# mpieva/mapping-iterative-assembler

Measured on AMD Instinct MI355X. Metric: reads aligned/sec per iteration (16.5kb mito ref, 100bp reads), higher is better.
Workload: dtype int32; 1 GPU; configs[1]: 1000000 synthetic 100 bp reads per GPU vs mt311 (16619 bp, circular), matrix flat; step = reiterate_assembly + pop_smp + cull + consensus; pass-1 coordinates = true positions; reads_per_gpu=1000000, total_reads=1000000, consensus_len=16619, bytes_per_read=182

## Files before the change

include/mia_hip.h:

```cpp
#ifndef MIA_HIP_H
#define MIA_HIP_H

#include <stddef.h>
#include <stdint.h>

#ifdef __cplusplus
extern "C" {
#endif

#define MIA_HIP_OK 0
#define MIA_HIP_ERR_DEVICE (-1)
#define MIA_HIP_ERR_ARG (-2)
#define MIA_HIP_ERR_RANGE (-3)
#define MIA_HIP_ERR_STATE (-4)
#define MIA_HIP_ERR_NOMEM (-5)

#define MIA_HIP_PSSM_WORDS (31 * 5 * 5)
#define MIA_HIP_MAX_READ 256
#define MIA_HIP_TALLY_WORDS 12

#define MIA_HIP_COL_INSERT (-1)
#define MIA_HIP_COL_CLIP (-2)

typedef struct mia_hip_ctx mia_hip_ctx;

int mia_hip_create(mia_hip_ctx **ctx, int device_index);
void mia_hip_destroy(mia_hip_ctx *ctx);
const char *mia_hip_last_error(const mia_hip_ctx *ctx);
int mia_hip_sync(mia_hip_ctx *ctx);


int mia_hip_set_pssm(mia_hip_ctx *ctx, const int32_t *fwd, const int32_t *rc);

int mia_hip_upload_reads(mia_hip_ctx *ctx, int64_t n_reads, const char *bases, const int64_t *offsets,
                         const uint8_t *rc, const uint8_t *strand_known, const int32_t *as, const int32_t *ae);


#define MIA_HIP_P1_PASSED 1
#define MIA_HIP_P1_KEPT 2
#define MIA_HIP_P1_STRAND_KNOWN 4
#define MIA_HIP_P1_SPLIT 8

int mia_hip_pass1(mia_hip_ctx *ctx, const char *ref, int32_t ref_len, int circular, int kmer_len, int soft_mask,
                  int64_t n_reads, const char *bases, const int64_t *offsets, int32_t *score, uint8_t *rc, int32_t *as,
                  int32_t *ae, uint8_t *flags);


int mia_hip_realign(mia_hip_ctx *ctx, const char *new_ref, int32_t ref_len, int circular);

int mia_hip_get_alignments(mia_hip_ctx *ctx, int32_t *score, int32_t *as, int32_t *ae);

int mia_hip_align_windows(mia_hip_ctx *ctx, const char *ref, int64_t ref_len, const int64_t *win_start, const int32_t *win_len);

int mia_hip_get_scripts(mia_hip_ctx *ctx, int16_t *cols, int32_t stride, int32_t *ref_start);

int mia_hip_cull(mia_hip_ctx *ctx, int32_t hard_cut, double slope, double intercept, int64_t slot_base);
int mia_hip_get_dropped(mia_hip_ctx *ctx, uint8_t *front_dropped, uint8_t *back_dropped);
int mia_hip_set_slot_dropped(mia_hip_ctx *ctx, const uint8_t *flags, int64_t n_flags);

int mia_hip_set_back_slots(mia_hip_ctx *ctx, const int64_t *back_slot);
int mia_hip_set_pass1_state(mia_hip_ctx *ctx, const int64_t *front_slot, const int64_t *back_slot, const int32_t *score);
int mia_hip_get_record_params(mia_hip_ctx *ctx, int32_t *params, int64_t *back_slot);
int mia_hip_set_read_base(mia_hip_ctx *ctx, int64_t read_base);
int mia_hip_links(mia_hip_ctx *ctx, int64_t **d_links, int64_t *n_links);
int mia_hip_set_links(mia_hip_ctx *ctx, const int64_t *d_links_all, int64_t n_all);
int mia_hip_link_lengths(mia_hip_ctx *ctx, int32_t **d_len, int32_t **d_act, int64_t *n);
int mia_hip_finish_links(mia_hip_ctx *ctx);

void mia_hip_score_cut(const int32_t *score, const int32_t *seq_len, const uint8_t *unique_best, int64_t n,
                       double *slope, double *intercept);
int mia_hip_pre_cull_counts(mia_hip_ctx *ctx, int64_t *n_records, int64_t *n_links);

int mia_hip_score_sums(mia_hip_ctx *ctx, int64_t *sums5);
int mia_hip_score_cut_from_sums(const int64_t *sums5, double *slope, double *intercept);
int mia_hip_num_records(mia_hip_ctx *ctx, int64_t *n_records);

int mia_hip_tally(mia_hip_ctx *ctx);
int mia_hip_tally_buffers(mia_hip_ctx *ctx, int32_t **d_tally, int64_t *n_tally_words, int32_t **d_gaps,
                          int64_t *n_gaps_words);
int mia_hip_ins_events(mia_hip_ctx *ctx, uint64_t **d_events, int64_t *n_events);
int mia_hip_set_ins_events(mia_hip_ctx *ctx, const uint64_t *d_events, int64_t n_events);
int mia_hip_get_tally(mia_hip_ctx *ctx, int32_t *tally, int32_t *gaps);
int mia_hip_set_tally(mia_hip_ctx *ctx, int32_t ref_len, const int32_t *tally, const int32_t *gaps);

int mia_hip_consensus(mia_hip_ctx *ctx, int cons_code, char *out, int64_t out_cap, int64_t *out_len);

int mia_hip_iterate(mia_hip_ctx *ctx, const char *new_ref, int32_t ref_len, int circular, int32_t hard_cut,
                    const double *slope_intercept, int cons_code, char *out, int64_t out_cap, int64_t *out_len);

#define MIA_HIP_COMM_ID_BYTES 128
int mia_hip_comm_unique_id(void *id128);
int mia_hip_comm_init(mia_hip_ctx *ctx, const void *id128, int32_t n_ranks, int32_t rank);
int mia_hip_comm_destroy(mia_hip_ctx *ctx);

#define MIA_HIP_OP_SUM 0
#define MIA_HIP_OP_MAX 1
typedef struct mia_hip_collectives {
  void *user;
  int32_t n_ranks, rank;
  int (*all_gather)(void *user, const void *d_send, void *d_recv, size_t bytes, void *hip_stream);
  int (*all_reduce_i32)(void *user, void *d_buf, size_t count, int op, void *hip_stream);
  int (*query)(void *user, int32_t *n_ranks, int32_t *rank);
  void (*abort)(void *user);
  void (*destroy)(void *user);
  const char *(*error)(void *user);
  const char *name;
} mia_hip_collectives;
int mia_hip_comm_attach(mia_hip_ctx *ctx, const mia_hip_collectives *table);
int mia_hip_comm_info(mia_hip_ctx *ctx, int32_t *n_ranks, int32_t *rank, const char **transport);

int mia_hip_loopback_create(int32_t n_ranks, void **group);
int mia_hip_loopback_table(void *group, int32_t rank, mia_hip_collectives *table);
void mia_hip_loopback_destroy(void *group);


int mia_hip_trim(mia_hip_ctx *ctx, const char *adapter, int64_t n_reads, const char *bases, const int64_t *offsets,
                 uint8_t *trimmed, int32_t *trim_point);

int mia_hip_trim_stats(mia_hip_ctx *ctx, int64_t *exact_reruns);

int mia_hip_trim_rerun_stats(mia_hip_ctx *ctx, int64_t *launches, int64_t *scratch_bytes);


int mia_hip_ma_tally(mia_hip_ctx *ctx, int32_t ref_len, const int32_t *gaps, int64_t n_records, const int32_t *start,
                     const uint8_t *revcom, const int64_t *col_off, const char *seq, const char *smp, int64_t n_ins,
                     const int32_t *ins_record, const int32_t *ins_pos, const int64_t *ins_off, const char *ins_bases);

int mia_hip_get_ins_tally(mia_hip_ctx *ctx, int32_t *ins_off, int32_t *ins_tally, int64_t cap_slots, int64_t *n_slots);

int mia_hip_ma_region(mia_hip_ctx *ctx, int32_t first, int32_t last, int64_t *n_rows, int64_t *width);
int mia_hip_get_ma_region(mia_hip_ctx *ctx, int64_t *rows, char *text, int64_t cap_rows);

int mia_hip_ma_ace(mia_hip_ctx *ctx, int64_t *n_records, int64_t *body_bytes);
int mia_hip_get_ma_ace(mia_hip_ctx *ctx, int64_t *af_pos, int64_t *padded_len, int64_t *body_off, char *body, int64_t cap_bytes);

int mia_hip_ma_sam(mia_hip_ctx *ctx, const char *ref_seq, int64_t *n_records, int64_t *body_bytes);
int mia_hip_get_ma_sam(mia_hip_ctx *ctx, int32_t *nm, int64_t *body_off, char *body, int64_t cap_bytes);

int mia_hip_ma_profile(mia_hip_ctx *ctx, const char *ref_seq, const uint8_t *use, int64_t *n_used, int64_t *n_events);
int mia_hip_get_ma_profile(mia_hip_ctx *ctx, int64_t *count, int64_t *del, int64_t *bad_code, int64_t *beyond);

int mia_hip_ma_ends(mia_hip_ctx *ctx, const char *ref_seq, const uint8_t *segment, const uint8_t *use, int64_t *n_used, int64_t *n_ends5,
                    int64_t *n_ends3);
int mia_hip_get_ma_ends(mia_hip_ctx *ctx, int64_t *ctx_count, int64_t *len_count, int64_t *halves);

int mia_hip_ma_cols(mia_hip_ctx *ctx, const uint8_t *segment, const uint8_t *use, int64_t *n_used, int64_t *n_events, int64_t *beyond,
                    int64_t *ends_outside);
int mia_hip_get_ma_cols(mia_hip_ctx *ctx, int32_t *cols);

int mia_hip_ma_dedup(mia_hip_ctx *ctx, int32_t ref_len, int64_t n_records, const int32_t *start, const int32_t *end, const uint8_t *revcom,
                     const int32_t *score, const int64_t *mate, int32_t tolerance, int64_t *n_molecules, int64_t *n_clusters);
int mia_hip_get_ma_dedup(mia_hip_ctx *ctx, uint8_t *keep, int64_t *rep, int64_t *size_hist, int64_t *orphans);

int mia_hip_ma_damage(mia_hip_ctx *ctx, const char *ref_seq, const uint8_t *use, const int64_t *mate, int32_t n_pos, int32_t single_stranded,
                      int32_t ends_mode, int64_t *n_molecules, int64_t *n_kept);
int mia_hip_get_ma_damage(mia_hip_ctx *ctx, uint8_t *pos5, uint8_t *pos3, uint8_t *keep, int64_t *hist, int64_t *orphans);

int mia_hip_ma_mask(mia_hip_ctx *ctx, int32_t n5, int32_t n3, int32_t mode, int32_t single_stranded, int64_t *n_kept, int64_t *cols_kept);
int mia_hip_get_ma_mask(mia_hip_ctx *ctx, int32_t *first, int32_t *count, int32_t *start, int64_t *col_off, char *seq, char *smp, int64_t cap_bytes,
                        uint8_t *pair_keep, int32_t *ins_pos, int64_t *hist, int64_t *scalars);


int mia_hip_myers(mia_hip_ctx *ctx, int64_t n_pairs, const char *const *seq_a, const char *const *seq_b, const int32_t *mode,
                  const int32_t *maxd, uint32_t *dist);

int mia_hip_myers_packed(mia_hip_ctx *ctx, int64_t n_pairs, const uint32_t *codes, int64_t n_words, const uint32_t *a_off, const uint32_t *b_off,
                         const int32_t *la, const int32_t *lb, const int32_t *mode, const int32_t *maxd, uint32_t *dist);

int mia_hip_myers_time(mia_hip_ctx *ctx, double *kernel_ms);

int mia_hip_myers_align(mia_hip_ctx *ctx, const char *seq_a, int32_t mode, const char *seq_b, int32_t maxd, uint32_t *dist,
                        char *bt_a, char *bt_b);

int mia_hip_kernel_time(mia_hip_ctx *ctx, int reset, double *align_ms, int64_t *align_launches);
int mia_hip_plain_stats(mia_hip_ctx *ctx, int reset, double *plain_ms, int64_t *plain_launches, int64_t *reads_in,
                        int64_t *reads_retried);

int mia_hip_filter_stats(mia_hip_ctx *ctx, int reset, int64_t *reads_seen, int64_t *reads_finished, double *kernel_ms, int64_t *launches);
int mia_hip_band_stats(mia_hip_ctx *ctx, int reset, int64_t *reads_finished, double *kernel_ms, int64_t *launches);
int mia_hip_bx_stats(mia_hip_ctx *ctx, int reset, int64_t *reads4, double *kernel_ms3, int64_t *launches);
int mia_hip_bx_counters(mia_hip_ctx *ctx, uint32_t *out32);
int mia_hip_stage_stats(mia_hip_ctx *ctx, int reset, int32_t cap, const char **names, double *ms, int64_t *launches, int32_t *n_stages);
int mia_hip_set_stage_mask(mia_hip_ctx *ctx, uint32_t mask);
int mia_hip_measure_peaks(mia_hip_ctx *ctx, int64_t copy_bytes, double *hbm_copy_gbs, double *valu_ginst_s);
int mia_hip_measure_issue(mia_hip_ctx *ctx, double *add_ginst_s, double *shader_clock_mhz);
int mia_hip_pass1_time(mia_hip_ctx *ctx, double *kernel_ms);
int mia_hip_pass1_filtered(mia_hip_ctx *ctx, int64_t *reads);
int mia_hip_pass1_anchored(mia_hip_ctx *ctx, int64_t *reads);

#ifdef __cplusplus
}
#endif
#endif
```

mapping-iterative-assembler_amd/__init__.py:

```python
import ctypes as C
import os

import numpy as np

_HERE = os.path.dirname(os.path.abspath(__file__))
LIB_PATH = os.environ.get("MIA_HIP_LIB") or os.path.join(_HERE, "libmia_hip.so")
ALT_LIB_PATH = os.path.join(_HERE, "libmia_hip_alt.so")
RELEASE_ENV = {"MIA_HIP_THREADS", "MIA_HIP_TIMING", "MIA_HIP_LOOPBACK_TIMEOUT", "MIA_HIP_SPIN_WAIT", "MIA_HIP_LIB"}


def alt_switches_set():
    return sorted(k for k in os.environ if k.startswith("MIA_HIP_") and k not in RELEASE_ENV)

PSSM_WORDS = 31 * 5 * 5
TALLY_WORDS = 12
COL_INSERT, COL_CLIP = -1, -2
P1_PASSED, P1_KEPT, P1_STRAND_KNOWN, P1_SPLIT = 1, 2, 4, 8


class MiaHipError(RuntimeError):
    pass


def _load(path=None):
    path = path or LIB_PATH
    if not os.path.exists(path):
        raise MiaHipError(f"{path} is missing: run __graft_entry__.build() (hipcc --offload-arch=gfx950)")
    lib = C.CDLL(path)
    P, vp = C.POINTER, C.c_void_p
    lib.mia_hip_create.argtypes = [P(vp), C.c_int]
    lib.mia_hip_destroy.argtypes = [vp]
    lib.mia_hip_destroy.restype = None
    lib.mia_hip_last_error.argtypes = [vp]
    lib.mia_hip_last_error.restype = C.c_char_p
    lib.mia_hip_sync.argtypes = [vp]
    lib.mia_hip_set_pssm.argtypes = [vp, vp, vp]
    lib.mia_hip_upload_reads.argtypes = [vp, C.c_int64, vp, vp, vp, vp, vp, vp]
    lib.mia_hip_pass1.argtypes = [vp, C.c_char_p, C.c_int32, C.c_int, C.c_int, C.c_int, C.c_int64, vp, vp, vp, vp, vp, vp, vp]
    lib.mia_hip_realign.argtypes = [vp, C.c_char_p, C.c_int32, C.c_int]
    lib.mia_hip_align_windows.argtypes = [vp, vp, C.c_int64, vp, vp]
    lib.mia_hip_get_alignments.argtypes = [vp, vp, vp, vp]
    lib.mia_hip_get_scripts.argtypes = [vp, vp, C.c_int32, vp]
    lib.mia_hip_cull.argtypes = [vp, C.c_int32, C.c_double, C.c_double, C.c_int64]
    lib.mia_hip_get_dropped.argtypes = [vp, vp, vp]
    lib.mia_hip_set_slot_dropped.argtypes = [vp, vp, C.c_int64]
    lib.mia_hip_score_cut.argtypes = [vp, vp, vp, C.c_int64, P(C.c_double), P(C.c_double)]
    lib.mia_hip_score_cut.restype = None
    lib.mia_hip_num_records.argtypes = [vp, P(C.c_int64)]
    lib.mia_hip_tally.argtypes = [vp]
    lib.mia_hip_tally_buffers.argtypes = [vp, P(vp), P(C.c_int64), P(vp), P(C.c_int64)]
    lib.mia_hip_ins_events.argtypes = [vp, P(vp), P(C.c_int64)]
    lib.mia_hip_set_ins_events.argtypes = [vp, vp, C.c_int64]
    lib.mia_hip_get_tally.argtypes = [vp, vp, vp]
    lib.mia_hip_set_tally.argtypes = [vp, C.c_int32, vp, vp]
    lib.mia_hip_iterate.argtypes = [vp, C.c_char_p, C.c_int32, C.c_int, C.c_int32, vp, C.c_int, vp, C.c_int64, P(C.c_int64)]
    lib.mia_hip_consensus.argtypes = [vp, C.c_int, vp, C.c_int64, P(C.c_int64)]
    lib.mia_hip_myers.argtypes = [vp, C.c_int64, vp, vp, vp, vp, vp]
    if hasattr(lib, "mia_hip_myers_packed"):
        lib.mia_hip_myers_packed.argtypes = [vp, C.c_int64, vp, C.c_int64, vp, vp, vp, vp, vp, vp, vp]
    lib.mia_hip_pre_cull_counts.argtypes = [vp, vp, vp]
    lib.mia_hip_filter_stats.argtypes = [vp, C.c_int, vp, vp, vp, vp]
    lib.mia_hip_band_stats.argtypes = [vp, C.c_int, vp, vp, vp]
    lib.mia_hip_bx_stats.argtypes = [vp, C.c_int, vp, vp, vp]
    lib.mia_hip_bx_counters.argtypes = [vp, vp]
    lib.mia_hip_myers_align.argtypes = [vp, C.c_char_p, C.c_int32, C.c_char_p, C.c_int32, vp, vp, vp]
    lib.mia_hip_pass1_time.argtypes = [vp, P(C.c_double)]
    lib.mia_hip_myers_time.argtypes = [vp, P(C.c_double)]
    lib.mia_hip_ma_tally.argtypes = [vp, C.c_int32, vp, C.c_int64, vp, vp, vp, vp, vp, C.c_int64, vp, vp, vp, vp]
    lib.mia_hip_trim.argtypes = [vp, C.c_char_p, C.c_int64, vp, vp, vp, vp]
    lib.mia_hip_set_back_slots.argtypes = [vp, vp]
    lib.mia_hip_set_pass1_state.argtypes = [vp, vp, vp, vp]
    lib.mia_hip_get_record_params.argtypes = [vp, vp, vp]
    lib.mia_hip_set_read_base.argtypes = [vp, C.c_int64]
    lib.mia_hip_links.argtypes = [vp, P(vp), P(C.c_int64)]
    lib.mia_hip_set_links.argtypes = [vp, vp, C.c_int64]
    lib.mia_hip_link_lengths.argtypes = [vp, P(vp), P(vp), P(C.c_int64)]
    lib.mia_hip_finish_links.argtypes = [vp]
    lib.mia_hip_plain_stats.argtypes = [vp, C.c_int, P(C.c_double), P(C.c_int64), P(C.c_int64), P(C.c_int64)]
    lib.mia_hip_score_sums.argtypes = [vp, vp]
    lib.mia_hip_score_cut_from_sums.argtypes = [vp, P(C.c_double), P(C.c_double)]
    lib.mia_hip_score_cut_from_sums.restype = C.c_int
    lib.mia_hip_trim_stats.argtypes = [vp, P(C.c_int64)]
    if hasattr(lib, "mia_hip_trim_rerun_stats"):
        lib.mia_hip_trim_rerun_stats.argtypes = [vp, P(C.c_int64), P(C.c_int64)]
    lib.mia_hip_get_ins_tally.argtypes = [vp, vp, vp, C.c_int64, P(C.c_int64)]
    if hasattr(lib, "mia_hip_ma_region"):
        lib.mia_hip_ma_region.argtypes = [vp, C.c_int32, C.c_int32, P(C.c_int64), P(C.c_int64)]
        lib.mia_hip_get_ma_region.argtypes = [vp, vp, vp, C.c_int64]
    if hasattr(lib, "mia_hip_ma_ace"):
        lib.mia_hip_ma_ace.argtypes = [vp, P(C.c_int64), P(C.c_int64)]
        lib.mia_hip_get_ma_ace.argtypes = [vp, vp, vp, vp, vp, C.c_int64]
    if hasattr(lib, "mia_hip_ma_sam"):
        lib.mia_hip_ma_sam.argtypes = [vp, vp, P(C.c_int64), P(C.c_int64)]
        lib.mia_hip_get_ma_sam.argtypes = [vp, vp, vp, vp, C.c_int64]
    if hasattr(lib, "mia_hip_ma_profile"):
        lib.mia_hip_ma_profile.argtypes = [vp, vp, vp, P(C.c_int64), P(C.c_int64)]
        lib.mia_hip_get_ma_profile.argtypes = [vp, vp, vp, P(C.c_int64), P(C.c_int64)]
    if hasattr(lib, "mia_hip_ma_ends"):
        lib.mia_hip_ma_ends.argtypes = [vp, vp, vp, vp, P(C.c_int64), P(C.c_int64), P(C.c_int64)]
        lib.mia_hip_get_ma_ends.argtypes = [vp, vp, vp, P(C.c_int64)]
    if hasattr(lib, "mia_hip_ma_cols"):
        lib.mia_hip_ma_cols.argtypes = [vp, vp, vp, P(C.c_int64), P(C.c_int64), P(C.c_int64), P(C.c_int64)]
        lib.mia_hip_get_ma_cols.argtypes = [vp, vp]
    if hasattr(lib, "mia_hip_ma_dedup"):
        lib.mia_hip_ma_dedup.argtypes = [vp, C.c_int32, C.c_int64, vp, vp, vp, vp, vp, C.c_int32, P(C.c_int64), P(C.c_int64)]
        lib.mia_hip_get_ma_dedup.argtypes = [vp, vp, vp, vp, P(C.c_int64)]
    if hasattr(lib, "mia_hip_ma_damage"):
        lib.mia_hip_ma_damage.argtypes = [vp, vp, vp, vp, C.c_int32, C.c_int32, C.c_int32, P(C.c_int64), P(C.c_int64)]
        lib.mia_hip_get_ma_damage.argtypes = [vp, vp, vp, vp, vp, P(C.c_int64)]
    if hasattr(lib, "mia_hip_ma_mask"):
        lib.mia_hip_ma_mask.argtypes = [vp, C.c_int32, C.c_int32, C.c_int32, C.c_int32, P(C.c_int64), P(C.c_int64)]
        lib.mia_hip_get_ma_mask.argtypes = [vp, vp, vp, vp, vp, vp, vp, C.c_int64, vp, vp, vp, vp]
    lib.mia_hip_kernel_time.argtypes = [vp, C.c_int, P(C.c_double), P(C.c_int64)]
    lib.mia_hip_stage_stats.argtypes = [vp, C.c_int, C.c_int32, vp, vp, vp, P(C.c_int32)]
    lib.mia_hip_set_stage_mask.argtypes = [vp, C.c_uint32]
    lib.mia_hip_comm_unique_id.argtypes = [vp]
    lib.mia_hip_comm_init.argtypes = [vp, vp, C.c_int32, C.c_int32]
    lib.mia_hip_comm_destroy.argtypes = [vp]
    lib.mia_hip_comm_attach.argtypes = [vp, vp]
    lib.mia_hip_comm_info.argtypes = [vp, P(C.c_int32), P(C.c_int32), P(C.c_char_p)]
    lib.mia_hip_loopback_create.argtypes = [C.c_int32, P(vp)]
    lib.mia_hip_loopback_table.argtypes = [vp, C.c_int32, vp]
    lib.mia_hip_loopback_destroy.argtypes = [vp]
    lib.mia_hip_loopback_destroy.restype = None
    lib.mia_hip_measure_peaks.argtypes = [vp, C.c_int64, P(C.c_double), P(C.c_double)]
    lib.mia_hip_measure_issue.argtypes = [vp, P(C.c_double), P(C.c_double)]
    return lib


_lib = None


def lib():
    global _lib
    if _lib is None:
        _lib = _load()
    return _lib


_alt_lib = None


def alt_lib():
    global _alt_lib
    if _alt_lib is None:
        _alt_lib = _load(ALT_LIB_PATH)
    return _alt_lib


def exported_symbols():
    return ["mia_hip_create", "mia_hip_destroy", "mia_hip_last_error", "mia_hip_sync", "mia_hip_set_pssm",
            "mia_hip_upload_reads", "mia_hip_pass1", "mia_hip_realign", "mia_hip_align_windows", "mia_hip_get_alignments", "mia_hip_get_scripts", "mia_hip_cull",
            "mia_hip_get_dropped", "mia_hip_set_slot_dropped", "mia_hip_score_cut", "mia_hip_num_records",
            "mia_hip_tally", "mia_hip_tally_buffers", "mia_hip_ins_events", "mia_hip_set_ins_events",
            "mia_hip_get_tally", "mia_hip_consensus", "mia_hip_myers", "mia_hip_myers_packed", "mia_hip_myers_align", "mia_hip_filter_stats", "mia_hip_band_stats", "mia_hip_bx_stats", "mia_hip_bx_counters", "mia_hip_kernel_time", "mia_hip_pass1_time", "mia_hip_myers_time", "mia_hip_pass1_filtered", "mia_hip_pass1_anchored", "mia_hip_pre_cull_counts", "mia_hip_ma_tally", "mia_hip_get_ins_tally", "mia_hip_ma_region", "mia_hip_get_ma_region", "mia_hip_ma_ace", "mia_hip_get_ma_ace", "mia_hip_ma_sam", "mia_hip_get_ma_sam", "mia_hip_ma_profile", "mia_hip_get_ma_profile", "mia_hip_ma_ends", "mia_hip_get_ma_ends", "mia_hip_ma_cols", "mia_hip_get_ma_cols", "mia_hip_ma_dedup", "mia_hip_get_ma_dedup", "mia_hip_ma_damage", "mia_hip_get_ma_damage", "mia_hip_ma_mask", "mia_hip_get_ma_mask", "mia_hip_trim", "mia_hip_trim_stats", "mia_hip_trim_rerun_stats", "mia_hip_set_back_slots", "mia_hip_set_pass1_state",
            "mia_hip_get_record_params", "mia_hip_set_read_base", "mia_hip_links", "mia_hip_set_links", "mia_hip_link_lengths",
            "mia_hip_finish_links", "mia_hip_plain_stats", "mia_hip_score_sums",
            "mia_hip_score_cut_from_sums", "mia_hip_stage_stats", "mia_hip_measure_peaks", "mia_hip_measure_issue", "mia_hip_set_tally", "mia_hip_iterate", "mia_hip_set_stage_mask", "mia_hip_comm_unique_id", "mia_hip_comm_init", "mia_hip_comm_destroy",
            "mia_hip_comm_attach", "mia_hip_comm_info", "mia_hip_loopback_create", "mia_hip_loopback_table", "mia_hip_loopback_destroy"]


def _ptr(a):
    return a.ctypes.data_as(C.c_void_p) if a is not None else None


def flat_pssm():
    p = np.zeros((31, 5, 5), dtype=np.int32)
    for i in range(5):
        for j in range(4):
            p[:, i, j] = 200 if i == j else -600
        p[:, i, 4] = -100
    p[:, 4, :] = -10
    return p


def revcom_pssm(p):
    idx = np.array([3, 2, 1, 0, 4])
    return np.ascontiguousarray(p[::-1][:, idx][:, :, idx]).astype(np.int32)


def read_pssm(path):
    p = np.zeros((31, 5, 5), dtype=np.int32)
    with open(path) as f:
        lines = f.read().split("\n")
    k = 0
    for d in range(31):
        if "# Matrix for position" not in lines[k]:
            raise ValueError(f"Problem parsing matrix file: {path}")
        for i in range(4):
            p[d, i, :4] = [int(x) for x in lines[k + 1 + i].split("\t")[:4]]
            p[d, i, 4] = -100
        p[d, 4, :] = -10
        k += 6
    return p


class Collectives(C.Structure):
    _fields_ = [("user", C.c_void_p), ("n_ranks", C.c_int32), ("rank", C.c_int32),
                ("all_gather", C.c_void_p), ("all_reduce_i32", C.c_void_p), ("query", C.c_void_p), ("abort", C.c_void_p),
                ("destroy", C.c_void_p), ("error", C.c_void_p), ("name", C.c_char_p)]


class LoopbackGroup:

    def __init__(self, n_ranks, like=None):
        self._l = like._l if like is not None else lib()
        self._g = C.c_void_p()
        if self._l.mia_hip_loopback_create(n_ranks, C.byref(self._g)) != 0:
            raise MiaHipError("mia_hip_loopback_create failed")
        self.n_ranks = n_ranks

    def attach(self, hip, rank):
        if hip._l is not self._l:
            raise MiaHipError("LoopbackGroup: this context comes from another build of the library than the group (pass like=<a context> when the group is made)")
        t = Collectives()
        if self._l.mia_hip_loopback_table(self._g, rank, C.byref(t)) != 0:
            raise MiaHipError("mia_hip_loopback_table failed")
        hip.comm_attach(t)

    def close(self):
        if self._g:
            self._l.mia_hip_loopback_destroy(self._g)
            self._g = C.c_void_p()


def comm_unique_id():
    buf = C.create_string_buffer(128)
    if lib().mia_hip_comm_unique_id(buf) != 0:
        raise MiaHipError("mia_hip_comm_unique_id failed: librccl could not be opened")
    return buf.raw


_IUPAC_BITS = np.zeros(256, np.uint8)
for _c, _v in zip("ACGTUSWRYKMBDHVN", (1, 2, 4, 8, 8, 6, 9, 5, 10, 12, 3, 14, 13, 11, 7, 15)):
    _IUPAC_BITS[ord(_c)] = _v
    _IUPAC_BITS[ord(_c.lower())] = _v


def pack_myers_pairs(seq_a, seq_b):
    n = len(seq_a)
    la = np.array([len(s) for s in seq_a], np.int32)
    lb = np.array([len(s) for s in seq_b], np.int32)
    wa, wb = (la + 7) // 8 + 1, (lb + 7) // 8 + 1
    tot = np.cumsum(np.stack([wa, wb], 1).reshape(-1).astype(np.int64))
    a_off = np.concatenate([[0], tot[1:-1:2]]).astype(np.uint32) if n else np.zeros(0, np.uint32)
    b_off = tot[0::2].astype(np.uint32)
    nib = np.zeros(int(tot[-1]) * 8 if n else 0, np.uint8)
    for i in range(n):
        a = np.frombuffer(seq_a[i] if isinstance(seq_a[i], bytes) else seq_a[i].encode(), np.uint8)
        b = np.frombuffer(seq_b[i] if isinstance(seq_b[i], bytes) else seq_b[i].encode(), np.uint8)
        nib[int(a_off[i]) * 8: int(a_off[i]) * 8 + len(a)] = _IUPAC_BITS[a]
        nib[int(b_off[i]) * 8: int(b_off[i]) * 8 + len(b)] = _IUPAC_BITS[b]
    codes = (nib.reshape(-1, 8).astype(np.uint32) << (4 * np.arange(8, dtype=np.uint32))).sum(axis=1).astype(np.uint32)
    return codes, a_off, b_off, la, lb


class MiaHip:

    def __init__(self, device=0):
        self.is_alt_build = bool(alt_switches_set() and not os.environ.get("MIA_HIP_LIB"))
        self._l = alt_lib() if self.is_alt_build else lib()
        self.lib_path = ALT_LIB_PATH if self.is_alt_build else LIB_PATH
        self._h = C.c_void_p()
        rc = self._l.mia_hip_create(C.byref(self._h), device)
        if rc != 0:
            raise MiaHipError(f"mia_hip_create failed ({rc}): no usable gfx950 device -- there is no CPU fallback")
        self.n = 0
        self.max_len = 0
        self.L = 0

    def close(self):
        if self._h:
            self._l.mia_hip_destroy(self._h)
            self._h = C.c_void_p()

    def __del__(self):
        try:
            self.close()
        except Exception:
            pass

    def _chk(self, rc):
        if rc != 0:
            raise MiaHipError(f"libmia_hip error {rc}: {self._l.mia_hip_last_error(self._h).decode()}")

    def set_pssm(self, fwd, rc=None):
        fwd = np.ascontiguousarray(fwd, dtype=np.int32)
        rc = np.ascontiguousarray(revcom_pssm(fwd) if rc is None else rc, dtype=np.int32)
        self._chk(self._l.mia_hip_set_pssm(self._h, _ptr(fwd), _ptr(rc)))

    def upload_reads(self, bases, offsets, rc, strand_known, as_, ae):
        bases = np.ascontiguousarray(bases, dtype=np.uint8)
        offsets = np.ascontiguousarray(offsets, dtype=np.int64)
        rc = np.ascontiguousarray(rc, dtype=np.uint8)
        sk = np.ascontiguousarray(strand_known, dtype=np.uint8)
        as_ = np.ascontiguousarray(as_, dtype=np.int32)
        ae = np.ascontiguousarray(ae, dtype=np.int32)
        self.n = len(offsets) - 1
        self.lens = (offsets[1:] - offsets[:-1]).astype(np.int32)
        self.max_len = int(self.lens.max()) if self.n else 0
        self._chk(self._l.mia_hip_upload_reads(self._h, self.n, _ptr(bases), _ptr(offsets), _ptr(rc), _ptr(sk), _ptr(as_), _ptr(ae)))

    def pass1(self, ref, circular, bases, offsets, kmer_len=-1, soft_mask=False):
        if isinstance(ref, str):
            ref = ref.encode()
        bases = np.ascontiguousarray(bases, dtype=np.uint8)
        offsets = np.ascontiguousarray(offsets, dtype=np.int64)
        n = len(offsets) - 1
        score = np.zeros(n, np.int32); as_ = np.zeros(n, np.int32); ae = np.zeros(n, np.int32)
        rc = np.zeros(n, np.uint8); flags = np.zeros(n, np.uint8)
# ... 307 lines not shown
            raise ValueError("ma_ends: the reference has %d characters, the tallied job %d columns" % (len(ref), self.L))
        if segment is not None:
            if isinstance(segment, str):
                segment = segment.encode("latin1")
            segment = np.frombuffer(segment, np.uint8) if isinstance(segment, (bytes, bytearray)) else np.ascontiguousarray(segment, dtype=np.uint8)
        if use is not None:
            use = np.ascontiguousarray(use, dtype=np.uint8)
        ctx, lens = np.zeros((2, 20, 6), dtype=np.int64), np.zeros((2, 513), dtype=np.int64)
        halves = C.c_int64()
        self._chk(self._l.mia_hip_ma_ends(self._h, C.c_char_p(ref), _ptr(segment) if segment is not None and segment.size else None,
                                          _ptr(use) if use is not None and use.size else None, None, None, None))
        self._chk(self._l.mia_hip_get_ma_ends(self._h, _ptr(ctx), _ptr(lens), C.byref(halves)))
        return ctx, lens, halves.value

    def ma_cols(self, segment=None, use=None):
        if segment is not None:
            if isinstance(segment, str):
                segment = segment.encode("latin1")
            segment = np.frombuffer(segment, np.uint8) if isinstance(segment, (bytes, bytearray)) else np.ascontiguousarray(segment, dtype=np.uint8)
        if use is not None:
            use = np.ascontiguousarray(use, dtype=np.uint8)
        cols = np.zeros((16, self.L), dtype=np.int32)
        n_used, n_events, beyond, outside = C.c_int64(), C.c_int64(), C.c_int64(), C.c_int64()
        self._chk(self._l.mia_hip_ma_cols(self._h, _ptr(segment) if segment is not None and segment.size else None,
                                          _ptr(use) if use is not None and use.size else None, C.byref(n_used), C.byref(n_events),
                                          C.byref(beyond), C.byref(outside)))
        self._chk(self._l.mia_hip_get_ma_cols(self._h, _ptr(cols)))
        return cols, n_used.value, n_events.value, beyond.value, outside.value

    def ma_dedup(self, ref_len, start, end, revcom, score, mate=None, tolerance=0):
        if not hasattr(self._l, "mia_hip_ma_dedup"):
            raise RuntimeError("this libmia_hip has no mia_hip_ma_dedup")
        start = np.ascontiguousarray(start, dtype=np.int32)
        end = np.ascontiguousarray(end, dtype=np.int32)
        revcom = np.ascontiguousarray(revcom, dtype=np.uint8)
        score = np.ascontiguousarray(score, dtype=np.int32)
        n = len(start)
        if not (len(end) == len(revcom) == len(score) == n):
            raise ValueError("ma_dedup: the arrays differ in length")
        if mate is not None:
            mate = np.ascontiguousarray(mate, dtype=np.int64)
            if len(mate) != n:
                raise ValueError("ma_dedup: the arrays differ in length")
        keep, rep, hist = np.zeros(n, dtype=np.uint8), np.zeros(n, dtype=np.int64), np.zeros((2, 1025), dtype=np.int64)
        n_mol, n_clu, orphans = C.c_int64(), C.c_int64(), C.c_int64()
        opt = lambda a: _ptr(a) if n else None
        self._chk(self._l.mia_hip_ma_dedup(self._h, int(ref_len), n, opt(start), opt(end), opt(revcom), opt(score),
                                           _ptr(mate) if mate is not None and n else None, int(tolerance), C.byref(n_mol), C.byref(n_clu)))
        self._chk(self._l.mia_hip_get_ma_dedup(self._h, opt(keep), opt(rep), _ptr(hist), C.byref(orphans)))
        return keep, rep, hist, n_mol.value, n_clu.value, orphans.value

    DAMAGE_MODES = {"any": 0, "5": 1, "3": 2, "both": 3}

    def ma_damage(self, ref_seq, n_pos, use=None, mate=None, single_stranded=False, mode="any"):
        if not hasattr(self._l, "mia_hip_ma_damage"):
            raise RuntimeError("this libmia_hip has no mia_hip_ma_damage")
        ref = ref_seq.encode("latin1") if isinstance(ref_seq, str) else bytes(ref_seq)
        if len(ref) != self.L:
            raise ValueError("ma_damage: the reference has %d characters, the tallied job %d columns" % (len(ref), self.L))
        if mode not in self.DAMAGE_MODES:
            raise ValueError("ma_damage: mode must be one of any, 5, 3, both")
        if use is not None:
            use = np.ascontiguousarray(use, dtype=np.uint8)
        if mate is not None:
            mate = np.ascontiguousarray(mate, dtype=np.int64)
        n = getattr(self, "_ma_n", 0)
        if (use is not None and len(use) != n) or (mate is not None and len(mate) != n):
            raise ValueError("ma_damage: use and mate hold one entry per tallied record (%d)" % n)
        n_mol, n_kept, orphans = C.c_int64(), C.c_int64(), C.c_int64()
        self._chk(self._l.mia_hip_ma_damage(self._h, C.c_char_p(ref), _ptr(use) if use is not None and use.size else None,
                                            _ptr(mate) if mate is not None and mate.size else None, int(n_pos), 1 if single_stranded else 0,
                                            self.DAMAGE_MODES[mode], C.byref(n_mol), C.byref(n_kept)))
        pos5, pos3, keep = np.zeros(n, dtype=np.uint8), np.zeros(n, dtype=np.uint8), np.zeros(n, dtype=np.uint8)
        hist = np.zeros((2, 16, 16), dtype=np.int64)
        opt = lambda a: _ptr(a) if n else None
        self._chk(self._l.mia_hip_get_ma_damage(self._h, opt(pos5), opt(pos3), opt(keep), _ptr(hist), C.byref(orphans)))
        return pos5, pos3, keep, hist, n_mol.value, n_kept.value, orphans.value

    def ma_mask(self, n5, n3, substitute=False, single_stranded=False):
        if not hasattr(self._l, "mia_hip_ma_mask"):
            raise RuntimeError("this libmia_hip has no mia_hip_ma_mask")
        n_kept, cols_kept = C.c_int64(), C.c_int64()
        self._chk(self._l.mia_hip_ma_mask(self._h, int(n5), int(n3), 1 if substitute else 0, 1 if single_stranded else 0, C.byref(n_kept), C.byref(cols_kept)))
        n = getattr(self, "_ma_n", 0)
        n_ins = getattr(self, "_ma_n_ins", 0)
        first, count, start = np.zeros(n, dtype=np.int32), np.zeros(n, dtype=np.int32), np.zeros(n, dtype=np.int32)
        col_off = np.zeros(n + 1, dtype=np.int64)
        seq, smp = np.zeros(cols_kept.value, dtype=np.uint8), np.zeros(cols_kept.value, dtype=np.uint8)
        pair_keep, ins_pos = np.zeros(n_ins, dtype=np.uint8), np.zeros(n_ins, dtype=np.int32)
        hist, scalars = np.zeros((2, 2, 16), dtype=np.int64), np.zeros(6, dtype=np.int64)
        opt = lambda a: _ptr(a) if a.size else None
        self._chk(self._l.mia_hip_get_ma_mask(self._h, opt(first), opt(count), opt(start), _ptr(col_off), opt(seq), opt(smp), cols_kept.value, opt(pair_keep),
                                              opt(ins_pos), _ptr(hist), _ptr(scalars)))
        return {"first": first, "count": count, "start": start, "col_off": col_off, "seq": seq, "smp": smp, "pair_keep": pair_keep, "ins_pos": ins_pos, "hist": hist,
                "emptied": [int(scalars[0]), int(scalars[1])], "stripped": int(scalars[2]), "pairs_dropped": int(scalars[3]), "n_kept": int(scalars[4]),
                "cols_kept": int(scalars[5])}

    def ins_tally(self):
        n = C.c_int64()
        off = np.empty(self.L + 1, dtype=np.int32)
        self._chk(self._l.mia_hip_get_ins_tally(self._h, _ptr(off), None, 0, C.byref(n)))
        t = np.zeros((max(n.value, 1), 9), dtype=np.int32)
        if n.value:
            self._chk(self._l.mia_hip_get_ins_tally(self._h, None, _ptr(t), n.value, None))
        return off, t[: n.value]

    def trim(self, adapter, bases, offsets):
        if isinstance(adapter, str):
            adapter = adapter.encode()
        bases = np.ascontiguousarray(bases, dtype=np.uint8)
        offsets = np.ascontiguousarray(offsets, dtype=np.int64)
        n = len(offsets) - 1
        trimmed = np.zeros(n, np.uint8)
        point = np.zeros(n, np.int32)
        self._chk(self._l.mia_hip_trim(self._h, adapter, n, _ptr(bases), _ptr(offsets), _ptr(trimmed), _ptr(point)))
        return trimmed, point

    def set_back_slots(self, back_slot):
        b = np.ascontiguousarray(back_slot, dtype=np.int64)
        assert len(b) == self.n
        self._chk(self._l.mia_hip_set_back_slots(self._h, _ptr(b)))

    def set_pass1_state(self, front_slot=None, back_slot=None, score=None):
        f = None if front_slot is None else np.ascontiguousarray(front_slot, dtype=np.int64)
        b = None if back_slot is None else np.ascontiguousarray(back_slot, dtype=np.int64)
        sc = None if score is None else np.ascontiguousarray(score, dtype=np.int32)
        self._chk(self._l.mia_hip_set_pass1_state(self._h, _ptr(f), _ptr(b), _ptr(sc)))

    def record_params(self):
        p = np.empty((self.n, 8), dtype=np.int32)
        b = np.empty(self.n, dtype=np.int64)
        self._chk(self._l.mia_hip_get_record_params(self._h, _ptr(p), _ptr(b)))
        return p, b

    def set_read_base(self, base):
        self._chk(self._l.mia_hip_set_read_base(self._h, int(base)))

    def links(self):
        p, n = C.c_void_p(), C.c_int64()
        self._chk(self._l.mia_hip_links(self._h, C.byref(p), C.byref(n)))
        return p.value, n.value

    def set_links(self, dptr, n):
        self._chk(self._l.mia_hip_set_links(self._h, C.c_void_p(dptr), int(n)))

    def link_lengths(self):
        p, q, n = C.c_void_p(), C.c_void_p(), C.c_int64()
        self._chk(self._l.mia_hip_link_lengths(self._h, C.byref(p), C.byref(q), C.byref(n)))
        return p.value, q.value, n.value

    def finish_links(self):
        self._chk(self._l.mia_hip_finish_links(self._h))

    def plain_stats(self, reset=False):
        ms, a, b, c = C.c_double(), C.c_int64(), C.c_int64(), C.c_int64()
        self._chk(self._l.mia_hip_plain_stats(self._h, 1 if reset else 0, C.byref(ms), C.byref(a), C.byref(b), C.byref(c)))
        return ms.value, a.value, b.value, c.value

    def trim_exact_reruns(self):
        n = C.c_int64()
        self._chk(self._l.mia_hip_trim_stats(self._h, C.byref(n)))
        return n.value

    def trim_rerun_stats(self):
        a, b = C.c_int64(), C.c_int64()
        self._chk(self._l.mia_hip_trim_rerun_stats(self._h, C.byref(a), C.byref(b)))
        return a.value, b.value

    def pass1_time(self):
        ms = C.c_double()
        self._chk(self._l.mia_hip_pass1_time(self._h, C.byref(ms)))
        return ms.value

    def sync(self):
        self._chk(self._l.mia_hip_sync(self._h))
```

mapping-iterative-assembler_amd/csrc/mia_consensus_kernels.h:

```cpp
#pragma once
#include <hip/hip_runtime.h>
#include <stdint.h>

#include "ma_records.h"
#include "mia_kernels.h"
#include "mia_layout.h"

namespace mia {

struct TallyBuf {
  int32_t* tally;
  int32_t Lp;
  int32_t* gaps;
  uint64_t* events;
  int32_t* n_events;
  int32_t cap_events;
  uint32_t* flags;
};

struct RecGeom {
  int start_w, end, split, ncols_f, ncols_b;
};
MIA_HD inline RecGeom rec_geom(int as, int ae, int L) {
  RecGeom g;
  g.start_w = as;
  g.end = ae > L ? ae - L : ae;
  g.split = as > g.end;
  g.ncols_f = g.split ? (L - as) : (g.end - as + 1);
  g.ncols_b = g.split ? g.end + 1 : 0;
  return g;
}

__global__ void k_scan_blocks(ReadSet rs, int32_t L, int64_t* partial) {
  __shared__ int32_t sh[256];
  const int64_t base = ((int64_t)blockIdx.x * 256 + threadIdx.x) * 16;
  int32_t s = 0;
  for (int k = 0; k < 16; k++) {
    int64_t i = base + k;
    if (i < rs.n && rs.sk[i]) s += rec_geom(rs.as[i], rs.ae[i], L).split ? 2 : 1;
  }
  sh[threadIdx.x] = s;
  __syncthreads();
  for (int o = 128; o > 0; o >>= 1) {
    if ((int)threadIdx.x < o) sh[threadIdx.x] += sh[threadIdx.x + o];
    __syncthreads();
  }
  if (threadIdx.x == 0) partial[blockIdx.x] = sh[0];
}
__global__ __launch_bounds__(256) void k_scan_partials(int64_t* partial, int nb, int64_t base, int64_t* total, const int32_t* abort_if = nullptr) {
  if (abort_if && *abort_if != 0) return;
  __shared__ int64_t s_run[256];
  const int t = threadIdx.x, per = (nb + 255) / 256, b0 = t * per, b1 = b0 + per < nb ? b0 + per : nb;
  int64_t mine = 0;
  for (int b = b0; b < b1; b++) mine += partial[b];
  const int lane = t & 63, w = t >> 6;
  int64_t inc = mine;
#pragma unroll
  for (int o = 1; o < 64; o <<= 1) { const int64_t u = (int64_t)__shfl_up((long long)inc, o); if (lane >= o) inc += u; }
  if (lane == 63) s_run[w] = inc;
  __syncthreads();
  int64_t off = 0;
  for (int k = 0; k < w; k++) off += s_run[k];
  const int64_t all = s_run[0] + s_run[1] + s_run[2] + s_run[3];
  int64_t run = base + off + inc - mine;
  for (int b = b0; b < b1; b++) { const int64_t v = partial[b]; partial[b] = run; run += v; }
  if (t == 255) *total = all;
}
__global__ void k_scan_apply(ReadSet rs, int32_t L, const int64_t* partial, int64_t* slot) {
  __shared__ int32_t sh[256];
  const int64_t base = ((int64_t)blockIdx.x * 256 + threadIdx.x) * 16;
  int32_t cnt[16], s = 0;
  for (int k = 0; k < 16; k++) {
    int64_t i = base + k;
    cnt[k] = (i < rs.n && rs.sk[i]) ? (rec_geom(rs.as[i], rs.ae[i], L).split ? 2 : 1) : 0;
    s += cnt[k];
  }
  sh[threadIdx.x] = s;
  __syncthreads();
  for (int o = 1; o < 256; o <<= 1) {
    int32_t v = ((int)threadIdx.x >= o) ? sh[threadIdx.x - o] : 0;
    __syncthreads();
    sh[threadIdx.x] += v;
    __syncthreads();
  }
  int64_t run = partial[blockIdx.x] + sh[threadIdx.x] - s;
  for (int k = 0; k < 16; k++) {
    int64_t i = base + k;
    if (i < rs.n) slot[i] = run;
    run += cnt[k];
  }
}

__global__ void k_score_sums_init(unsigned long long* sums, const int32_t* wide_count) {
  if (threadIdx.x == 0) {
    sums[0] = 0; sums[1] = 0; sums[2] = 0; sums[3] = (unsigned long long)(long long)INT32_MAX; sums[4] = (unsigned long long)(long long)INT32_MIN; sums[5] = 0; sums[6] = 0;
    sums[7] = wide_count ? (unsigned long long)*wide_count : 0;
  }
}

__global__ __launch_bounds__(256) void k_score_sums(ReadSet rs, unsigned long long* out, int32_t L, const int64_t* back_slot,
                                                     const int64_t* front_slot0) {
  __shared__ unsigned long long sh[5][256];
  __shared__ int shl[2][256];
  unsigned long long sx = 0, sy = 0, j = 0, nrec = 0, nlink = 0;
  int lmin = INT32_MAX, lmax = INT32_MIN;
  for (int64_t i = (int64_t)blockIdx.x * blockDim.x + threadIdx.x; i < rs.n; i += (int64_t)gridDim.x * blockDim.x) {
    const int sc = rs.score[i], ln = rs.len[i];
    if (sc >= 2000) { sx += (unsigned long long)ln; sy += (unsigned long long)sc; j++; lmin = ln < lmin ? ln : lmin; lmax = ln > lmax ? ln : lmax; }
    if (rs.sk[i]) {
      const bool split = rec_geom(rs.as[i], rs.ae[i], L).split;
      nrec += split ? 2 : 1;
      if (!split && back_slot[i] >= 0) nlink++;
    } else {
      nlink += (front_slot0[i] >= 0) + (back_slot[i] >= 0);
    }
  }
  sh[0][threadIdx.x] = sx; sh[1][threadIdx.x] = sy; sh[2][threadIdx.x] = j; sh[3][threadIdx.x] = nrec; sh[4][threadIdx.x] = nlink;
  shl[0][threadIdx.x] = lmin; shl[1][threadIdx.x] = lmax;
  __syncthreads();
  for (int o = 128; o > 0; o >>= 1) {
    if ((int)threadIdx.x < o) {
      for (int k = 0; k < 5; k++) sh[k][threadIdx.x] += sh[k][threadIdx.x + o];
      shl[0][threadIdx.x] = min(shl[0][threadIdx.x], shl[0][threadIdx.x + o]);
      shl[1][threadIdx.x] = max(shl[1][threadIdx.x], shl[1][threadIdx.x + o]);
    }
    __syncthreads();
  }
  if (threadIdx.x == 0) {
    atomicAdd(&out[0], sh[0][0]); atomicAdd(&out[1], sh[1][0]); atomicAdd(&out[2], sh[2][0]);
    atomicAdd(&out[5], sh[3][0]); atomicAdd(&out[6], sh[4][0]);
    atomicMin(reinterpret_cast<long long*>(&out[3]), (long long)shl[0][0]);
    atomicMax(reinterpret_cast<long long*>(&out[4]), (long long)shl[1][0]);
  }
}

struct RecInfo {
  int32_t* flen;
  int32_t* blen;
  int32_t* actf;
  int32_t* trec;
};
enum { TREC_AS = 0, TREC_AE, TREC_LEN_ABR, TREC_FLAGS, TREC_REFSTART, TREC_ROFF, TREC_ACTF, TREC_SPARE, TREC_PARAMS = 8 };
constexpr int TRF_RC = 1, TRF_DF = 2, TRF_DB = 4, TRF_DIAG = 8, TRF_TOO_LONG = 16, TRF_SK = 32, TRF_ONEGAP = 64;
constexpr int TRF_NO_N = 128;
__device__ __forceinline__ void rec_write(const ReadSet& rs, int64_t i, int32_t* trec, uint8_t* drop_front, uint8_t* drop_back, uint8_t df, uint8_t db, const int32_t* p,
                                          uint32_t st, int32_t actf, const int32_t* umax) {
  drop_front[i] = df;
  drop_back[i] = db;
  int4* t4 = reinterpret_cast<int4*>(trec + i * 16);
  const int fl = (rs.rc[i] ? TRF_RC : 0) | (df ? TRF_DF : 0) | (db ? TRF_DB : 0) | ((st & ST_DIAG) ? TRF_DIAG : 0) |
                 ((st & ST_TOO_LONG) ? TRF_TOO_LONG : 0) | (rs.sk[i] ? TRF_SK : 0) | ((st & ST_ONEGAP) ? TRF_ONEGAP : 0) |
                 ((umax && umax[i] >= 0) ? TRF_NO_N : 0);
  t4[0] = make_int4(rs.as[i], rs.ae[i], (int32_t)((uint32_t)rs.len[i] | ((uint32_t)(uint16_t)rs.abr[i] << 16)), fl);
  t4[1] = make_int4(rs.refstart[i], (int32_t)rs.roff[i], actf, (int32_t)(st >> 8));
  t4[2] = make_int4(p[0], p[1], p[2], p[3]);
  t4[3] = make_int4(p[4], p[5], p[6], p[7]);
}

__device__ __forceinline__ void rec_make(const ReadSet& rs, int64_t i, uint8_t* drop_front, uint8_t* drop_back, uint8_t df, uint8_t db, const int32_t* p,
                                         uint32_t st, int32_t actf, const int32_t* umax, int4* r4) {
  drop_front[i] = df;
  drop_back[i] = db;
  const int fl = (rs.rc[i] ? TRF_RC : 0) | (df ? TRF_DF : 0) | (db ? TRF_DB : 0) | ((st & ST_DIAG) ? TRF_DIAG : 0) |
                 ((st & ST_TOO_LONG) ? TRF_TOO_LONG : 0) | (rs.sk[i] ? TRF_SK : 0) | ((st & ST_ONEGAP) ? TRF_ONEGAP : 0) |
                 ((umax && umax[i] >= 0) ? TRF_NO_N : 0);
  r4[0] = make_int4(rs.as[i], rs.ae[i], (int32_t)((uint32_t)rs.len[i] | ((uint32_t)(uint16_t)rs.abr[i] << 16)), fl);
  r4[1] = make_int4(rs.refstart[i], (int32_t)rs.roff[i], actf, (int32_t)(st >> 8));
  r4[2] = make_int4(p[0], p[1], p[2], p[3]);
  r4[3] = make_int4(p[4], p[5], p[6], p[7]);
}
__device__ __forceinline__ void rec_store_wave(int32_t* trec, int64_t i0, int64_t n, const int4* r4, int lane, int4* buf) {
#pragma unroll
  for (int q = 0; q < 4; q++) buf[lane * 4 + q] = r4[q];
  __builtin_amdgcn_fence(__ATOMIC_RELEASE, "wavefront");
  __builtin_amdgcn_wave_barrier();
  __builtin_amdgcn_fence(__ATOMIC_ACQUIRE, "wavefront");
  int4* out = reinterpret_cast<int4*>(trec) + i0 * 4;
#pragma unroll
  for (int k = 0; k < 4; k++) {
    const int w = k * 64 + lane;
    if (i0 + (w >> 2) < n) out[w] = buf[w];
  }
}

struct SlotInfo {
  int64_t base;
  const int64_t* n_local_p;
  int32_t* reclen;
  int32_t* recact;
  unsigned long long* writer;
  int32_t* mult;
};
constexpr unsigned long long LINK_NONE = 0xFFFFFull;
struct Links {
  int64_t* rec;
  int32_t* n;
  int32_t cap;
};

__device__ __forceinline__ void rec_store_at(int64_t i, const RecGeom& g, int nf, int nb, int af, int bases, int64_t slot_i, RecInfo& ri,
                                             SlotInfo& si, int64_t read_base, uint32_t* flags) {
  const int flen = g.ncols_f + nf, blen = g.split ? g.ncols_b + nb : 0;
  ri.flen[i] = flen; ri.blen[i] = blen; ri.actf[i] = af + nf;
  const int64_t ls = slot_i - si.base;
  if (ls >= 0 && ls + (g.split ? 1 : 0) < (*si.n_local_p)) {
    const unsigned long long me = ((unsigned long long)(read_base + i) << 20) | LINK_NONE;
    si.reclen[ls] = flen; si.recact[ls] = af + nf; si.mult[ls] = 1; si.writer[ls] = me;
    if (g.split) { si.reclen[ls + 1] = blen; si.recact[ls + 1] = bases - (af + nf); si.mult[ls + 1] = 1; si.writer[ls + 1] = me; }
  } else atomicOr(flags, 4u);
}
__device__ __forceinline__ void rec_store(int64_t i, const RecGeom& g, int nf, int nb, int af, int bases, const int64_t* slot, RecInfo& ri,
                                          SlotInfo& si, int64_t read_base, uint32_t* flags) {
  rec_store_at(i, g, nf, nb, af, bases, slot[i], ri, si, read_base, flags);
}

__global__ __launch_bounds__(256) void k_rec_geom(ReadSet rs, int32_t L, const int64_t* slot, RecInfo ri, SlotInfo si, int64_t read_base,
                                                    uint32_t* flags) {
  const int lane = threadIdx.x & 63;
  const int64_t i0 = (int64_t)blockIdx.x * 256 + (threadIdx.x & ~63);
  const int64_t me = i0 + lane;
  bool walk = false;
  if (me < rs.n) {
    if (!rs.sk[me]) { ri.flen[me] = 0; ri.blen[me] = 0; ri.actf[me] = 0; }
    else if (rs.status[me] & ST_DIAG) {
      const int len2 = rs.len[me], abr = rs.abr[me];
      const RecGeom g = rec_geom(rs.as[me], rs.ae[me], L);
      const int af = (len2 - abr) < g.ncols_f ? (len2 - abr) : g.ncols_f;
      rec_store(me, g, 0, 0, af, len2 - abr, slot, ri, si, read_base, flags);
    } else if ((rs.status[me] & ST_ONEGAP) && !rec_geom(rs.as[me], rs.ae[me], L).split) {
      const uint32_t desc = rs.status[me] >> 8;
      const int len2 = rs.len[me], abr = rs.abr[me], gn = (int)((desc >> 10) & 63u), ins = (int)(desc & 1u);
      const RecGeom g = rec_geom(rs.as[me], rs.ae[me], L);
      rec_store(me, g, ins ? gn : 0, 0, len2 - abr - (ins ? gn : 0), len2 - abr, slot, ri, si, read_base, flags);
    } else walk = true;
  }
  unsigned long long todo = __ballot(walk);
  while (todo) {
    const int64_t i = i0 + __builtin_ctzll(todo);
    todo &= todo - 1;
    const int len2 = rs.len[i], abr = rs.abr[i];
    const RecGeom g = rec_geom(rs.as[i], rs.ae[i], L);
    const int16_t* cols = rs.cols + (int64_t)i * rs.stride;
    const int cbase = rs.refstart[i] - g.start_w;
    int nf = 0, nb = 0, af = 0;
    int n_ev = 0, ins_rows = 0, ev_row = 0, ev_len = 0, ev_kind = 0;
    for (int r0 = abr; r0 < len2; r0 += 64) {
      const int r = r0 + lane;
      bool isF = false, isB = false, alF = false, ins_row = false, ins_start = false, jump = false;
      int jump_len = 0;
      if (r < len2) {
        const int cp = r > abr ? (int)cols[r - 1] : -3;
        if (cols[r] == COL_INSERT) {
          int rn = r + 1;
          while (rn < len2 && cols[rn] < 0) rn++;
          const int o = cbase + cols[rn];
          if (o < g.ncols_f) isF = true; else if (g.split && o - g.ncols_f < g.ncols_b) isB = true;
          ins_row = true;
          ins_start = cp != COL_INSERT;
        } else if (cols[r] >= 0) {
          alF = (cbase + cols[r]) < g.ncols_f;
          if (cp >= 0 && cols[r] - cp > 1) { jump = true; jump_len = cols[r] - cp - 1; }
        }
      }
      nf += __popcll(__ballot(isF));
      nb += __popcll(__ballot(isB));
      af += __popcll(__ballot(alF));
      const unsigned long long m_ins = __ballot(ins_start), m_del = __ballot(jump);
      ins_rows += __popcll(__ballot(ins_row));
      if (n_ev == 0 && (m_ins | m_del)) {
        const int l = __builtin_ctzll(m_ins | m_del);
        ev_row = r0 + l;
        ev_kind = (int)((m_ins >> l) & 1ull);
        ev_len = __shfl(jump_len, l);
      }
      n_ev += __popcll(m_ins) + __popcll(m_del);
    }
    if (lane == 0) {
      const uint32_t st = rs.status[i];
      if (!(st & (ST_ESCAPE | ST_TOO_LONG | ST_SKIPPED | ST_BAND | ST_DIAG))) {
        const int gn = ev_kind ? ins_rows : ev_len, n_al = len2 - abr;
        const bool one = n_ev == 1 && !g.split && gn > 0 && gn < 64 && ev_row < 512 && g.ncols_f == (ev_kind ? n_al - gn : n_al + gn);
        const uint32_t want = one ? (ST_ONEGAP | (((uint32_t)ev_kind | ((uint32_t)ev_row << 1) | ((uint32_t)gn << 10)) << 8)) : ST_OK;
        if (st != want) rs.status[i] = want;
      }
    }
    if (lane == 0) rec_store(i, g, nf, nb, af, len2 - abr, slot, ri, si, read_base, flags);
  }
}

__global__ __launch_bounds__(256) void k_slot_count(ReadSet rs, int32_t L, int64_t* partial, int nb, int64_t base, int64_t* total, uint32_t* blocks_done, const int32_t* abort_if = nullptr) {
  if (abort_if && *abort_if != 0) return;
  __shared__ bool last;
  __shared__ int64_t s_run[256];
  __shared__ int32_t wsum[16][4];
  const int64_t base_read = (int64_t)blockIdx.x * 4096;
  uint8_t sk16[16];
  int32_t as16[16], ae16[16];
#pragma unroll
  for (int k = 0; k < 16; k++) {
    const int64_t i = base_read + k * 256 + threadIdx.x;
    const bool in = i < rs.n;
    sk16[k] = in ? rs.sk[i] : (uint8_t)0;
    as16[k] = in ? rs.as[i] : 0;
    ae16[k] = in ? rs.ae[i] : 0;
  }
#pragma unroll
  for (int k = 0; k < 16; k++) {
    const int cnt = sk16[k] ? (rec_geom(as16[k], ae16[k], L).split ? 2 : 1) : 0;
    const int w = __popcll(__ballot(cnt >= 1)) + __popcll(__ballot(cnt == 2));
    if ((threadIdx.x & 63) == 0) wsum[k][threadIdx.x >> 6] = w;
  }
  __syncthreads();
  if (threadIdx.x < 16 && blockIdx.x * 16 + (int)threadIdx.x < nb)
    partial[blockIdx.x * 16 + threadIdx.x] = (int64_t)wsum[threadIdx.x][0] + wsum[threadIdx.x][1] + wsum[threadIdx.x][2] + wsum[threadIdx.x][3];
  if (!blocks_done) {
    if (threadIdx.x == 0) {
      int64_t g = 0;
      for (int k = 0; k < 16; k++) g += (int64_t)wsum[k][0] + wsum[k][1] + wsum[k][2] + wsum[k][3];
      partial[nb + blockIdx.x] = g;
    }
    return;
  }
  __threadfence();
  __syncthreads();
  if (threadIdx.x == 0) last = atomicAdd(blocks_done, 1u) == (uint32_t)gridDim.x - 1u;
  __syncthreads();
  if (!last) return;
  __threadfence();
  const int t = threadIdx.x, per = (nb + 255) / 256, b0 = t * per, b1 = b0 + per < nb ? b0 + per : nb;
  int64_t mine = 0;
  for (int b2 = b0; b2 < b1; b2++) mine += __builtin_nontemporal_load(partial + b2);
  s_run[t] = mine;
  __syncthreads();
  for (int o = 1; o < 256; o <<= 1) {
    const int64_t a2 = t >= o ? s_run[t - o] : 0;
    __syncthreads();
    s_run[t] += a2;
    __syncthreads();
  }
  int64_t run = base + s_run[t] - mine;
  for (int b2 = b0; b2 < b1; b2++) { const int64_t v = __builtin_nontemporal_load(partial + b2); partial[b2] = run; run += v; }
  if (t == 255) *total = s_run[255];
  if (t == 0) *blocks_done = 0;
}

__global__ __launch_bounds__(256) void k_cull_records(ReadSet rs, int32_t L, const int64_t* partial, int64_t* slot, RecInfo ri, SlotInfo si, int64_t read_base,
                                                        uint32_t* flags, uint8_t* slot_dropped, int64_t n_slots, int32_t hard_cut, double slope, double intercept,
                                                        int64_t* back_slot, const int64_t* front_slot0, Links lk, const double* dev_cut, const int32_t* abort_if = nullptr,
                                                        int32_t raw_nb = 0, int64_t slot_base = 0, int64_t* total_out = nullptr,
                                                        int32_t with_records = 0, uint8_t* drop_front = nullptr, uint8_t* drop_back = nullptr, const int32_t* umax = nullptr) {
  if (abort_if && *abort_if != 0) return;
  __shared__ int32_t wsum[4];
  __shared__ int64_t s_red[2][4], s_first, s_total;
  const int lane = threadIdx.x & 63, wv = threadIdx.x >> 6;
  if (raw_nb) {
    const int ng = (raw_nb + 15) >> 4, myg = (int)(blockIdx.x >> 4);
    int64_t pre = 0, tot = 0;
    for (int g = threadIdx.x; g < ng; g += 256) { const int64_t v = partial[raw_nb + g]; tot += v; if (g < myg) pre += v; }
    if (threadIdx.x < 16) { const int b = myg * 16 + (int)threadIdx.x; if (b < (int)blockIdx.x) pre += partial[b]; }
#pragma unroll
    for (int o = 32; o; o >>= 1) { pre += __shfl_xor(pre, o); tot += __shfl_xor(tot, o); }
    if (lane == 0) { s_red[0][wv] = pre; s_red[1][wv] = tot; }
    __syncthreads();
    if (threadIdx.x == 0) {
      s_first = slot_base + s_red[0][0] + s_red[0][1] + s_red[0][2] + s_red[0][3];
      s_total = s_red[1][0] + s_red[1][1] + s_red[1][2] + s_red[1][3];
      if (blockIdx.x == 0 && total_out) *total_out = s_total;
    }
    si.n_local_p = &s_total;
  }
  const int64_t i0 = (int64_t)blockIdx.x * 256 + (threadIdx.x & ~63);
  const int64_t me = i0 + lane;
  const bool in = me < rs.n;
  const bool sk = in && rs.sk[me];
  int as_me = 0, ae_me = 0;
  if (sk) { as_me = rs.as[me]; ae_me = rs.ae[me]; }
  const RecGeom g_me = rec_geom(as_me, ae_me, L);
  const int cnt = sk ? (g_me.split ? 2 : 1) : 0;
  const unsigned long long m1 = __ballot(cnt >= 1), m2 = __ballot(cnt == 2), below = (1ull << lane) - 1ull;
  if (lane == 0) wsum[wv] = __popcll(m1) + __popcll(m2);
  __syncthreads();
  int64_t my_slot = (raw_nb ? s_first : partial[blockIdx.x]) + __popcll(m1 & below) + __popcll(m2 & below);
  for (int k = 0; k < wv; k++) my_slot += wsum[k];
  if (in) slot[me] = my_slot;
  int my_flen = 0, my_actf = 0, my_blen = 0;
  uint32_t my_st = in ? rs.status[me] : 0u;
  bool walk = false;
  if (in) {
    if (!sk) { ri.flen[me] = 0; ri.blen[me] = 0; ri.actf[me] = 0; }
    else if (rs.status[me] & ST_DIAG) {
      const int len2 = rs.len[me], abr = rs.abr[me];
      const int af = (len2 - abr) < g_me.ncols_f ? (len2 - abr) : g_me.ncols_f;
      rec_store_at(me, g_me, 0, 0, af, len2 - abr, my_slot, ri, si, read_base, flags);
      my_flen = g_me.ncols_f; my_actf = af; my_blen = g_me.split ? g_me.ncols_b : 0;
    } else if ((rs.status[me] & ST_ONEGAP) && !g_me.split) {
      const uint32_t desc = rs.status[me] >> 8;
      const int len2 = rs.len[me], abr = rs.abr[me], gn = (int)((desc >> 10) & 63u), ins = (int)(desc & 1u);
      rec_store_at(me, g_me, ins ? gn : 0, 0, len2 - abr - (ins ? gn : 0), len2 - abr, my_slot, ri, si, read_base, flags);
      my_flen = g_me.ncols_f + (ins ? gn : 0); my_actf = len2 - abr;
    } else walk = true;
  }
  unsigned long long todo = __ballot(walk);
  while (todo) {
    const int li = __builtin_ctzll(todo);
    const int64_t i = i0 + li;
    todo &= todo - 1;
    const int len2 = rs.len[i], abr = rs.abr[i];
    const RecGeom g = rec_geom(rs.as[i], rs.ae[i], L);
    const int16_t* cols = rs.cols + (int64_t)i * rs.stride;
    const int cbase = rs.refstart[i] - g.start_w;
    int nf = 0, nb = 0, af = 0;
    int n_ev = 0, ins_rows = 0, ev_row = 0, ev_len = 0, ev_kind = 0;
    for (int r0 = abr; r0 < len2; r0 += 64) {
      const int r = r0 + lane;
      bool isF = false, isB = false, alF = false, ins_row = false, ins_start = false, jump = false;
      int jump_len = 0;
      if (r < len2) {
        const int cp = r > abr ? (int)cols[r - 1] : -3;
        if (cols[r] == COL_INSERT) {
          int rn = r + 1;
          while (rn < len2 && cols[rn] < 0) rn++;
          const int o = cbase + cols[rn];
          if (o < g.ncols_f) isF = true; else if (g.split && o - g.ncols_f < g.ncols_b) isB = true;
          ins_row = true;
          ins_start = cp != COL_INSERT;
        } else if (cols[r] >= 0) {
          alF = (cbase + cols[r]) < g.ncols_f;
          if (cp >= 0 && cols[r] - cp > 1) { jump = true; jump_len = cols[r] - cp - 1; }
        }
      }
      nf += __popcll(__ballot(isF));
      nb += __popcll(__ballot(isB));
      af += __popcll(__ballot(alF));
      const unsigned long long m_ins = __ballot(ins_start), m_del = __ballot(jump);
      ins_rows += __popcll(__ballot(ins_row));
      if (n_ev == 0 && (m_ins | m_del)) {
        const int l = __builtin_ctzll(m_ins | m_del);
        ev_row = r0 + l;
        ev_kind = (int)((m_ins >> l) & 1ull);
        ev_len = __shfl(jump_len, l);
      }
      n_ev += __popcll(m_ins) + __popcll(m_del);
    }
    const int64_t slot_i = __shfl(my_slot, li);
    uint32_t st_new = rs.status[i];
    if (!(st_new & (ST_ESCAPE | ST_TOO_LONG | ST_SKIPPED | ST_BAND | ST_DIAG))) {
      const int gn = ev_kind ? ins_rows : ev_len, n_al = len2 - abr;
      const bool one = n_ev == 1 && !g.split && gn > 0 && gn < 64 && ev_row < 512 && g.ncols_f == (ev_kind ? n_al - gn : n_al + gn);
      const uint32_t want = one ? (ST_ONEGAP | (((uint32_t)ev_kind | ((uint32_t)ev_row << 1) | ((uint32_t)gn << 10)) << 8)) : ST_OK;
      if (st_new != want) { if (lane == 0) rs.status[i] = want; st_new = want; }
    }
    if (lane == 0) rec_store_at(i, g, nf, nb, af, len2 - abr, slot_i, ri, si, read_base, flags);
    if (lane == li) { my_flen = g.ncols_f + nf; my_actf = af + nf; my_blen = g.split ? g.ncols_b + nb : 0; my_st = st_new; }
  }
  __shared__ int4 s_rec[4][256];
  int4 r4[4] = {make_int4(0, 0, 0, 0), make_int4(0, 0, 0, 0), make_int4(0, 0, 0, 0), make_int4(0, 0, 0, 0)};
  if (in) {
  if (dev_cut) { slope = dev_cut[0]; intercept = dev_cut[1]; }
  const double min_score = hard_cut > 0 ? (double)hard_cut : (double)(intercept + (slope * (double)rs.len[me]));
  const bool low = (double)rs.score[me] < min_score;
  auto add_link = [&](int64_t target, int kind, int fl, int ac) {
    const int e = atomicAdd(lk.n, 1);
    if (e < lk.cap) {
      int64_t* r = lk.rec + (int64_t)e * 4;
      r[0] = read_base + me; r[1] = target;
      r[2] = ((int64_t)fl << 32) | (uint32_t)ac;
      r[3] = (low ? 1 : 0) | (kind << 8);
    } else atomicOr(flags, 8u);
  };
  int32_t p[8] = {0, 0, 0, 0, 0, 0, 0, 0};
  if (!sk) {
    if (front_slot0[me] >= 0) add_link(front_slot0[me], 1, 0, 0);
    if (back_slot[me] >= 0) add_link(back_slot[me], 2, 0, 0);
    if (with_records) rec_make(rs, me, drop_front, drop_back, 0, 0, p, my_st, 0, umax, r4);
  } else {
  uint8_t df = 0, db = 0;
  if (with_records && my_slot < n_slots) df = low ? (uint8_t)1 : slot_dropped[my_slot];
  if (with_records && g_me.split && my_slot + 1 < n_slots) db = low ? (uint8_t)1 : slot_dropped[my_slot + 1];
  if (low && my_slot < n_slots) slot_dropped[my_slot] = 1;
  if (g_me.split) {
    if (low && my_slot + 1 < n_slots) slot_dropped[my_slot + 1] = 1;
    back_slot[me] = my_slot + 1;
  } else if (back_slot[me] >= 0) add_link(back_slot[me], 0, my_flen, my_actf);
  if (with_records) {
    const int64_t ls = my_slot - si.base, n_local = *si.n_local_p;
    if (ls >= 0 && ls < n_local) { p[2] = my_flen + my_blen; p[3] = 1; }
    if (g_me.split && ls + 1 < n_local) { p[4] = my_flen; p[5] = my_actf; p[6] = my_flen + my_blen; p[7] = 1; }
    rec_make(rs, me, drop_front, drop_back, df, db, p, my_st, my_actf, umax, r4);
  }
  }
  }
  if (with_records) rec_store_wave(ri.trec, i0, rs.n, r4, lane, s_rec[wv]);
}

__global__ void k_cull_mark(ReadSet rs, int32_t L, const int64_t* slot, uint8_t* slot_dropped, int64_t n_slots, int32_t hard_cut, double slope,
                            double intercept, int64_t* back_slot, const int64_t* front_slot0, RecInfo ri, Links lk, int64_t read_base,
                            uint32_t* flags, const double* dev_cut) {
  int64_t i = (int64_t)blockIdx.x * blockDim.x + threadIdx.x;
  if (i >= rs.n) return;
  if (dev_cut) { slope = dev_cut[0]; intercept = dev_cut[1]; }
  const double min_score = hard_cut > 0 ? (double)hard_cut : (double)(intercept + (slope * (double)rs.len[i]));
  const bool low = (double)rs.score[i] < min_score;
  auto add_link = [&](int64_t target, int kind, int fl, int ac) {
    const int e = atomicAdd(lk.n, 1);
    if (e < lk.cap) {
      int64_t* r = lk.rec + (int64_t)e * 4;
      r[0] = read_base + i; r[1] = target;
      r[2] = ((int64_t)fl << 32) | (uint32_t)ac;
      r[3] = (low ? 1 : 0) | (kind << 8);
    } else atomicOr(flags, 8u);
  };
  if (!rs.sk[i]) {
    if (front_slot0[i] >= 0) add_link(front_slot0[i], 1, 0, 0);
    if (back_slot[i] >= 0) add_link(back_slot[i], 2, 0, 0);
    return;
  }
  const bool split = rec_geom(rs.as[i], rs.ae[i], L).split;
  const int64_t s = slot[i];
  if (low && s < n_slots) slot_dropped[s] = 1;
  if (split) {
    if (low && s + 1 < n_slots) slot_dropped[s + 1] = 1;
    back_slot[i] = s + 1;
  } else if (back_slot[i] >= 0) add_link(back_slot[i], 0, ri.flen[i], ri.actf[i]);
}

__global__ void k_links_apply(const int64_t* links, const int32_t* n_links_p, int32_t cap, SlotInfo si, uint8_t* slot_dropped, int64_t n_slots,
                              int32_t* link_len, int32_t* link_act, uint32_t* flags, const int32_t* abort_if = nullptr) {
  if (abort_if && *abort_if != 0) return;
  const int n_links = min(*n_links_p, cap);
  for (int e = blockIdx.x * blockDim.x + threadIdx.x; e < n_links; e += gridDim.x * blockDim.x) {
    const int64_t* r = links + (int64_t)e * 4;
    const int64_t ls = r[1] - si.base;
    link_len[e] = -1;
    link_act[e] = -1;
    if (ls < 0 || ls >= (*si.n_local_p)) continue;
    atomicMax(&si.writer[ls], ((unsigned long long)r[0] << 20) | (unsigned long long)e);
    atomicAdd(&si.mult[ls], 1);
    if ((r[3] & 1) && r[1] < n_slots) slot_dropped[r[1]] = 1;
    link_len[e] = si.reclen[ls];
    link_act[e] = si.recact[ls];
  }
}

__global__ void k_rec_params(ReadSet rs, int32_t L, const int64_t* slot, const uint8_t* slot_dropped, int64_t n_slots, const int64_t* back_slot,
                             RecInfo ri, SlotInfo si, const int64_t* links, const int32_t* link_len, const int32_t* link_act, const int32_t* n_links_p,
                             int32_t cap, int64_t read_base,
                             uint8_t* drop_front, uint8_t* drop_back, uint32_t* flags, const int32_t* abort_if = nullptr,
                             const int32_t* umax = nullptr,
                             int32_t skip_if_no_links = 0) {
  if (abort_if && *abort_if != 0) return;
  if (skip_if_no_links && *n_links_p == 0) return;
  int64_t i = (int64_t)blockIdx.x * blockDim.x + threadIdx.x;
  if (i >= rs.n) return;
  const int n_links = min(*n_links_p, cap);
  uint8_t df = 0, db = 0;
  int32_t p[8] = {0, 0, 0, 0, 0, 0, 0, 0};
  if (rs.sk[i]) {
    const bool split = rec_geom(rs.as[i], rs.ae[i], L).split;
    const int64_t s = slot[i], ls = s - si.base;
    if (s < n_slots) df = slot_dropped[s];
    if (split && s + 1 < n_slots) db = slot_dropped[s + 1];
    const int flen = ri.flen[i], blen = ri.blen[i], actf = ri.actf[i];
    int back_len = blen;
    if (!split && back_slot[i] >= 0) {
      back_len = -1;
      for (int e = 0; e < n_links; e++)
        if (links[(int64_t)e * 4] == read_base + i && (links[(int64_t)e * 4 + 3] >> 8) == 0) { back_len = link_len[e]; break; }
      if (back_len < 0) { atomicOr(flags, 4u); back_len = 0; }
    }
    auto fill = [&](int32_t* q, int64_t lsl, int own_base, int own_off, int own_B, int own_len) {
      const unsigned long long w = si.writer[lsl];
      if ((w & LINK_NONE) == LINK_NONE) { q[0] = own_base; q[1] = own_off; q[2] = own_B; }
      else {
        const int we = (int)(w & LINK_NONE);
        const int64_t* r = links + (int64_t)we * 4;
        const int kind = (int)(r[3] >> 8);
        if (kind == 0) {
          const int rf = (int)(r[2] >> 32), ra = (int)(uint32_t)r[2];
          q[0] = rf; q[1] = ra; q[2] = rf + own_len;
        } else {
          int sib_len = 0, sib_act = 0;
          for (int e = 0; e < n_links; e++)
            if (links[(int64_t)e * 4] == r[0] && (links[(int64_t)e * 4 + 3] >> 8) == 3 - kind) {
              sib_len = link_len[e]; sib_act = link_act[e];
              if (sib_len < 0) { atomicOr(flags, 4u); sib_len = 0; sib_act = 0; }
              break;
            }
          if (kind == 1) { q[0] = 0; q[1] = 0; q[2] = own_len + sib_len; }
          else { q[0] = sib_len; q[1] = sib_act; q[2] = sib_len + own_len; }
        }
      }
      q[3] = si.mult[lsl];
    };
    if (ls >= 0 && ls < (*si.n_local_p)) fill(p, ls, 0, 0, flen + back_len, flen);
    if (split && ls + 1 < (*si.n_local_p)) fill(p + 4, ls + 1, flen, actf, flen + blen, blen);
  }
  const uint32_t st = rs.status[i];
  rec_write(rs, i, ri.trec, drop_front, drop_back, df, db, p, st, ri.actf[i], umax);
}

__device__ __forceinline__ int depth_code(int dff, int dfb) {
  return dff <= PSSM_DEPTH ? dff : (dfb < PSSM_DEPTH ? 2 * PSSM_DEPTH - dfb : PSSM_DEPTH);
}

constexpr int TALLY_EV_CAP = 256;
constexpr int TALLY_CHUNK_LINEAR = 256;
constexpr int TALLY_BUCKET = 128, TALLY_WIN = 384, TALLY_CHUNK = 512;

__device__ __forceinline__ int tally_slot(int gc, int win_base, int Lp) {
  const int wc = gc - win_base;
  return wc < 0 ? wc + Lp : wc;
}

template <bool BINNED>
__device__ __forceinline__ void tally_one_read(int64_t i, int lane, const ReadSet& rs, const RefInfo& ref, const int32_t* pssm2,
                                               const uint8_t* drop_front, const uint8_t* drop_back, const TallyBuf& tb,
                                               int32_t* lds, int win_base, const int32_t* rec_params, const int32_t* rec_actf,
                                               const int16_t* pssm_lds, unsigned long long* ev_buf, int* ev_cnt, int32_t* n_cnt = nullptr,
                                               const int32_t* rec_lds = nullptr) {
  const int32_t* tr = rec_lds ? rec_lds : rec_params + i * 16;
  const int flags = tr[TREC_FLAGS];
  if (!(flags & TRF_SK)) return;
  if (flags & TRF_TOO_LONG) { if (lane == 0) atomicOr(tb.flags, 2u); return; }
  const int L = ref.L, Lp = tb.Lp;
  const int len2 = tr[TREC_LEN_ABR] & 0xFFFF, abr = (int)(int16_t)((uint32_t)tr[TREC_LEN_ABR] >> 16);
  const RecGeom g = rec_geom(tr[TREC_AS], tr[TREC_AE], L);
  const int16_t* cols = rs.cols + (int64_t)i * rs.stride;
  const int cbase = tr[TREC_REFSTART] - g.start_w;
  const uint8_t* rp = rs.packed + (uint32_t)tr[TREC_ROFF];
  const bool is_rc = (flags & TRF_RC) != 0;
  const int pmo = is_rc ? PSSM_WORDS : 0;
  const int32_t* pm = pssm2 + pmo;
  const bool dF = (flags & TRF_DF) != 0, dB = (flags & TRF_DB) != 0;
  const bool diag = (flags & TRF_DIAG) != 0;
  if (g.split && g.start_w >= L) { if (lane == 0) atomicOr(tb.flags, 2u); return; }
  const int32_t* prm = tr + TREC_PARAMS;
  const int fBase = prm[0], fOff = prm[1], fB = prm[2], fMult = prm[3], bBase = prm[4], bOff = prm[5], bB = prm[6], bMult = prm[7];
  const int actF = tr[TREC_ACTF];
  auto dcode = [&](bool back, int act) {
    const int a = back ? bOff + (act - actF) : fOff + act;
    return depth_code((back ? bBase : fBase) + a, (back ? bB : fB) - a - 1);
  };
  auto emit = [&](int o, int act, int code ) {
    int p, gc, mult;
    bool dropped, back;
    if (o < g.ncols_f) { p = o; gc = g.start_w + o; back = false; dropped = dF; mult = fMult; }
    else if (g.split && o - g.ncols_f < g.ncols_b) { p = o - g.ncols_f; gc = p; back = true; dropped = dB; mult = bMult; }
    else return;
    if (gc < 0 || gc >= Lp) { atomicOr(tb.flags, 2u); return; }
    const int d = dcode(back, act);
    if (d < 0 || d > 2 * PSSM_DEPTH) { atomicOr(tb.flags, 2u); return; }
    const int wc = tally_slot(gc, win_base, Lp);
    const bool in_lds = BINNED && wc >= 0 && wc < TALLY_WIN;
    int s0 = 0, s1 = 0, s2 = 0, s3 = 0;
    if (!dropped && code != 5) {
      if (BINNED) { const int16_t* row = pssm_lds + pmo + d * 25 + code; s0 = row[0]; s1 = row[5]; s2 = row[10]; s3 = row[15]; }
      else { const int32_t* row = pm + d * 25 + code; s0 = row[0]; s1 = row[5]; s2 = row[10]; s3 = row[15]; }
    }
    auto aadd = [](auto* q, int v) { (void)__hip_atomic_fetch_add(q, v, __ATOMIC_RELAXED, __HIP_MEMORY_SCOPE_AGENT); };
    auto add_all = [&](auto* t, const int ws, auto* ncount) {
      if (!dropped) {
        aadd(&t[T_COV * ws], mult);
        if (code == 5) aadd(&t[T_GAP * ws], mult);
        else {
          if (code < 4) aadd(&t[(T_A + code) * ws], mult);
          else if (ncount) aadd(ncount, mult);
          if (!ncount) {
            aadd(&t[T_SA * ws], mult * s0);
            aadd(&t[T_SC * ws], mult * s1);
            aadd(&t[T_SG * ws], mult * s2);
            aadd(&t[T_ST * ws], mult * s3);
          }
        }
      }
      if (p > 0) aadd(&t[T_SPAN * ws], mult);
// ... 1137 lines not shown
```

mapping-iterative-assembler_amd/csrc/mia_hip.hip:

```cpp
#include <hip/hip_runtime.h>
#include <atomic>
#include <hip/hip_ext.h>
#include <stdio.h>
#include <stdlib.h>
#include <string.h>

#include <algorithm>
#include <cmath>
#include <chrono>
#include <optional>
#include <string>
#include <thread>
#include <tuple>
#include <utility>
#include <vector>

#include "../../include/mia_hip.h"
#include "dev_buf.h"
#include "ref_ahead.h"
#include "dev_pool.h"
#include "mia_comm.h"
#include "mia_consensus_kernels.h"
#include "mia_kernels.h"
#include "bandx_kernels.h"
#include "align_route.h"
#include "pass1_route.h"
#include "mia_pass1_kernels.h"
#include "mia_myers_kernels.h"
#include "mia_trim_kernels.h"
#include "mia_peak_kernels.h"
#include "mia_iter_kernels.h"
#include "mia_ma_region_kernels.h"
#include "mia_ma_ace_kernels.h"
#include "mia_ma_sam_kernels.h"
#include "mia_ma_profile_kernels.h"
#include "mia_ma_ends_kernels.h"
#include "mia_ma_cols_kernels.h"
#include "mia_ma_dedup_kernels.h"
#include "mia_ma_damage_kernels.h"
#include "mia_ma_mask_kernels.h"

using namespace mia;

enum Stage { STG_TRACE = 0, STG_PLAIN, STG_FILTER, STG_BAND, STG_BX_PLAN, STG_BX_VALUES, STG_BX_TRACE, STG_TALLY, STG_PASS1, STG_MA_SELECT, STG_MA_RENDER, STG_MA_ACE_LAYOUT, STG_MA_ACE_RENDER, STG_MA_MASK_BOUNDS, STG_MA_MASK_LAYOUT, STG_MA_MASK_APPLY, STG_MA_SAM_LAYOUT, STG_MA_SAM_RENDER, STG_MA_DAMAGE_HITS, STG_MA_DAMAGE_MOLECULES, STG_MA_PROFILE, STG_MA_DEDUP_KEYS, STG_MA_DEDUP_SORT, STG_MA_DEDUP_RUNS, STG_MA_DEDUP_NEXT, STG_MA_DEDUP_ANCHORS, STG_MA_DEDUP_CLUSTERS, STG_MA_TALLY, STG_MA_COLS, STG_MA_ENDS, STG_COUNT };
static const char* const STAGE_NAMES[STG_COUNT] = {"k_align_quad", "k_align_quad_plain", "k_diag_filter", "k_band_align", "k_bx_plan",
                                                   "k_bx_values", "k_bx_trace", "k_tally_binned", "k_pass1", "k_ma_region_select",
                                                   "k_ma_region_render", "k_ma_ace_layout", "k_ma_ace_render", "k_ma_mask_bounds", "k_ma_mask_layout", "k_ma_mask_apply", "k_ma_sam_layout",
                                                   "k_ma_sam_render", "k_ma_damage_hits", "k_ma_damage_molecules", "k_ma_profile", "k_ma_dedup_keys", "k_ma_dedup_sort", "k_ma_dedup_runs",
                                                   "k_ma_dedup_next", "k_ma_dedup_anchors", "k_ma_dedup_clusters", "k_ma_tally", "k_ma_cols", "k_ma_ends"};

constexpr int OPEN_WGS = 1024;
constexpr int64_t OPEN_SLAB_BYTES = (int64_t)MAX_READ * 64 * 12;
constexpr int CTRL_BINS = 0;
constexpr int CTRL_HDR = (3 * N_BINS + 2 + 1) & ~1;
constexpr int CTRL_FILTER = CTRL_HDR + PH_WORDS;
constexpr int CTRL_LKN = CTRL_FILTER + 4, CTRL_CULLF = CTRL_LKN + 1, CTRL_NEV = CTRL_CULLF + 1, CTRL_TFLAGS = CTRL_NEV + 1;
constexpr int CTRL_GENN = CTRL_TFLAGS + 2;
constexpr int CTRL_BXC = (CTRL_GENN + 1 + 63) & ~63;
constexpr int CTRL_WORDS = CTRL_BXC + BXC_WORDS;
constexpr int CTRL_C0 = CTRL_BINS + 3 * N_BINS, CTRL_CN = CTRL_WORDS - CTRL_C0;

#ifdef MIA_HIP_ALT_PATHS
static inline const char* alt_env(const char* name) { return getenv(name); }
#define ALT_KERNEL(k) ((const void*)(k))
#else
static inline const char* alt_env(const char*) { return nullptr; }
#define ALT_KERNEL(k) ((const void*)nullptr)
#endif
static inline std::optional<int> alt_int(const char* name) {
  const char* v = alt_env(name);
  return v ? std::optional<int>(atoi(v)) : std::nullopt;
}

struct mia_hip_ctx {
  int device = 0;
  int cus = 1;
  std::string err;
  DevPool pool;
  unsigned char* h_pin = nullptr; static constexpr size_t PIN_BYTES = 1 << 20, PIN_MISC = 64 << 10;
  DevBuf<int32_t> d_ctrl; int ctrl_half = 0;
  int32_t* ctrl = nullptr;
  int32_t* d_genn = nullptr;
  const int32_t* d_ctr0 = nullptr;
  uint32_t dbg = 0;

  hipStream_t stream = nullptr;
  hipStream_t stream2 = nullptr; hipEvent_t ev_fork = nullptr, ev_join = nullptr;
  hipEvent_t ev_cons = nullptr;
  hipStream_t stream3 = nullptr; hipEvent_t ev_join3 = nullptr;
  uint32_t ext_events = 31u; bool align_end_signalled = false;
  bool spin_wait = true;
  uint32_t stage_mask = ~0u;
  struct StageTimer { std::vector<std::pair<hipEvent_t, hipEvent_t>> pending; double ms = 0; int64_t launches = 0; };
  StageTimer stg[STG_COUNT];
  std::vector<std::pair<hipEvent_t, hipEvent_t>> ev_free;

  DevBuf<int32_t> d_pssm;
  int max_abs = 0;
  int max_pos = 0;
  bool have_pssm = false;
  bool flat = false;
  PackSet packs;
  ReadSet rs{};
  DevBuf<uint8_t> d_packed; DevBuf<uint32_t> d_roff; DevBuf<uint16_t> d_len;
  DevBuf<uint8_t> d_rc, d_sk;
  DevBuf<int32_t> d_as, d_ae, d_score, d_refstart;
  DevBuf<int16_t> d_abr; DevBuf<uint32_t> d_status; DevBuf<int16_t> d_cols;
  int max_len = 0;
  int min_len = 0;
  std::vector<int32_t> h_len;
  DevBuf<uint64_t> d_rplanes; int rplane_words = 0;
  DevBuf<int32_t> d_umax; bool umax_valid = false;
  DevBuf<uint8_t> d_ref; int L = 0, wrap = 0; int explicit_win = 0; bool have_ref = false; bool aligned = false;
  bool ref_mostly_bases = true;
  bool ref_few_n = true;
  int64_t kh_entries = 0;

  DevBuf<int32_t> d_bin_of, d_list, d_wide_list, d_retry_list;
  int32_t* d_bins = nullptr;
  int32_t* d_plan_hdr = nullptr;
  bool deferred = false;
  DevBuf<unsigned char> d_slabs[N_CPL];
  DevBuf<unsigned char> d_slabs_retry[3];
  DevBuf<unsigned char> d_quad_slabs;
  int quad_wgs = 0;
  int grid_wgs = 0;
  int window_wgs[N_CPL] = {0, 0, 0};
  int64_t plain_retried = 0, plain_total = 0;
  bool wide_to_caller = false;
  DevBuf<int32_t> d_scratch; DevBuf<int64_t> d_scratch_off;
  DevBuf<int32_t> d_open_list; DevBuf<unsigned char> d_slabs_open; bool use_direct_open = true; int64_t direct_open_steps = 0;

  int use_filter = 1;
  DevBuf<int32_t> d_kocc_cnt, d_kocc_pos;
  DevBuf<uint64_t> d_planes;
  uint32_t* d_filter_n = nullptr; int64_t filter_proven = 0, filter_seen = 0;
  int use_banddp = 1;
  DevBuf<int32_t> d_left_list;
  DevBuf<uint32_t> d_band_slabs;
  int64_t band_done = 0;

  bool bx_ok = false;
  int use_bx = 1, use_lanes = 1; bool bx_serial = false; uint32_t bx_dbg = 0;
  DevBuf<int32_t> d_bx_sub, d_bx_mrow; DevBuf<int16_t> d_bx_loss, d_bx_dl;
  int32_t bx_min_m = 0, bx_max_m = 0;
  DevBuf<uint32_t> d_refnib;
  DevBuf<uint32_t> d_khash; DevBuf<int32_t> d_khash_ovf;
  DevBuf<KbPair> d_kbits;
  int use_quick = 1; int64_t quick_steps = 0;
  DevBuf<uint32_t> d_prep_bar; uint32_t prep_bar_count = 0; bool no_prep_fuse = false;
  struct RefAhead {
    DevBuf<uint8_t> d_ref; DevBuf<uint64_t> d_planes; DevBuf<uint32_t> d_refnib, d_khash; DevBuf<int32_t> d_khash_ovf; DevBuf<KbPair> d_kbits;
    bool queued = false;
    bool valid = false;
    RefAheadKey key; std::string str;
  } ahead;
  bool no_ref_ahead = false;
  bool ref_ready = false;
  bool last_route_bx = false;
  DevBuf<uint32_t> d_bx_plan; DevBuf<int32_t> d_bx_expect, d_bx_lists;
  DevBuf<BxCandRec> d_bx_cand; bool plan_split = true;
  DevBuf<BxCandRec> d_bx_cand2; int use_fine = 1;
  uint32_t* d_bx_ctr = nullptr;
  DevBuf<uint32_t> d_bx_slabs;
  int bx_values_wgs = 0, bx_trace_wgs = 0;
  DevBuf<uint32_t> d_bx_slabs_late; int bx_late_wgs = 0;
  DevBuf<uint32_t> d_bx_slabs_late2;
  DevBuf<int32_t> d_retry2;
  bool diag_scripts_missing = false;
  int64_t bx_seen = 0, bx_done[3] = {0, 0, 0};
  int64_t bx_launches = 0;
  uint32_t bx_last[BXC_COUNTERS] = {0};

  DevBuf<int64_t> d_slot, d_partial, d_total;
  DevBuf<uint8_t> d_slot_dropped, d_drop_f, d_drop_b; int64_t n_slots = 0;
  DevBuf<int64_t> d_back_slot;
  DevBuf<int64_t> d_front_slot0;
  DevBuf<int32_t> d_link_act;
  RecInfo ri{};
  DevBuf<int32_t> d_ri_flen, d_ri_blen, d_ri_actf, d_ri_trec;
  SlotInfo si{};
  DevBuf<int32_t> d_si_reclen, d_si_recact, d_si_mult; DevBuf<unsigned long long> d_si_writer;
  Links lk{};
  DevBuf<int64_t> d_lk_rec;
  int64_t* d_links_all = nullptr; int32_t n_links_all = 0;
  int32_t* d_n_links_all = nullptr; int64_t links_cap_all = 0; DevBuf<int32_t> d_n_links_gathered;
  DevBuf<int32_t> d_link_len;
  uint32_t* d_cull_flags = nullptr;
  DevBuf<uint32_t> d_cull_sync;
  DevBuf<unsigned long long> d_sums;
  int64_t read_base = 0;
  int64_t slot_base = 0;
  bool culled = false, links_applied = false;
  std::vector<DevBuf<int64_t>> owned_links;
  bool cull_scan = false, tail_scans = false;
  bool cull_with_records = true;
  int64_t pre_cull_records = 0, pre_cull_links = 0; bool pre_cull_valid = false;

  TallyBuf tb{}; DevBuf<int32_t> d_tb_tally, d_ins_off, d_ins_total; DevBuf<uint64_t> d_tb_events;
  DevBuf<int32_t> d_ins_tally; DevBuf<char> d_calls, d_ins_calls;
  int64_t ins_tally_cap = 0;
  int32_t n_events_host = 0; bool tallied = false;
  int64_t ins_total_host = 0;
  bool consensus_done = false;
  bool fake_event_overflow = false;
  bool no_linear_tally = false, sort2_unpacked = false;
  bool tally_linear = false;
  int tally_pk_bias = -1;
  int use_binned_tally = 1;
  DevBuf<int32_t> d_bucket, d_order;
  int bucket_clean_nb = -1;
  int buckets_queued = 0;
  bool no_side_buckets = false;
  DevBuf<int32_t> d_tally_slabs;
  DevBuf<int32_t> d_gen_list;
  bool tally_defer = true;
  bool tally_strand_split = true;
  bool tally_rall = true;
  bool tally_runs = true;
  DevBuf<int32_t> d_order2; DevBuf<uint8_t> d_okey; DevBuf<int32_t> d_sort2;

  bool in_iterate = false;
  const int32_t* abort_if = nullptr;
  bool spec_ok = false, spec_pending = false, spec_filtered = false, spec_bx = false, spec_plain = false;
  int64_t spec_redone = 0;
  bool no_spec = false;
  bool spec_force = false; DevBuf<int32_t> d_one;
  bool pend_encode = false; int32_t pend_L = 0, pend_wl = 0, pend_total = 0;
  bool zero_copy = true;
  const double* dev_cut = nullptr; DevBuf<double> d_cut_buf;
  DevBuf<char> d_ascii; const char* ascii_src = nullptr;
  DevBuf<char> d_cons;
  DevBuf<int32_t> d_cons_pos;
  unsigned char* h_pin2 = nullptr; size_t pin2_bytes = 0;
  int64_t iter_fallbacks = 0;

  double pass1_ms = 0; int64_t pass1_filtered = 0, pass1_anchored = 0;
  double myers_kernel_ms = 0; bool myers_no_lanes = false, myers_no_ond = false;
  int64_t trim_escapes = 0;
  int64_t trim_launches = 0, trim_scratch_bytes = 0;
  bool trim_exact = false;
  bool ma_resident = false; int64_t ma_n = 0, ma_n_ins = 0; int32_t ma_L = 0;
  DevBuf<int32_t> d_ma_start, d_ma_gaps, d_ma_ipos, d_ma_rec_ins, d_ma_ins_list;
  DevBuf<int64_t> d_ma_coff, d_ma_ioff, d_ma_colmap, d_ma_rows;
  DevBuf<char> d_ma_seq, d_ma_ib, d_ma_text;
  DevBuf<unsigned long long> d_ma_ctl;
  struct MaOut {
    bool region_done = false, ace_done = false, sam_done = false, prof_done = false, ends_done = false, cols_done = false, damage_done = false, mask_done = false;
    int32_t first = 0, last = -1; int64_t rows = 0, width = 0, ace_bytes = 0, sam_bytes = 0;
  } ma_out;
  bool ma_ace_gaps_ok = false, ma_ace_cols_ok = false;
  DevBuf<int64_t> d_ace_g, d_ace_af, d_ace_len, d_ace_off; DevBuf<char> d_ace_body;
  bool ma_sam_gaps_ok = false;
  DevBuf<char> d_sam_ref, d_sam_body; DevBuf<int64_t> d_sam_cum, d_sam_cig, d_sam_off; DevBuf<int32_t> d_sam_nm;
  DevBuf<unsigned long long> d_sam_ctl;
  DevBuf<uint8_t> d_ma_rev, d_prof_use; DevBuf<char> d_ma_smp, d_prof_ref; DevBuf<unsigned long long> d_prof_bins;
  int64_t ma_cols = 0; int64_t ma_prof_bins[MA_PROF_BINS] = {0};
  DevBuf<uint8_t> d_ends_seg; DevBuf<unsigned long long> d_ends_bins;
  int64_t ma_ends_bins[MA_ENDS_BINS] = {0};
  DevBuf<uint32_t> d_cols_tab; DevBuf<unsigned long long> d_cols_out;
  std::vector<int32_t> ma_cols_tab;
  struct MaDedup {
    bool done = false; int64_t n = 0, molecules = 0, clusters = 0, orphans = 0;
    DevBuf<int32_t> d_start, d_end, d_score; DevBuf<uint8_t> d_rc, d_keep; DevBuf<int64_t> d_mate, d_rep;
    DevBuf<unsigned long long> d_key[2], d_runkey, d_best, d_ctl, d_hist;
    DevBuf<uint32_t> d_val[2], d_jump[2], d_counts, d_runid, d_first, d_mark, d_cluster, d_anchor;
    int64_t hist[MA_DEDUP_HIST] = {0};
  } dedup;

  struct MaDamage {
    DevBuf<int64_t> d_mate; DevBuf<uint32_t> d_hit; DevBuf<uint8_t> d_pos, d_keep; DevBuf<unsigned long long> d_bins;
    int64_t bins[MA_DMG_BINS] = {0};
  } damage;

  struct MaMask {
    DevBuf<uint32_t> d_lohi; DevBuf<int32_t> d_rec, d_ipos; DevBuf<int64_t> d_off; DevBuf<char> d_seq, d_smp; DevBuf<uint8_t> d_pair_keep;
    DevBuf<unsigned long long> d_ctl, d_bins;
    int64_t bins[MA_MASK_BINS] = {0}, cols_kept = 0; int32_t mode = 0;
  } mask;

  mia_hip_collectives coll{}; bool comm = false; int comm_ranks = 1, comm_rank = 0; std::string coll_name;
  DevBuf<unsigned long long> d_gather;
  std::vector<int64_t> h_gather;
  int64_t ev_pad = 0;
  DevBuf<int64_t> d_lstage, d_lmine, d_lall;
  DevBuf<int32_t> d_scores_all;
};

static void read_alt_switches(mia_hip_ctx* ctx) {
  auto on = [](const char* name) { const char* v = alt_env(name); return v && atoi(v) != 0; };
  if (on("MIA_HIP_NO_DIAG_FILTER")) { ctx->use_filter = 0; ctx->use_bx = 0; }
  if (on("MIA_HIP_NO_BAND_DP")) { ctx->use_banddp = 0; ctx->use_bx = 0; }
  if (on("MIA_HIP_NO_BANDX")) ctx->use_bx = 0;
  if (on("MIA_HIP_NO_LANES")) ctx->use_lanes = 0;
  if (on("MIA_HIP_BX_SERIAL")) ctx->bx_serial = true;
  if (on("MIA_HIP_NO_PLAN_SPLIT")) ctx->plan_split = false;
  if (on("MIA_HIP_NO_FINE")) ctx->use_fine = 0;
  if (const char* v = alt_env("MIA_HIP_FINE")) ctx->use_fine = atoi(v);
  if (on("MIA_HIP_NO_QUICK_PLAN")) ctx->use_quick = 0;
  if (const char* v = alt_env("MIA_HIP_QUICK_PLAN")) ctx->use_quick = atoi(v);
  if (on("MIA_HIP_NO_DIRECT_OPEN")) ctx->use_direct_open = false;
  if (on("MIA_HIP_NO_PREP_FUSE")) ctx->no_prep_fuse = true;
  if (on("MIA_HIP_NO_REF_AHEAD")) ctx->no_ref_ahead = true;
  if (on("MIA_HIP_NO_SPEC")) ctx->no_spec = true;
  if (on("MIA_HIP_SPEC_TEST")) ctx->spec_force = true;
  if (on("MIA_HIP_NO_SIDE_BUCKETS")) ctx->no_side_buckets = true;
  if (on("MIA_HIP_NO_ZERO_COPY")) ctx->zero_copy = false;
  if (on("MIA_HIP_NO_EXT_EVENTS")) ctx->ext_events = 0u;
  if (on("MIA_HIP_FAKE_EVENT_OVERFLOW")) ctx->fake_event_overflow = true;
  if (on("MIA_HIP_CULL_SCAN")) ctx->cull_scan = true;
  if (on("MIA_HIP_TAIL_SCANS")) ctx->tail_scans = true;
  if (on("MIA_HIP_NO_CULL_RECORDS")) ctx->cull_with_records = false;
  if (on("MIA_HIP_NO_BINNED_TALLY")) ctx->use_binned_tally = 0;
  if (on("MIA_HIP_NO_LINEAR_TALLY")) ctx->no_linear_tally = true;
  if (on("MIA_HIP_SORT2_UNPACKED")) ctx->sort2_unpacked = true;
  if (on("MIA_HIP_TALLY_INLINE")) ctx->tally_defer = false;
  if (const char* v = alt_env("MIA_HIP_STRAND_SPLIT")) ctx->tally_strand_split = atoi(v) != 0;
  if (on("MIA_HIP_NO_TALLY_RUNS")) ctx->tally_runs = false;
  if (on("MIA_HIP_NO_TALLY_RALL")) ctx->tally_rall = false;
  if (on("MIA_HIP_MYERS_NO_LANES")) ctx->myers_no_lanes = true;
  if (on("MIA_HIP_MYERS_NO_OND")) ctx->myers_no_ond = true;
  if (on("MIA_HIP_TRIM_EXACT")) ctx->trim_exact = true;
  if (const char* v = alt_env("MIA_HIP_DEBUG_SKIP")) ctx->dbg = (uint32_t)atoi(v);
  if (const char* v = alt_env("MIA_HIP_BX_DEBUG")) ctx->bx_dbg = (uint32_t)atoi(v);
}

#define HIPCHK(call)                                                                                   \
  do {                                                                                                 \
    hipError_t e_ = (call);                                                                            \
    if (e_ != hipSuccess) {                                                                            \
      ctx->err = std::string(#call) + ": " + hipGetErrorString(e_);                                    \
      return MIA_HIP_ERR_DEVICE;                                                                       \
    }                                                                                                  \
  } while (0)

static int dev_nomem(mia_hip_ctx* ctx, hipError_t e) {
  if (e == hipSuccess) return MIA_HIP_OK;
  ctx->err = std::string("hipMalloc: ") + hipGetErrorString(e);
  return MIA_HIP_ERR_NOMEM;
}
template <class T>
static int dev_alloc(mia_hip_ctx* ctx, DevBuf<T>& b, int64_t n) { return dev_nomem(ctx, b.alloc(n)); }
template <class T>
static int dev_ensure(mia_hip_ctx* ctx, DevBuf<T>& b, int64_t need, int64_t alloc_elems) { return dev_nomem(ctx, b.ensure(need, alloc_elems)); }
template <class T>
static int dev_ensure(mia_hip_ctx* ctx, DevBuf<T>& b, int64_t need) { return dev_nomem(ctx, b.ensure(need, need)); }

template <class T>
static int pool_take(mia_hip_ctx* ctx, PoolLease<T>& lease, size_t n) { return dev_nomem(ctx, lease.take(ctx->pool, n)); }

static_assert(CTRL_WORDS % 64 == 0, "the second half of the control block starts on a cache line, as the first does");
static void ctrl_bind(mia_hip_ctx* ctx, int half) {
  const bool own_links = ctx->d_n_links_all && ctx->d_n_links_all == ctx->lk.n;
  int32_t* b = ctx->d_ctrl + (size_t)half * CTRL_WORDS;
  ctx->ctrl_half = half;
  ctx->ctrl = b;
  ctx->d_bins = b + CTRL_BINS;
  ctx->d_plan_hdr = b + CTRL_HDR;
  ctx->d_filter_n = reinterpret_cast<uint32_t*>(b + CTRL_FILTER);
  ctx->lk.n = b + CTRL_LKN;
  ctx->d_cull_flags = reinterpret_cast<uint32_t*>(b + CTRL_CULLF);
  ctx->tb.n_events = b + CTRL_NEV;
  ctx->tb.flags = reinterpret_cast<uint32_t*>(b + CTRL_TFLAGS);
  ctx->d_genn = b + CTRL_GENN;
  ctx->d_bx_ctr = reinterpret_cast<uint32_t*>(b + CTRL_BXC);
  ctx->d_ctr0 = b + CTRL_C0;
  if (own_links) ctx->d_n_links_all = ctx->lk.n;
}

extern "C" const char* mia_hip_last_error(const mia_hip_ctx* ctx) { return ctx ? ctx->err.c_str() : "null context"; }

extern "C" int mia_hip_create(mia_hip_ctx** out, int device_index) {
  if (!out) return MIA_HIP_ERR_ARG;
  *out = nullptr;
  int ndev = 0;
  if (hipGetDeviceCount(&ndev) != hipSuccess || ndev <= 0) return MIA_HIP_ERR_DEVICE;
  if (device_index < 0 || device_index >= ndev) return MIA_HIP_ERR_ARG;
  mia_hip_ctx* ctx = new mia_hip_ctx();
  ctx->device = device_index;
  const unsigned evf = hipEventDisableTiming;
  if (hipSetDevice(device_index) != hipSuccess || hipStreamCreateWithFlags(&ctx->stream, hipStreamNonBlocking) != hipSuccess ||
      hipStreamCreateWithFlags(&ctx->stream2, hipStreamNonBlocking) != hipSuccess || hipStreamCreateWithFlags(&ctx->stream3, hipStreamNonBlocking) != hipSuccess ||
      hipEventCreateWithFlags(&ctx->ev_join3, evf) != hipSuccess || hipEventCreateWithFlags(&ctx->ev_cons, evf) != hipSuccess ||
      hipEventCreateWithFlags(&ctx->ev_fork, evf) != hipSuccess || hipEventCreateWithFlags(&ctx->ev_join, evf) != hipSuccess) {
    delete ctx;
    return MIA_HIP_ERR_DEVICE;
  }
  {
    hipDeviceProp_t prop;
    if (hipGetDeviceProperties(&prop, device_index) != hipSuccess) { delete ctx; return MIA_HIP_ERR_DEVICE; }
    ctx->cus = prop.multiProcessorCount > 0 ? prop.multiProcessorCount : 1;
    ctx->grid_wgs = prop.multiProcessorCount * 32;
    ctx->quad_wgs = prop.multiProcessorCount * 16;
    read_alt_switches(ctx);
    if (const char* sw = getenv("MIA_HIP_SPIN_WAIT")) ctx->spin_wait = atoi(sw) != 0;
  }
  if (dev_alloc(ctx, ctx->d_pssm, 2 * PSSM_WORDS) || dev_alloc(ctx, ctx->d_ctrl, 2 * CTRL_WORDS) ||
      dev_alloc(ctx, ctx->d_total, 1) || dev_alloc(ctx, ctx->d_ins_total, 1) ||
      dev_alloc(ctx, ctx->d_bx_sub, 2 * BX_SUB_WORDS) || dev_alloc(ctx, ctx->d_bx_mrow, 2 * 31 * 4) || dev_alloc(ctx, ctx->d_bx_loss, BX_LOSS_WORDS) ||
      dev_alloc(ctx, ctx->d_bx_dl, BX_DL_WORDS) ||
      dev_alloc(ctx, ctx->d_cut_buf, 2)) {
    delete ctx;
    return MIA_HIP_ERR_NOMEM;
  }
  ctrl_bind(ctx, 0);
  if (hipMemset(ctx->d_ctrl, 0, 2 * CTRL_WORDS * 4) != hipSuccess) { delete ctx; return MIA_HIP_ERR_DEVICE; }
  {
    const int32_t one = 1;
    if (dev_alloc(ctx, ctx->d_one, 1) || hipMemcpy(ctx->d_one, &one, 4, hipMemcpyHostToDevice) != hipSuccess) { delete ctx; return MIA_HIP_ERR_DEVICE; }
    if (dev_alloc(ctx, ctx->d_prep_bar, 1) || hipMemset(ctx->d_prep_bar, 0, 4) != hipSuccess) { delete ctx; return MIA_HIP_ERR_DEVICE; }
  }
  if (hipHostMalloc((void**)&ctx->h_pin, mia_hip_ctx::PIN_BYTES, hipHostMallocDefault) != hipSuccess) ctx->h_pin = nullptr;
  if (ctx->h_pin) memset(ctx->h_pin, 0, mia_hip_ctx::PIN_MISC);
  else ctx->no_prep_fuse = true;
  *out = ctx;
  return MIA_HIP_OK;
}

extern "C" int mia_hip_comm_destroy(mia_hip_ctx* ctx);
extern "C" void mia_hip_destroy(mia_hip_ctx* ctx) {
  if (!ctx) return;
  (void)hipSetDevice(ctx->device);
  (void)hipStreamSynchronize(ctx->stream);
  (void)mia_hip_comm_destroy(ctx);
  if (ctx->h_pin) (void)hipHostFree(ctx->h_pin);
  if (ctx->h_pin2) (void)hipHostFree(ctx->h_pin2);
  for (auto& e : ctx->ev_free) { (void)hipEventDestroy(e.first); (void)hipEventDestroy(e.second); }
  for (auto& t : ctx->stg) for (auto& e : t.pending) { (void)hipEventDestroy(e.first); (void)hipEventDestroy(e.second); }
  (void)hipStreamDestroy(ctx->stream);
  if (ctx->stream2) (void)hipStreamDestroy(ctx->stream2);
  if (ctx->stream3) (void)hipStreamDestroy(ctx->stream3);
  if (ctx->ev_join3) (void)hipEventDestroy(ctx->ev_join3);
  if (ctx->ev_cons) (void)hipEventDestroy(ctx->ev_cons);
  if (ctx->ev_fork) (void)hipEventDestroy(ctx->ev_fork);
  if (ctx->ev_join) (void)hipEventDestroy(ctx->ev_join);
  delete ctx;
}

extern "C" int mia_hip_sync(mia_hip_ctx* ctx) {
  if (!ctx) return MIA_HIP_ERR_ARG;
  HIPCHK(hipSetDevice(ctx->device));
  HIPCHK(hipStreamSynchronize(ctx->stream));
  return MIA_HIP_OK;
}

extern "C" int mia_hip_set_pssm(mia_hip_ctx* ctx, const int32_t* fwd, const int32_t* rc) {
  if (!ctx || !fwd || !rc) return MIA_HIP_ERR_ARG;
  HIPCHK(hipSetDevice(ctx->device));
  int m = 0;
  for (int i = 0; i < PSSM_WORDS; i++) {
    int a = fwd[i] < 0 ? -fwd[i] : fwd[i], b = rc[i] < 0 ? -rc[i] : rc[i];
    if (a > m) m = a;
    if (b > m) m = b;
  }
  if (m > 32000) { ctx->err = "PSSM entries beyond +-32000 do not fit the int16 substitution table"; return MIA_HIP_ERR_RANGE; }
  ctx->max_abs = m;
  {
    int lo = 0, hi = 0;
    for (int k = 0; k < PSSM_WORDS; k++) { lo = std::min(lo, std::min((int)fwd[k], (int)rc[k])); hi = std::max(hi, std::max((int)fwd[k], (int)rc[k])); }
    ctx->tally_pk_bias = -lo + hi <= 2047 ? -lo : -1;
  }
  ctx->max_pos = 0;
  for (int i = 0; i < PSSM_WORDS; i++) { if (fwd[i] > ctx->max_pos) ctx->max_pos = fwd[i]; if (rc[i] > ctx->max_pos) ctx->max_pos = rc[i]; }
  const int cpls[N_CPL] = {4, 8, 12};
  for (int c = 0; c < N_CPL; c++) ctx->packs.ok[c] = make_pack_params(64 * cpls[c], m, &ctx->packs.p[c]) ? 1 : 0;
  HIPCHK(hipMemcpyAsync(ctx->d_pssm, fwd, PSSM_WORDS * 4, hipMemcpyHostToDevice, ctx->stream));
  HIPCHK(hipMemcpyAsync(ctx->d_pssm + PSSM_WORDS, rc, PSSM_WORDS * 4, hipMemcpyHostToDevice, ctx->stream));
  HIPCHK(hipStreamSynchronize(ctx->stream));
  ctx->have_pssm = true;
  ctx->flat = pssm_is_flat(fwd, rc);
  ctx->tally_linear = true;
  for (int d = 0; d < 2 * PSSM_DEPTH + 1; d++)
    for (int x = 0; x < 4; x++)
      for (int b = 0; b < 5; b++)
        if (fwd[(d * 5 + x) * 5 + b] != fwd[x * 5 + b] || rc[(d * 5 + x) * 5 + b] != fwd[x * 5 + b]) ctx->tally_linear = false;
  if (ctx->no_linear_tally) ctx->tally_linear = false;
  {
    std::vector<int32_t> sub(2 * BX_SUB_WORDS, 0), mrow(2 * 31 * 4, 0);
    std::vector<int16_t> loss(BX_LOSS_WORDS, 0), dl(BX_DL_WORDS, 0);
    ctx->bx_ok = bx_make_tables(fwd, rc, sub.data(), mrow.data(), loss.data(), dl.data(), &ctx->bx_min_m, &ctx->bx_max_m);
    if (ctx->bx_ok) {
      for (int k = 0; k < BX_SUB_WORDS; k++) sub[(size_t)BX_SUB_WORDS + k] = sub[(size_t)k] * 256;
      HIPCHK(hipMemcpyAsync(ctx->d_bx_sub, sub.data(), sub.size() * 4, hipMemcpyHostToDevice, ctx->stream));
      HIPCHK(hipMemcpyAsync(ctx->d_bx_mrow, mrow.data(), mrow.size() * 4, hipMemcpyHostToDevice, ctx->stream));
      HIPCHK(hipMemcpyAsync(ctx->d_bx_loss, loss.data(), loss.size() * 2, hipMemcpyHostToDevice, ctx->stream));
      HIPCHK(hipMemcpyAsync(ctx->d_bx_dl, dl.data(), dl.size() * 2, hipMemcpyHostToDevice, ctx->stream));
      HIPCHK(hipStreamSynchronize(ctx->stream));
    }
    ctx->umax_valid = false;
    if (ctx->bx_ok && ctx->d_umax && ctx->rs.n > 0) {
      hipLaunchKernelGGL(k_bx_umax, dim3((unsigned)((ctx->rs.n + 255) / 256)), dim3(256), 0, ctx->stream, ctx->rs, ctx->d_bx_mrow, ctx->d_umax);
      HIPCHK(hipGetLastError());
      ctx->umax_valid = true;
    }
  }
  return MIA_HIP_OK;
}

static inline uint8_t base_code(char b) {
  switch (b) { case 'A': return 0; case 'C': return 1; case 'G': return 2; case 'T': return 3; default: return 4; }
}

static void pack_reads(int64_t n, const char* bases, const int64_t* offsets, const uint32_t* roff, const uint16_t* len, uint8_t* packed) {
  uint8_t lut[256];
  for (int c = 0; c < 256; c++) lut[c] = base_code((char)c);
  auto range = [&](int64_t lo, int64_t hi) {
    for (int64_t i = lo; i < hi; i++) {
      const unsigned char* s = reinterpret_cast<const unsigned char*>(bases) + offsets[i];
      uint8_t* d = packed + roff[i];
      const int l = len[i];
      int k = 0;
      for (; k + 1 < l; k += 2) d[k >> 1] = (uint8_t)(lut[s[k]] | (lut[s[k + 1]] << 4));
      if (k < l) d[k >> 1] = lut[s[k]];
    }
  };
  int T = (int)std::thread::hardware_concurrency();
  if (const char* e = getenv("MIA_HIP_THREADS")) T = atoi(e);
  T = std::max(1, std::min(std::min(T, 32), (int)(n / 16384) + 1));
  if (T == 1) { range(0, n); return; }
  std::vector<std::thread> th;
  for (int t = 1; t < T; t++) th.emplace_back(range, n * t / T, n * (t + 1) / T);
  range(0, n / T);
  for (auto& x : th) x.join();
}

extern "C" int mia_hip_upload_reads(mia_hip_ctx* ctx, int64_t n, const char* bases, const int64_t* offsets, const uint8_t* rc,
                                    const uint8_t* strand_known, const int32_t* as, const int32_t* ae) {
  if (!ctx || n < 0 || (n > 0 && (!bases || !offsets || !rc || !strand_known || !as || !ae))) return MIA_HIP_ERR_ARG;
  if (n >= (int64_t)1 << 31) { ctx->err = "more than 2^31 reads per context"; return MIA_HIP_ERR_ARG; }
  HIPCHK(hipSetDevice(ctx->device));
  std::vector<uint32_t> roff((size_t)n);
  std::vector<uint16_t> len((size_t)n);
  uint64_t total = 0;
  int max_len = 1;
  for (int64_t i = 0; i < n; i++) {
    int64_t l = offsets[i + 1] - offsets[i];
    if (l < 1 || l > MIA_HIP_MAX_READ) { ctx->err = "read length outside 1..256 (INIT_ALN_SEQ_LEN)"; return MIA_HIP_ERR_ARG; }
    roff[i] = (uint32_t)total;
    len[i] = (uint16_t)l;
    if (l > max_len) max_len = (int)l;
    total += (uint64_t)(((l + 1) / 2 + 3) & ~3);
    if (total >= ((uint64_t)1 << 32)) { ctx->err = "packed read store exceeds 4 GiB per context"; return MIA_HIP_ERR_ARG; }
  }
  std::vector<uint8_t> packed((size_t)total + 8, 0);
  pack_reads(n, bases, offsets, roff.data(), len.data(), packed.data());
  ctx->max_len = max_len;
  ctx->min_len = max_len;
  ctx->h_len.assign(len.begin(), len.end());
  for (int64_t i = 0; i < n; i++) if ((int)len[(size_t)i] < ctx->min_len) ctx->min_len = len[(size_t)i];
  const int stride = (max_len + 3) & ~3;
  int nomem = 0;
  nomem |= dev_alloc(ctx, ctx->d_packed, packed.size());
  nomem |= dev_alloc(ctx, ctx->d_roff, n);
  nomem |= dev_alloc(ctx, ctx->d_len, n);
  nomem |= dev_alloc(ctx, ctx->d_rc, n);
  nomem |= dev_alloc(ctx, ctx->d_sk, n);
  nomem |= dev_alloc(ctx, ctx->d_as, n);
  nomem |= dev_alloc(ctx, ctx->d_ae, n);
  nomem |= dev_alloc(ctx, ctx->d_score, n);
  nomem |= dev_alloc(ctx, ctx->d_refstart, n);
  nomem |= dev_alloc(ctx, ctx->d_abr, n);
  nomem |= dev_alloc(ctx, ctx->d_status, n);
  nomem |= dev_alloc(ctx, ctx->d_cols, n * stride);
  nomem |= dev_alloc(ctx, ctx->d_bin_of, n);
  nomem |= dev_alloc(ctx, ctx->d_umax, n);
  ctx->rplane_words = (max_len + 63) >> 6;
  nomem |= dev_alloc(ctx, ctx->d_rplanes, n * 2 * ctx->rplane_words + 2);
  nomem |= dev_alloc(ctx, ctx->d_list, n + 4 * N_BINS);
  nomem |= dev_alloc(ctx, ctx->d_wide_list, n);
  nomem |= dev_alloc(ctx, ctx->d_retry_list, n);
  nomem |= dev_alloc(ctx, ctx->d_slot, n);
  nomem |= dev_alloc(ctx, ctx->d_partial, (size_t)(n / 256 + n / 4096 + 8));
  nomem |= dev_alloc(ctx, ctx->d_drop_f, n);
  nomem |= dev_alloc(ctx, ctx->d_drop_b, n);
  nomem |= dev_alloc(ctx, ctx->d_slot_dropped, 2 * n + 16);
  ctx->n_slots = ctx->d_slot_dropped.cap;
  nomem |= dev_alloc(ctx, ctx->d_back_slot, n) | dev_alloc(ctx, ctx->d_front_slot0, n);
  nomem |= dev_alloc(ctx, ctx->d_ri_flen, n) | dev_alloc(ctx, ctx->d_ri_blen, n) | dev_alloc(ctx, ctx->d_ri_actf, n) |
         dev_alloc(ctx, ctx->d_ri_trec, n * 16);
  const int64_t slot_cap = 2 * n + 16;
  nomem |= dev_alloc(ctx, ctx->d_si_reclen, slot_cap) | dev_alloc(ctx, ctx->d_si_recact, slot_cap) | dev_alloc(ctx, ctx->d_si_writer, slot_cap) |
         dev_alloc(ctx, ctx->d_si_mult, slot_cap);
  ctx->lk.cap = (int32_t)std::min<int64_t>(n + 16, (int64_t)1 << 20);
  if (ctx->lk.cap > (int32_t)LINK_NONE - 1) ctx->lk.cap = (int32_t)LINK_NONE - 1;
  nomem |= dev_alloc(ctx, ctx->d_lk_rec, (size_t)ctx->lk.cap * 4);
  ctx->ri.flen = ctx->d_ri_flen; ctx->ri.blen = ctx->d_ri_blen; ctx->ri.actf = ctx->d_ri_actf; ctx->ri.trec = ctx->d_ri_trec;
  ctx->si.reclen = ctx->d_si_reclen; ctx->si.recact = ctx->d_si_recact; ctx->si.writer = ctx->d_si_writer; ctx->si.mult = ctx->d_si_mult;
  ctx->lk.rec = ctx->d_lk_rec;
  if (nomem) return MIA_HIP_ERR_NOMEM;
  HIPCHK(hipMemcpyAsync(ctx->d_packed, packed.data(), packed.size(), hipMemcpyHostToDevice, ctx->stream));
  HIPCHK(hipMemcpyAsync(ctx->d_roff, roff.data(), (size_t)n * 4, hipMemcpyHostToDevice, ctx->stream));
  HIPCHK(hipMemcpyAsync(ctx->d_len, len.data(), (size_t)n * 2, hipMemcpyHostToDevice, ctx->stream));
  HIPCHK(hipMemcpyAsync(ctx->d_rc, rc, (size_t)n, hipMemcpyHostToDevice, ctx->stream));
  HIPCHK(hipMemcpyAsync(ctx->d_sk, strand_known, (size_t)n, hipMemcpyHostToDevice, ctx->stream));
  HIPCHK(hipMemcpyAsync(ctx->d_as, as, (size_t)n * 4, hipMemcpyHostToDevice, ctx->stream));
  HIPCHK(hipMemcpyAsync(ctx->d_ae, ae, (size_t)n * 4, hipMemcpyHostToDevice, ctx->stream));
  HIPCHK(hipMemsetAsync(ctx->d_score, 0, (size_t)n * 4, ctx->stream));
  HIPCHK(hipMemsetAsync(ctx->d_status, 0, (size_t)n * 4, ctx->stream));
  HIPCHK(hipMemsetAsync(ctx->d_abr, 0, (size_t)n * 2, ctx->stream));
  HIPCHK(hipMemsetAsync(ctx->d_slot_dropped, 0, (size_t)ctx->n_slots, ctx->stream));
  HIPCHK(hipMemsetAsync(ctx->d_back_slot, 0xFF, (size_t)n * 8, ctx->stream));
  HIPCHK(hipMemsetAsync(ctx->d_front_slot0, 0xFF, (size_t)n * 8, ctx->stream));
  HIPCHK(hipMemsetAsync(ctx->d_drop_f, 0, (size_t)n, ctx->stream));
  HIPCHK(hipMemsetAsync(ctx->d_drop_b, 0, (size_t)n, ctx->stream));
  HIPCHK(hipStreamSynchronize(ctx->stream));
  ReadSet& r = ctx->rs;
  r.n = n; r.packed = ctx->d_packed; r.roff = ctx->d_roff; r.len = ctx->d_len; r.rc = ctx->d_rc; r.sk = ctx->d_sk;
  r.as = ctx->d_as; r.ae = ctx->d_ae; r.score = ctx->d_score; r.refstart = ctx->d_refstart; r.abr = ctx->d_abr;
  r.status = ctx->d_status; r.cols = ctx->d_cols; r.stride = stride;
  ctx->d_order.release(); ctx->d_order2.release(); ctx->d_okey.release();
  ctx->umax_valid = false;
  if (n > 0) hipLaunchKernelGGL(k_read_planes, dim3((unsigned)((n + 255) / 256)), dim3(256), 0, ctx->stream, ctx->rs, ctx->rplane_words, ctx->d_rplanes);
  if (ctx->have_pssm && ctx->bx_ok && n > 0) {
    hipLaunchKernelGGL(k_bx_umax, dim3((unsigned)((n + 255) / 256)), dim3(256), 0, ctx->stream, ctx->rs, ctx->d_bx_mrow, ctx->d_umax);
    HIPCHK(hipGetLastError());
    ctx->umax_valid = true;
  }
  ctx->aligned = false;
  ctx->tallied = false;
  ctx->culled = false;
  return MIA_HIP_OK;
}

template <typename... KArgs, typename... Args>
static void launch_k(void (*kernel)(KArgs...), dim3 g, dim3 b, size_t shm, hipStream_t s, hipEvent_t stop, Args&&... args) {
  static_assert(sizeof...(KArgs) == sizeof...(Args), "every kernel argument, defaults included");
  if (stop) hipExtLaunchKernelGGL(kernel, g, b, (uint32_t)shm, s, nullptr, stop, 0, static_cast<KArgs>(args)...);
  else hipLaunchKernelGGL(kernel, g, b, shm, s, static_cast<KArgs>(args)...);
}

static int stage_begin(mia_hip_ctx* ctx, Stage st, hipStream_t on = nullptr) {
  if (!((ctx->stage_mask >> st) & 1u)) return 0;
  if (ctx->ev_free.empty()) {
    hipEvent_t x, y;
    if (hipEventCreate(&x) != hipSuccess || hipEventCreate(&y) != hipSuccess) return -1;
    ctx->ev_free.push_back({x, y});
  }
  auto p = ctx->ev_free.back();
  ctx->ev_free.pop_back();
  ctx->stg[st].pending.push_back(p);
  (void)hipEventRecord(p.first, on ? on : ctx->stream);
  return 0;
}
static void stage_end(mia_hip_ctx* ctx, Stage st, hipStream_t on = nullptr) {
  if (((ctx->stage_mask >> st) & 1u) && !ctx->stg[st].pending.empty()) (void)hipEventRecord(ctx->stg[st].pending.back().second, on ? on : ctx->stream);
}

template <typename... KArgs, typename... Args>
static int stage_launch(mia_hip_ctx* ctx, Stage st, void (*kernel)(KArgs...), dim3 g, dim3 b, size_t shm, hipStream_t s, Args&&... args) {
  static_assert(sizeof...(KArgs) == sizeof...(Args), "every kernel argument, defaults included");
  if (!((ctx->stage_mask >> st) & 1u)) {
    if (stage_begin(ctx, st, s)) return -1;
    hipLaunchKernelGGL(kernel, g, b, shm, s, static_cast<KArgs>(args)...);
    stage_end(ctx, st, s);
    return 0;
  }
  if (ctx->ev_free.empty()) {
    hipEvent_t x, y;
    if (hipEventCreate(&x) != hipSuccess || hipEventCreate(&y) != hipSuccess) return -1;
    ctx->ev_free.push_back({x, y});
  }
  auto p = ctx->ev_free.back();
  ctx->ev_free.pop_back();
  ctx->stg[st].pending.push_back(p);
  hipExtLaunchKernelGGL(kernel, g, b, (uint32_t)shm, s, p.first, p.second, 0, static_cast<KArgs>(args)...);
  return 0;
}

static void drain_events(mia_hip_ctx* ctx, int except = -1) {
  for (int k = 0; k < STG_COUNT; k++) {
    if (k == except) continue;
    auto& t = ctx->stg[k];
    for (auto& e : t.pending) {
      float ms = 0;
      if (hipEventSynchronize(e.second) == hipSuccess && hipEventElapsedTime(&ms, e.first, e.second) == hipSuccess) {
        t.ms += ms;
        t.launches++;
      }
      ctx->ev_free.push_back(e);
    }
    t.pending.clear();
  }
}

extern "C" int mia_hip_set_stage_mask(mia_hip_ctx* ctx, uint32_t mask) {
  if (!ctx) return MIA_HIP_ERR_ARG;
  HIPCHK(hipSetDevice(ctx->device));
  drain_events(ctx);
  ctx->stage_mask = mask;
  return MIA_HIP_OK;
}

extern "C" int mia_hip_stage_stats(mia_hip_ctx* ctx, int reset, int32_t cap, const char** names, double* ms, int64_t* launches, int32_t* n_stages) {
  if (!ctx) return MIA_HIP_ERR_ARG;
  HIPCHK(hipSetDevice(ctx->device));
  drain_events(ctx);
  if (n_stages) *n_stages = STG_COUNT;
  for (int k = 0; k < STG_COUNT && k < cap; k++) {
    if (names) names[k] = STAGE_NAMES[k];
    if (ms) ms[k] = ctx->stg[k].ms;
    if (launches) launches[k] = ctx->stg[k].launches;
  }
  if (reset) for (auto& t : ctx->stg) { t.ms = 0; t.launches = 0; }
  return MIA_HIP_OK;
}

extern "C" int mia_hip_kernel_time(mia_hip_ctx* ctx, int reset, double* align_ms, int64_t* launches) {
  if (!ctx) return MIA_HIP_ERR_ARG;
  HIPCHK(hipSetDevice(ctx->device));
  drain_events(ctx);
  if (align_ms) *align_ms = ctx->stg[STG_TRACE].ms;
  if (launches) *launches = ctx->stg[STG_TRACE].launches;
  if (reset) { ctx->stg[STG_TRACE].ms = 0; ctx->stg[STG_TRACE].launches = 0; }
  return MIA_HIP_OK;
}

extern "C" int mia_hip_filter_stats(mia_hip_ctx* ctx, int reset, int64_t* reads_seen, int64_t* reads_finished, double* kernel_ms, int64_t* launches) {
  if (!ctx) return MIA_HIP_ERR_ARG;
  HIPCHK(hipSetDevice(ctx->device));
  drain_events(ctx);
  if (reads_seen) *reads_seen = ctx->filter_seen;
  if (reads_finished) *reads_finished = ctx->filter_proven;
  if (kernel_ms) *kernel_ms = ctx->stg[STG_FILTER].ms;
  if (launches) *launches = ctx->stg[STG_FILTER].launches;
  if (reset) { ctx->filter_seen = 0; ctx->filter_proven = 0; ctx->stg[STG_FILTER].ms = 0; ctx->stg[STG_FILTER].launches = 0; }
  return MIA_HIP_OK;
}

extern "C" int mia_hip_band_stats(mia_hip_ctx* ctx, int reset, int64_t* reads_finished, double* kernel_ms, int64_t* launches) {
  if (!ctx) return MIA_HIP_ERR_ARG;
  HIPCHK(hipSetDevice(ctx->device));
  drain_events(ctx);
  if (reads_finished) *reads_finished = ctx->band_done;
  if (kernel_ms) *kernel_ms = ctx->stg[STG_BAND].ms;
  if (launches) *launches = ctx->stg[STG_BAND].launches;
  if (reset) { ctx->band_done = 0; ctx->stg[STG_BAND].ms = 0; ctx->stg[STG_BAND].launches = 0; }
  return MIA_HIP_OK;
}

extern "C" int mia_hip_bx_stats(mia_hip_ctx* ctx, int reset, int64_t* reads4, double* kernel_ms3, int64_t* launches) {
  if (!ctx) return MIA_HIP_ERR_ARG;
  HIPCHK(hipSetDevice(ctx->device));
  drain_events(ctx);
  if (reads4) { reads4[0] = ctx->bx_seen; reads4[1] = ctx->bx_done[0]; reads4[2] = ctx->bx_done[1]; reads4[3] = ctx->bx_done[2]; }
  if (kernel_ms3) for (int k = 0; k < 3; k++) kernel_ms3[k] = ctx->stg[STG_BX_PLAN + k].ms;
  if (launches) *launches = ctx->bx_launches;
  if (reset) { ctx->bx_seen = 0; for (int k = 0; k < 3; k++) { ctx->bx_done[k] = 0; ctx->stg[STG_BX_PLAN + k].ms = 0; ctx->stg[STG_BX_PLAN + k].launches = 0; } ctx->bx_launches = 0; }
  return MIA_HIP_OK;
}

#ifdef MIA_HIP_ALT_PATHS
extern "C" int mia_hip_debug_tally_kinds(mia_hip_ctx* ctx, uint64_t* out8) {
  if (!ctx || !out8) return MIA_HIP_ERR_ARG;
  HIPCHK(hipStreamSynchronize(ctx->stream));
  HIPCHK(hipMemcpyFromSymbol(out8, HIP_SYMBOL(g_tally_kinds), 8 * sizeof(uint64_t)));
// ... 656 lines not shown
  int run2 = 0;
  for (int b = 0; b < N_BINS; b++) { h.h_off2[b] = run2; run2 += b >= BIN_QUAD0 ? ((h.h_count2[b] + 3) & ~3) : 0; }
  ctx->plain_total += (int64_t)h.n_quads * 4;
  for (int b = BIN_QUAD0; b < N_BINS; b++) ctx->plain_retried += h.h_count2[b];
  h.n_quads = run2 / 4;
  h.quad_begin = 0;
  if (h.n_quads > 0) {
    HIPCHK(hipMemsetAsync(ctx->d_list, 0xFF, (size_t)run2 * 4, ctx->stream));
    HIPCHK(hipMemcpyAsync(c.d_off, h.h_off2, (size_t)N_BINS * 4, hipMemcpyHostToDevice, ctx->stream));
    hipLaunchKernelGGL(k_plan_fill, dim3(c.gb), dim3(256), 0, ctx->stream, n, ctx->d_bin_of, c.d_off, c.d_cursor, ctx->d_list);
  }
  return MIA_HIP_OK;
}

static int align_planner_host_trace(mia_hip_ctx* ctx, AlignCall& c, HostPlan& h) {
  const int64_t slab = (int64_t)Q_G * MAX_READ * Q_TRACE_STRIDE;
  const int grid = h.n_quads < ctx->quad_wgs ? h.n_quads : ctx->quad_wgs;
  if (!ctx->d_quad_slabs && dev_alloc(ctx, ctx->d_quad_slabs, slab * ctx->quad_wgs)) return MIA_HIP_ERR_NOMEM;
  const size_t quad_lds = (size_t)Q_G * q_sub_bytes(ctx->max_len) + 16;
  if (stage_begin(ctx, STG_TRACE)) return MIA_HIP_ERR_NOMEM;
  hipLaunchKernelGGL(k_align_quad, dim3(grid), dim3(64), quad_lds, ctx->stream, ctx->rs, c.ref, ctx->d_pssm, ctx->packs.p[0], ctx->d_list + h.quad_begin,
                     h.n_quads, ctx->d_quad_slabs, slab, ctx->d_wide_list, c.d_wide_count, ctx->d_retry_list, c.d_wide_count + 1, 1,
                     ctx->dbg, (const int32_t*)nullptr);
  stage_end(ctx, STG_TRACE);
  HIPCHK(hipGetLastError());
  HIPCHK(hipMemcpyAsync(&h.h_misc[2], c.d_wide_count, 8, hipMemcpyDeviceToHost, ctx->stream));
  HIPCHK(hipStreamSynchronize(ctx->stream));
  const int32_t n_retry = h.h_misc[3];
  if (n_retry > 0) {
    hipError_t e = launch_window_class(ctx, 0, ctx->d_retry_list, n_retry);
    if (e != hipSuccess) { ctx->err = std::string("k_align_window retry launch: ") + hipGetErrorString(e); return MIA_HIP_ERR_DEVICE; }
  } else {
    h.wide_known = true;
  }
  return MIA_HIP_OK;
}

static int align_planner_host(mia_hip_ctx* ctx, AlignCall& c) {
  const AlignRoute& r = c.r;
  HostPlan h;
  if (int rc = align_planner_host_fill(ctx, c, h)) return rc;
  if ((h.n_quads > 0 || r.filtered) && r.use_plain) { if (int rc = align_planner_host_plain(ctx, c, h)) return rc; }
  if (h.n_quads > 0) { if (int rc = align_planner_host_trace(ctx, c, h)) return rc; }
  if (c.pending_join) { if (int rcj = bx_join_and_retry(ctx, c)) return rcj; h.wide_known = false; }
  if (!h.wide_known) {
    HIPCHK(hipMemcpyAsync(&h.h_misc[2], c.d_wide_count, 4, hipMemcpyDeviceToHost, ctx->stream));
    if (h.bx_counters_later) HIPCHK(hipMemcpyAsync(h.h_bxc, ctx->d_bx_ctr, BXC_WORDS * 4, hipMemcpyDeviceToHost, ctx->stream));
    HIPCHK(hipStreamSynchronize(ctx->stream));
    if (h.bx_counters_later) host_take_bx_counters(ctx, h);
  }
  const int32_t n_wide = h.h_misc[2];
  if (n_wide > 0) { if (int rcw = run_wide(ctx, c.ref, n_wide)) return rcw; }
  return align_close(ctx);
}

static int align_all(mia_hip_ctx* ctx) {
  const int64_t n = ctx->rs.n;
  if (!ctx->spec_ok) { ctx->spec_pending = false; ctx->abort_if = nullptr; }
  ctx->align_end_signalled = false;
  ctx->buckets_queued = 0;
  if (n == 0) { ctx->aligned = true; return MIA_HIP_OK; }
  AlignCall c;
  c.r = align_route(align_route_in(ctx));
  const AlignRoute& r = c.r;
  ctx->last_route_bx = r.bx;
  c.ref = RefInfo{ctx->d_ref, ctx->L, ctx->wrap, ctx->explicit_win};
  c.d_count = ctx->d_bins; c.d_off = ctx->d_bins + N_BINS; c.d_cursor = ctx->d_bins + 2 * N_BINS; c.d_wide_count = ctx->d_bins + 3 * N_BINS;
  c.gb = (int)((n + (int64_t)256 * PLAN_PER - 1) / ((int64_t)256 * PLAN_PER));
  c.dbg_steps = ctx->deferred && alt_env("MIA_HIP_ITER_DEBUG") != nullptr;
  if (int rc = align_ensure_buffers(ctx, c)) return rc;
  if (int rc = align_ref_prep(ctx, c)) return rc;
  if (r.bx) {
    align_bx_dev(ctx, c);
    if (int rc = align_plan_launches(ctx, c)) return rc;
    if (r.three_streams) { if (int rc = align_band_dps(ctx, c)) return rc; }
    else if (r.two_streams) { if (int rc = align_band_dps_serial(ctx, c)) return rc; }
    ctx->bx_launches++;
  } else if (r.filtered) {
    if (int rc = align_round1(ctx, c)) return rc;
  }
  c.ps = r.planner_aside ? ctx->stream2 : ctx->stream;
  if (r.plan_count_late)
    hipLaunchKernelGGL(k_plan_count, dim3(c.gb), dim3(256), 0, c.ps, ctx->rs, c.ref, ctx->packs, 1, (int)r.filtered, (int)(r.filtered && r.use_plain), ctx->d_bin_of,
                       c.d_count, ctx->d_filter_n);
  if (!ctx->deferred) return align_planner_host(ctx, c);
  if (int rc = align_planner_deferred(ctx, c)) return rc;
  return align_finish_deferred(ctx, c);
}

extern "C" int mia_hip_align_windows(mia_hip_ctx* ctx, const char* ref, int64_t ref_len, const int64_t* win_start, const int32_t* win_len) {
  if (!ctx || !ref || !win_start || !win_len || ref_len <= 0) return MIA_HIP_ERR_ARG;
  if (!ctx->have_pssm || !ctx->d_packed) { ctx->err = "set_pssm and upload_reads must precede align_windows"; return MIA_HIP_ERR_STATE; }
  if (ref_len > INT32_MAX - 128) { ctx->err = "align_windows: the reference string must stay below 2^31 characters"; return MIA_HIP_ERR_ARG; }
  HIPCHK(hipSetDevice(ctx->device));
  const int64_t n = ctx->rs.n;
  std::vector<int32_t> as((size_t)n), ae((size_t)n);
  for (int64_t i = 0; i < n; i++) {
    if (win_len[i] <= 0 || win_start[i] < 0 || win_start[i] + win_len[i] > ref_len) {
      ctx->err = "align_windows: window " + std::to_string(i) + " is empty or leaves the reference string";
      return MIA_HIP_ERR_ARG;
    }
    as[(size_t)i] = (int32_t)win_start[i];
    ae[(size_t)i] = (int32_t)(win_start[i] + win_len[i] - 1);
  }
  std::vector<uint8_t> codes((size_t)ref_len + 64, 4);
  for (int64_t i = 0; i < ref_len; i++) codes[(size_t)i] = base_code(ref[i]);
  if (dev_ensure(ctx, ctx->d_ref, (int64_t)codes.size())) return MIA_HIP_ERR_NOMEM;
  HIPCHK(hipMemcpyAsync(ctx->d_ref, codes.data(), codes.size(), hipMemcpyHostToDevice, ctx->stream));
  if (n) {
    HIPCHK(hipMemcpyAsync(ctx->d_as, as.data(), (size_t)n * 4, hipMemcpyHostToDevice, ctx->stream));
    HIPCHK(hipMemcpyAsync(ctx->d_ae, ae.data(), (size_t)n * 4, hipMemcpyHostToDevice, ctx->stream));
  }
  ctx->L = (int)ref_len; ctx->wrap = (int)ref_len; ctx->have_ref = false; ctx->explicit_win = 1; ctx->ref_mostly_bases = true; ctx->kh_entries = 0;
  const int rcode = align_all(ctx);
  HIPCHK(hipStreamSynchronize(ctx->stream));
  return rcode;
}

extern "C" int mia_hip_get_alignments(mia_hip_ctx* ctx, int32_t* score, int32_t* as, int32_t* ae) {
  if (!ctx) return MIA_HIP_ERR_ARG;
  if (!ctx->aligned) { ctx->err = "realign first"; return MIA_HIP_ERR_STATE; }
  HIPCHK(hipSetDevice(ctx->device));
  const size_t n = (size_t)ctx->rs.n;
  if (score) HIPCHK(hipMemcpyAsync(score, ctx->d_score, n * 4, hipMemcpyDeviceToHost, ctx->stream));
  if (as) HIPCHK(hipMemcpyAsync(as, ctx->d_as, n * 4, hipMemcpyDeviceToHost, ctx->stream));
  if (ae) HIPCHK(hipMemcpyAsync(ae, ctx->d_ae, n * 4, hipMemcpyDeviceToHost, ctx->stream));
  HIPCHK(hipStreamSynchronize(ctx->stream));
  return MIA_HIP_OK;
}

extern "C" int mia_hip_get_scripts(mia_hip_ctx* ctx, int16_t* cols, int32_t stride, int32_t* ref_start) {
  if (!ctx || (cols && stride < ctx->max_len)) return MIA_HIP_ERR_ARG;
  if (!ctx->aligned) { ctx->err = "realign first"; return MIA_HIP_ERR_STATE; }
  HIPCHK(hipSetDevice(ctx->device));
  const size_t n = (size_t)ctx->rs.n;
  if (cols) {
    if (ctx->diag_scripts_missing && n > 0) {
      hipLaunchKernelGGL(k_diag_scripts, dim3((unsigned)((n + 255) / 256)), dim3(256), 0, ctx->stream, ctx->rs);
      HIPCHK(hipGetLastError());
      ctx->diag_scripts_missing = false;
    }
    HIPCHK(hipMemcpy2DAsync(cols, (size_t)stride * 2, ctx->d_cols, (size_t)ctx->rs.stride * 2, (size_t)ctx->max_len * 2, n,
                            hipMemcpyDeviceToHost, ctx->stream));
  }
  if (ref_start) HIPCHK(hipMemcpyAsync(ref_start, ctx->d_refstart, n * 4, hipMemcpyDeviceToHost, ctx->stream));
  HIPCHK(hipStreamSynchronize(ctx->stream));
  return MIA_HIP_OK;
}

static int finish_params(mia_hip_ctx* ctx);
static int finish_cull(mia_hip_ctx* ctx) {
  const int64_t nl = ctx->links_cap_all;
  if (dev_ensure(ctx, ctx->d_link_len, nl, nl + 64) || dev_ensure(ctx, ctx->d_link_act, nl, nl + 64)) return MIA_HIP_ERR_NOMEM;
  hipLaunchKernelGGL(k_links_apply, dim3(32), dim3(256), 0, ctx->stream, ctx->d_links_all, ctx->d_n_links_all, (int32_t)ctx->links_cap_all, ctx->si,
                     ctx->d_slot_dropped, ctx->n_slots, ctx->d_link_len, ctx->d_link_act, ctx->d_cull_flags, ctx->abort_if);
  ctx->links_applied = true;
  return finish_params(ctx);
}

static int finish_params(mia_hip_ctx* ctx) {
  const int64_t n = ctx->rs.n;
  hipLaunchKernelGGL(k_rec_params, dim3((int)((n + 255) / 256)), dim3(256), 0, ctx->stream, ctx->rs, ctx->L, ctx->d_slot, ctx->d_slot_dropped,
                     ctx->n_slots, ctx->d_back_slot, ctx->ri, ctx->si, ctx->d_links_all, ctx->d_link_len, ctx->d_link_act, ctx->d_n_links_all,
                     (int32_t)ctx->links_cap_all, ctx->read_base, ctx->d_drop_f, ctx->d_drop_b, ctx->d_cull_flags, ctx->abort_if,
                     (ctx->umax_valid && ctx->rs.roff == ctx->d_roff && ctx->d_rplanes && ctx->d_umax) ? ctx->d_umax : (const int32_t*)nullptr,
                     (ctx->cull_with_records && ctx->d_n_links_all == ctx->lk.n) ? 1 : 0);
  HIPCHK(hipGetLastError());
  return MIA_HIP_OK;
}

static int check_cull_flags(mia_hip_ctx* ctx, uint32_t fl) {
  if (fl & 8u) { ctx->err = "more formerly split reads than the link list holds"; return MIA_HIP_ERR_RANGE; }
  if (fl & 4u) {
    ctx->err = "a formerly split read points at an AlnSeq slot that holds no record of this iteration (the reference would show "
               "the slot's content from an earlier iteration); not reproduced";
    return MIA_HIP_ERR_RANGE;
  }
  return MIA_HIP_OK;
}

extern "C" int mia_hip_cull(mia_hip_ctx* ctx, int32_t hard_cut, double slope, double intercept, int64_t slot_base) {
  if (!ctx) return MIA_HIP_ERR_ARG;
  if (!ctx->aligned) { ctx->err = "realign first"; return MIA_HIP_ERR_STATE; }
  if (ctx->explicit_win) { ctx->err = "the last alignment ran on caller-supplied windows (align_windows): realign first"; return MIA_HIP_ERR_STATE; }
  HIPCHK(hipSetDevice(ctx->device));
  const int64_t n = ctx->rs.n;
  if (n == 0) return MIA_HIP_OK;
  const int nb = (int)((n + 255) / 256);
  if (!ctx->d_cull_sync) {
    if (dev_alloc(ctx, ctx->d_cull_sync, 4)) return MIA_HIP_ERR_NOMEM;
    HIPCHK(hipMemsetAsync(ctx->d_cull_sync, 0, 16, ctx->stream));
  }
  hipLaunchKernelGGL(k_slot_count, dim3((unsigned)((n + 4095) / 4096)), dim3(256), 0, ctx->stream, ctx->rs, ctx->L, ctx->d_partial, nb, slot_base, ctx->d_total, (uint32_t*)nullptr, ctx->abort_if);
  if (ctx->cull_scan) hipLaunchKernelGGL(k_scan_partials, dim3(1), dim3(256), 0, ctx->stream, ctx->d_partial, nb, slot_base, ctx->d_total, ctx->abort_if);
  if (slot_base + 2 * n + 16 > ctx->n_slots) {
    DevBuf<uint8_t> nd;
    const int64_t ns = slot_base + 2 * n + 16;
    if (dev_alloc(ctx, nd, ns)) return MIA_HIP_ERR_NOMEM;
    HIPCHK(hipMemsetAsync(nd, 0, (size_t)ns, ctx->stream));
    HIPCHK(hipMemcpyAsync(nd, ctx->d_slot_dropped, (size_t)ctx->n_slots, hipMemcpyDeviceToDevice, ctx->stream));
    HIPCHK(hipStreamSynchronize(ctx->stream));
    ctx->d_slot_dropped = std::move(nd);
    ctx->n_slots = ns;
  }
  ctx->slot_base = slot_base;
  ctx->si.base = slot_base;
  ctx->si.n_local_p = ctx->d_total;
  if (!ctx->in_iterate) HIPCHK(hipMemsetAsync(ctx->lk.n, 0, 8, ctx->stream));
  hipLaunchKernelGGL(k_cull_records, dim3((unsigned)nb), dim3(256), 0, ctx->stream, ctx->rs, ctx->L, (const int64_t*)ctx->d_partial, ctx->d_slot, ctx->ri, ctx->si,
                     ctx->read_base, ctx->d_cull_flags, ctx->d_slot_dropped, ctx->n_slots, hard_cut, slope, intercept, ctx->d_back_slot,
                     (const int64_t*)ctx->d_front_slot0, ctx->lk, ctx->dev_cut, ctx->abort_if, ctx->cull_scan ? 0 : nb, slot_base, ctx->d_total,
                     ctx->cull_with_records ? 1 : 0, ctx->d_drop_f, ctx->d_drop_b,
                     (ctx->umax_valid && ctx->rs.roff == ctx->d_roff && ctx->d_rplanes && ctx->d_umax) ? ctx->d_umax : (const int32_t*)nullptr);
  HIPCHK(hipGetLastError());
  ctx->d_links_all = ctx->lk.rec;
  ctx->d_n_links_all = ctx->lk.n;
  ctx->links_cap_all = ctx->lk.cap;
  ctx->culled = true;
  ctx->links_applied = false;
  return finish_cull(ctx);
}

extern "C" int mia_hip_set_back_slots(mia_hip_ctx* ctx, const int64_t* back_slot) {
  if (ctx) ctx->pre_cull_valid = false;
  if (!ctx || !back_slot) return MIA_HIP_ERR_ARG;
  if (!ctx->d_back_slot) { ctx->err = "upload_reads first"; return MIA_HIP_ERR_STATE; }
  HIPCHK(hipSetDevice(ctx->device));
  HIPCHK(hipMemcpyAsync(ctx->d_back_slot, back_slot, (size_t)ctx->rs.n * 8, hipMemcpyHostToDevice, ctx->stream));
  HIPCHK(hipStreamSynchronize(ctx->stream));
  return MIA_HIP_OK;
}

extern "C" int mia_hip_set_pass1_state(mia_hip_ctx* ctx, const int64_t* front_slot, const int64_t* back_slot, const int32_t* score) {
  if (ctx) ctx->pre_cull_valid = false;
  if (!ctx) return MIA_HIP_ERR_ARG;
  if (!ctx->d_back_slot) { ctx->err = "upload_reads first"; return MIA_HIP_ERR_STATE; }
  HIPCHK(hipSetDevice(ctx->device));
  const size_t n = (size_t)ctx->rs.n;
  if (front_slot) HIPCHK(hipMemcpyAsync(ctx->d_front_slot0, front_slot, n * 8, hipMemcpyHostToDevice, ctx->stream));
  if (back_slot) HIPCHK(hipMemcpyAsync(ctx->d_back_slot, back_slot, n * 8, hipMemcpyHostToDevice, ctx->stream));
  if (score) HIPCHK(hipMemcpyAsync(ctx->d_score, score, n * 4, hipMemcpyHostToDevice, ctx->stream));
  HIPCHK(hipStreamSynchronize(ctx->stream));
  return MIA_HIP_OK;
}

extern "C" int mia_hip_set_read_base(mia_hip_ctx* ctx, int64_t read_base) {
  if (!ctx || read_base < 0) return MIA_HIP_ERR_ARG;
  ctx->read_base = read_base;
  return MIA_HIP_OK;
}

extern "C" int mia_hip_links(mia_hip_ctx* ctx, int64_t** d_links, int64_t* n_links) {
  if (!ctx || !ctx->culled) return MIA_HIP_ERR_STATE;
  int32_t nl = 0;
  HIPCHK(hipSetDevice(ctx->device));
  HIPCHK(hipMemcpyAsync(&nl, ctx->lk.n, 4, hipMemcpyDeviceToHost, ctx->stream));
  HIPCHK(hipStreamSynchronize(ctx->stream));
  if (d_links) *d_links = ctx->lk.rec;
  if (n_links) *n_links = nl;
  return MIA_HIP_OK;
}

extern "C" int mia_hip_set_links(mia_hip_ctx* ctx, const int64_t* d_links_all, int64_t n_all) {
  if (!ctx || n_all < 0 || (n_all > 0 && !d_links_all)) return MIA_HIP_ERR_ARG;
  if (!ctx->culled) { ctx->err = "cull first"; return MIA_HIP_ERR_STATE; }
  if (n_all >= (int64_t)LINK_NONE) { ctx->err = "too many links"; return MIA_HIP_ERR_RANGE; }
  HIPCHK(hipSetDevice(ctx->device));
  if (n_all * 4 > (ctx->owned_links.empty() ? 0 : ctx->owned_links.back().cap)) {
    DevBuf<int64_t> nb;
    if (dev_alloc(ctx, nb, (n_all + 64) * 4)) return MIA_HIP_ERR_NOMEM;
    ctx->owned_links.push_back(std::move(nb));
  }
  if (!ctx->owned_links.empty()) ctx->d_links_all = ctx->owned_links.back();
  if (n_all > 0) HIPCHK(hipMemcpyAsync(ctx->d_links_all, d_links_all, (size_t)n_all * 32, hipMemcpyDeviceToDevice, ctx->stream));
  ctx->n_links_all = (int32_t)n_all;
  if (!ctx->d_n_links_gathered && dev_alloc(ctx, ctx->d_n_links_gathered, 1)) return MIA_HIP_ERR_NOMEM;
  const int32_t n32 = (int32_t)n_all;
  HIPCHK(hipMemcpyAsync(ctx->d_n_links_gathered, &n32, 4, hipMemcpyHostToDevice, ctx->stream));
  ctx->d_n_links_all = ctx->d_n_links_gathered;
  ctx->links_cap_all = n_all;
  const int64_t n = ctx->rs.n;
  HIPCHK(hipMemsetAsync(ctx->d_cull_flags, 0, 4, ctx->stream));
  hipLaunchKernelGGL(k_rec_geom, dim3((unsigned)((n + 255) / 256)), dim3(256), 0, ctx->stream, ctx->rs, ctx->L, ctx->d_slot, ctx->ri, ctx->si,
                     ctx->read_base, ctx->d_cull_flags);
  HIPCHK(hipGetLastError());
  const int rc_fc = finish_cull(ctx);
  HIPCHK(hipStreamSynchronize(ctx->stream));
  return rc_fc;
}

extern "C" int mia_hip_link_lengths(mia_hip_ctx* ctx, int32_t** d_len, int32_t** d_act, int64_t* n) {
  if (!ctx || !ctx->links_applied) return MIA_HIP_ERR_STATE;
  HIPCHK(hipSetDevice(ctx->device));
  HIPCHK(hipStreamSynchronize(ctx->stream));
  if (d_len) *d_len = ctx->d_link_len;
  if (d_act) *d_act = ctx->d_link_act;
  if (n) *n = ctx->n_links_all;
  return MIA_HIP_OK;
}

extern "C" int mia_hip_finish_links(mia_hip_ctx* ctx) {
  if (!ctx || !ctx->links_applied) return MIA_HIP_ERR_STATE;
  HIPCHK(hipSetDevice(ctx->device));
  HIPCHK(hipMemsetAsync(ctx->d_cull_flags, 0, 4, ctx->stream));
  return finish_params(ctx);
}

extern "C" int mia_hip_get_record_params(mia_hip_ctx* ctx, int32_t* params, int64_t* back_slot) {
  if (!ctx) return MIA_HIP_ERR_ARG;
  if (!ctx->culled) { ctx->err = "cull first"; return MIA_HIP_ERR_STATE; }
  HIPCHK(hipSetDevice(ctx->device));
  const size_t n = (size_t)ctx->rs.n;
  if (params) HIPCHK(hipMemcpy2DAsync(params, 32, ctx->ri.trec + TREC_PARAMS, 64, 32, n, hipMemcpyDeviceToHost, ctx->stream));
  if (back_slot) HIPCHK(hipMemcpyAsync(back_slot, ctx->d_back_slot, n * 8, hipMemcpyDeviceToHost, ctx->stream));
  HIPCHK(hipStreamSynchronize(ctx->stream));
  return MIA_HIP_OK;
}

extern "C" int mia_hip_get_dropped(mia_hip_ctx* ctx, uint8_t* front, uint8_t* back) {
  if (!ctx) return MIA_HIP_ERR_ARG;
  HIPCHK(hipSetDevice(ctx->device));
  const size_t n = (size_t)ctx->rs.n;
  if (front) HIPCHK(hipMemcpyAsync(front, ctx->d_drop_f, n, hipMemcpyDeviceToHost, ctx->stream));
  if (back) HIPCHK(hipMemcpyAsync(back, ctx->d_drop_b, n, hipMemcpyDeviceToHost, ctx->stream));
  uint32_t cflags = 0;
  if (ctx->culled) HIPCHK(hipMemcpyAsync(&cflags, ctx->d_cull_flags, 4, hipMemcpyDeviceToHost, ctx->stream));
  HIPCHK(hipStreamSynchronize(ctx->stream));
  return check_cull_flags(ctx, cflags);
}

extern "C" int mia_hip_set_slot_dropped(mia_hip_ctx* ctx, const uint8_t* flags, int64_t n_flags) {
  if (!ctx || !flags || n_flags < 0) return MIA_HIP_ERR_ARG;
  if (!ctx->d_slot_dropped) { ctx->err = "upload_reads first"; return MIA_HIP_ERR_STATE; }
  HIPCHK(hipSetDevice(ctx->device));
  if (n_flags > ctx->n_slots) {
    const int rca = dev_alloc(ctx, ctx->d_slot_dropped, n_flags + 16);
    ctx->n_slots = ctx->d_slot_dropped.cap;
    if (rca) return rca;
  }
  HIPCHK(hipMemsetAsync(ctx->d_slot_dropped, 0, (size_t)ctx->n_slots, ctx->stream));
  HIPCHK(hipMemcpyAsync(ctx->d_slot_dropped, flags, (size_t)n_flags, hipMemcpyHostToDevice, ctx->stream));
  HIPCHK(hipStreamSynchronize(ctx->stream));
  return MIA_HIP_OK;
}

extern "C" void mia_hip_score_cut(const int32_t* score, const int32_t* seq_len, const uint8_t* unique_best, int64_t n,
                                  double* slope, double* intercept) {
  int64_t sx = 0, sy = 0, j = 0;
  int32_t lmin = INT32_MAX, lmax = INT32_MIN;
  for (int64_t i = 0; i < n; i++) {
    const bool u = (!unique_best || unique_best[i]) && score[i] >= 2000;
    sx += u ? seq_len[i] : 0;
    sy += u ? score[i] : 0;
    j += u;
    if (u) { lmin = seq_len[i] < lmin ? seq_len[i] : lmin; lmax = seq_len[i] > lmax ? seq_len[i] : lmax; }
  }
  double xbar = (double)sx, ybar = (double)sy;
  xbar /= (double)(size_t)j;
  ybar /= (double)(size_t)j;
  double slope_bf, intercept_bf, max_delta = 0;
  if (j > 0 && lmin == lmax) {
    const double zero = 0.0;
    slope_bf = zero / zero;
    intercept_bf = ybar - slope_bf * xbar;
  } else {
    double ssxy = 0, ssxx = 0;
    auto used = [&](int64_t i) { return (!unique_best || unique_best[i]) && score[i] >= 2000; };
    for (int64_t i = 0; i < n; i++) if (used(i)) {
      ssxy += (seq_len[i] - xbar) * (score[i] - ybar);
      ssxx += (seq_len[i] - xbar) * (seq_len[i] - xbar);
    }
    slope_bf = ssxy / ssxx;
    intercept_bf = ybar - slope_bf * xbar;
    double m4[4] = {0, 0, 0, 0};
    for (int64_t i = 0; i < n; i++) if (used(i)) {
      double d = (score[i] - ((slope_bf * seq_len[i]) + intercept_bf)) / seq_len[i];
      if (d > m4[i & 3]) m4[i & 3] = d;
    }
    for (int k = 0; k < 4; k++) if (m4[k] > max_delta) max_delta = m4[k];
  }
  *intercept = intercept_bf;
  if ((slope_bf - max_delta) > 0) *slope = slope_bf - (max_delta * 2.0);
  else *slope = (double)(slope_bf * (80 / 100.0));
}

extern "C" int mia_hip_score_sums(mia_hip_ctx* ctx, int64_t* sums5) {
  if (!ctx || !sums5) return MIA_HIP_ERR_ARG;
  if (!ctx->aligned) { ctx->err = "realign first"; return MIA_HIP_ERR_STATE; }
  HIPCHK(hipSetDevice(ctx->device));
  if (!ctx->d_sums && dev_alloc(ctx, ctx->d_sums, 8)) return MIA_HIP_ERR_NOMEM;
  ctx->pre_cull_valid = false;
  hipLaunchKernelGGL(k_score_sums_init, dim3(1), dim3(64), 0, ctx->stream, ctx->d_sums, (const int32_t*)nullptr);
  const int64_t n = ctx->rs.n;
  if (n > 0) {
    int grid = (int)std::min<int64_t>((n + 255) / 256, (int64_t)ctx->cus);
    hipLaunchKernelGGL(k_score_sums, dim3(grid), dim3(256), 0, ctx->stream, ctx->rs, ctx->d_sums, ctx->L, ctx->d_back_slot, ctx->d_front_slot0);
    HIPCHK(hipGetLastError());
  }
  int64_t local7[7];
  int64_t* stage = ctx->h_pin ? reinterpret_cast<int64_t*>(ctx->h_pin + (16 << 10)) : local7;
  HIPCHK(hipMemcpyAsync(stage, ctx->d_sums, 56, hipMemcpyDeviceToHost, ctx->stream));
  HIPCHK(hipStreamSynchronize(ctx->stream));
  memcpy(sums5, stage, 40);
  ctx->pre_cull_records = stage[5];
  ctx->pre_cull_links = stage[6];
  ctx->pre_cull_valid = true;
  return MIA_HIP_OK;
}

extern "C" int mia_hip_pre_cull_counts(mia_hip_ctx* ctx, int64_t* n_records, int64_t* n_links) {
  if (!ctx) return MIA_HIP_ERR_ARG;
  if (!ctx->pre_cull_valid) { ctx->err = "score_sums (after the last realign) first"; return MIA_HIP_ERR_STATE; }
  if (n_records) *n_records = ctx->pre_cull_records;
  if (n_links) *n_links = ctx->pre_cull_links;
  return MIA_HIP_OK;
}

extern "C" int mia_hip_score_cut_from_sums(const int64_t* sums5, double* slope, double* intercept) {
  const int64_t sx = sums5[0], sy = sums5[1], j = sums5[2];
  if (!(j > 0 && sums5[3] == sums5[4])) return 1;
  double xbar = (double)sx, ybar = (double)sy;
  xbar /= (double)(size_t)j;
  ybar /= (double)(size_t)j;
  const double zero = 0.0;
  const double slope_bf = zero / zero;
  const double intercept_bf = ybar - slope_bf * xbar;
  const double max_delta = 0;
  *intercept = intercept_bf;
  if ((slope_bf - max_delta) > 0) *slope = slope_bf - (max_delta * 2.0);
  else *slope = (double)(slope_bf * (80 / 100.0));
  return 0;
}

extern "C" int mia_hip_num_records(mia_hip_ctx* ctx, int64_t* n_records) {
  if (!ctx || !n_records) return MIA_HIP_ERR_ARG;
  if (!ctx->aligned) { ctx->err = "realign first"; return MIA_HIP_ERR_STATE; }
  HIPCHK(hipSetDevice(ctx->device));
  const int64_t n = ctx->rs.n;
  *n_records = 0;
  if (n == 0) return MIA_HIP_OK;
  const int nb = (int)((n + 4095) / 4096);
  hipLaunchKernelGGL(k_scan_blocks, dim3(nb), dim3(256), 0, ctx->stream, ctx->rs, ctx->L, ctx->d_partial);
  hipLaunchKernelGGL(k_scan_partials, dim3(1), dim3(256), 0, ctx->stream, ctx->d_partial, nb, (int64_t)0, ctx->d_total);
  HIPCHK(hipMemcpyAsync(n_records, ctx->d_total, 8, hipMemcpyDeviceToHost, ctx->stream));
  HIPCHK(hipStreamSynchronize(ctx->stream));
  return MIA_HIP_OK;
}

static int ensure_events(mia_hip_ctx* ctx, int64_t elems) {
  const int rc = dev_alloc(ctx, ctx->d_tb_events, elems);
  ctx->tb.events = ctx->d_tb_events;
  ctx->tb.cap_events = (int32_t)std::min<int64_t>(ctx->d_tb_events.cap, INT32_MAX);
  return rc;
}

// ... 283 lines not shown
```

Before: 1.493 billion reads/s.

## Fuse link application into cull kernel and add lean cull path inside iterate

New measurement: 1.525 billion reads/s, median of 6. +2.2%, better.

```diff
diff --git a/include/mia_hip.h b/include/mia_hip.h
--- a/include/mia_hip.h
+++ b/include/mia_hip.h
@@ -66,6 +66,7 @@
 int mia_hip_set_links(mia_hip_ctx *ctx, const int64_t *d_links_all, int64_t n_all);
 int mia_hip_link_lengths(mia_hip_ctx *ctx, int32_t **d_len, int32_t **d_act, int64_t *n);
 int mia_hip_finish_links(mia_hip_ctx *ctx);
+int mia_hip_cull_stats(mia_hip_ctx *ctx, int64_t *links_before, int32_t *lean);
 
 void mia_hip_score_cut(const int32_t *score, const int32_t *seq_len, const uint8_t *unique_best, int64_t n,
                        double *slope, double *intercept);
diff --git a/mapping-iterative-assembler_amd/__init__.py b/mapping-iterative-assembler_amd/__init__.py
--- a/mapping-iterative-assembler_amd/__init__.py
+++ b/mapping-iterative-assembler_amd/__init__.py
@@ -76,6 +76,8 @@
     lib.mia_hip_set_links.argtypes = [vp, vp, C.c_int64]
     lib.mia_hip_link_lengths.argtypes = [vp, P(vp), P(vp), P(C.c_int64)]
     lib.mia_hip_finish_links.argtypes = [vp]
+    if hasattr(lib, "mia_hip_cull_stats"):
+        lib.mia_hip_cull_stats.argtypes = [vp, P(C.c_int64), P(C.c_int32)]
     lib.mia_hip_plain_stats.argtypes = [vp, C.c_int, P(C.c_double), P(C.c_int64), P(C.c_int64), P(C.c_int64)]
     lib.mia_hip_score_sums.argtypes = [vp, vp]
     lib.mia_hip_score_cut_from_sums.argtypes = [vp, P(C.c_double), P(C.c_double)]
@@ -155,7 +157,7 @@
             "mia_hip_tally", "mia_hip_tally_buffers", "mia_hip_ins_events", "mia_hip_set_ins_events",
             "mia_hip_get_tally", "mia_hip_consensus", "mia_hip_myers", "mia_hip_myers_packed", "mia_hip_myers_align", "mia_hip_filter_stats", "mia_hip_band_stats", "mia_hip_bx_stats", "mia_hip_bx_counters", "mia_hip_kernel_time", "mia_hip_pass1_time", "mia_hip_myers_time", "mia_hip_pass1_filtered", "mia_hip_pass1_anchored", "mia_hip_pre_cull_counts", "mia_hip_ma_tally", "mia_hip_get_ins_tally", "mia_hip_ma_region", "mia_hip_get_ma_region", "mia_hip_ma_ace", "mia_hip_get_ma_ace", "mia_hip_ma_sam", "mia_hip_get_ma_sam", "mia_hip_ma_profile", "mia_hip_get_ma_profile", "mia_hip_ma_ends", "mia_hip_get_ma_ends", "mia_hip_ma_cols", "mia_hip_get_ma_cols", "mia_hip_ma_dedup", "mia_hip_get_ma_dedup", "mia_hip_ma_damage", "mia_hip_get_ma_damage", "mia_hip_ma_mask", "mia_hip_get_ma_mask", "mia_hip_trim", "mia_hip_trim_stats", "mia_hip_trim_rerun_stats", "mia_hip_set_back_slots", "mia_hip_set_pass1_state",
             "mia_hip_get_record_params", "mia_hip_set_read_base", "mia_hip_links", "mia_hip_set_links", "mia_hip_link_lengths",
-            "mia_hip_finish_links", "mia_hip_plain_stats", "mia_hip_score_sums",
+            "mia_hip_finish_links", "mia_hip_cull_stats", "mia_hip_plain_stats", "mia_hip_score_sums",
             "mia_hip_score_cut_from_sums", "mia_hip_stage_stats", "mia_hip_measure_peaks", "mia_hip_measure_issue", "mia_hip_set_tally", "mia_hip_iterate", "mia_hip_set_stage_mask", "mia_hip_comm_unique_id", "mia_hip_comm_init", "mia_hip_comm_destroy",
             "mia_hip_comm_attach", "mia_hip_comm_info", "mia_hip_loopback_create", "mia_hip_loopback_table", "mia_hip_loopback_destroy"]
 
@@ -769,6 +771,11 @@
     def finish_links(self):
         self._chk(self._l.mia_hip_finish_links(self._h))
 
+    def cull_stats(self):
+        n, lean = C.c_int64(), C.c_int32()
+        self._chk(self._l.mia_hip_cull_stats(self._h, C.byref(n), C.byref(lean)))
+        return n.value, bool(lean.value)
+
     def plain_stats(self, reset=False):
         ms, a, b, c = C.c_double(), C.c_int64(), C.c_int64(), C.c_int64()
         self._chk(self._l.mia_hip_plain_stats(self._h, 1 if reset else 0, C.byref(ms), C.byref(a), C.byref(b), C.byref(c)))
diff --git a/mapping-iterative-assembler_amd/csrc/cull_body.h b/mapping-iterative-assembler_amd/csrc/cull_body.h
--- /dev/null
+++ b/mapping-iterative-assembler_amd/csrc/cull_body.h
@@ -0,0 +1,60 @@
+#pragma once
+#include <stdint.h>
+
+#ifndef MIA_HD
+#if defined(__HIPCC__)
+#define MIA_HD __host__ __device__
+#else
+#define MIA_HD
+#endif
+#endif
+
+namespace mia {
+
+struct RecGeom {
+  int start_w, end, split, ncols_f, ncols_b;
+};
+MIA_HD inline RecGeom rec_geom(int as, int ae, int L) {
+  RecGeom g;
+  g.start_w = as;
+  g.end = ae > L ? ae - L : ae;
+  g.split = as > g.end;
+  g.ncols_f = g.split ? (L - as) : (g.end - as + 1);
+  g.ncols_b = g.split ? g.end + 1 : 0;
+  return g;
+}
+
+MIA_HD inline int cull_records(bool sk, int as, int ae, int L) { return sk ? (rec_geom(as, ae, L).split ? 2 : 1) : 0; }
+
+MIA_HD inline int cull_link_mark(int64_t back_slot, int64_t front_slot0) { return (back_slot >= 0 ? 1 : 0) | (front_slot0 >= 0 ? 2 : 0); }
+MIA_HD inline int cull_links_marked(bool sk, bool split, int mark) {
+  if (!sk) return (mark & 1) + ((mark >> 1) & 1);
+  return (!split && (mark & 1)) ? 1 : 0;
+}
+MIA_HD inline int cull_links(bool sk, bool split, int64_t back_slot, int64_t front_slot0) {
+  return cull_links_marked(sk, split, cull_link_mark(back_slot, front_slot0));
+}
+
+MIA_HD inline int cull_groups(int nb) { return (nb + 15) >> 4; }
+MIA_HD inline int64_t cull_partial_words(int64_t n) { const int64_t nb = (n + 255) / 256; return nb + 2 * ((nb + 15) / 16) + 8; }
+
+struct CullShare {
+  int64_t pre, tot, links;
+};
+MIA_HD inline CullShare cull_share(const int64_t* partial, int nb, int block, int t, int threads) {
+  const int ng = cull_groups(nb), myg = block >> 4;
+  CullShare s = {0, 0, 0};
+  if (t < 16) {
+    const int b = myg * 16 + t;
+    if (b < block) s.pre = partial[b];
+  }
+  for (int g = t; g < ng; g += threads) {
+    const int64_t v = partial[nb + g];
+    s.tot += v;
+    if (g < myg) s.pre += v;
+    s.links += partial[nb + ng + g];
+  }
+  return s;
+}
+
+}
diff --git a/mapping-iterative-assembler_amd/csrc/mia_consensus_kernels.h b/mapping-iterative-assembler_amd/csrc/mia_consensus_kernels.h
--- a/mapping-iterative-assembler_amd/csrc/mia_consensus_kernels.h
+++ b/mapping-iterative-assembler_amd/csrc/mia_consensus_kernels.h
@@ -2,6 +2,7 @@
 #include <hip/hip_runtime.h>
 #include <stdint.h>
 
+#include "cull_body.h"
 #include "ma_records.h"
 #include "mia_kernels.h"
 #include "mia_layout.h"
@@ -18,18 +19,6 @@
   uint32_t* flags;
 };
 
-struct RecGeom {
-  int start_w, end, split, ncols_f, ncols_b;
-};
-MIA_HD inline RecGeom rec_geom(int as, int ae, int L) {
-  RecGeom g;
-  g.start_w = as;
-  g.end = ae > L ? ae - L : ae;
-  g.split = as > g.end;
-  g.ncols_f = g.split ? (L - as) : (g.end - as + 1);
-  g.ncols_b = g.split ? g.end + 1 : 0;
-  return g;
-}
 
 __global__ void k_scan_blocks(ReadSet rs, int32_t L, int64_t* partial) {
   __shared__ int32_t sh[256];
@@ -157,15 +146,17 @@
   t4[3] = make_int4(p[4], p[5], p[6], p[7]);
 }
 
-__device__ __forceinline__ void rec_make(const ReadSet& rs, int64_t i, uint8_t* drop_front, uint8_t* drop_back, uint8_t df, uint8_t db, const int32_t* p,
-                                         uint32_t st, int32_t actf, const int32_t* umax, int4* r4) {
-  drop_front[i] = df;
-  drop_back[i] = db;
-  const int fl = (rs.rc[i] ? TRF_RC : 0) | (df ? TRF_DF : 0) | (db ? TRF_DB : 0) | ((st & ST_DIAG) ? TRF_DIAG : 0) |
-                 ((st & ST_TOO_LONG) ? TRF_TOO_LONG : 0) | (rs.sk[i] ? TRF_SK : 0) | ((st & ST_ONEGAP) ? TRF_ONEGAP : 0) |
-                 ((umax && umax[i] >= 0) ? TRF_NO_N : 0);
-  r4[0] = make_int4(rs.as[i], rs.ae[i], (int32_t)((uint32_t)rs.len[i] | ((uint32_t)(uint16_t)rs.abr[i] << 16)), fl);
-  r4[1] = make_int4(rs.refstart[i], (int32_t)rs.roff[i], actf, (int32_t)(st >> 8));
+struct RecVals {
+  int32_t as, ae, len, abr, refstart;
+  uint32_t roff;
+  bool rc, sk, no_n;
+};
+__device__ __forceinline__ void rec_make(const RecVals& v, uint8_t df, uint8_t db, const int32_t* p, uint32_t st, int32_t actf, int4* r4) {
+  const int fl = (v.rc ? TRF_RC : 0) | (df ? TRF_DF : 0) | (db ? TRF_DB : 0) | ((st & ST_DIAG) ? TRF_DIAG : 0) |
+                 ((st & ST_TOO_LONG) ? TRF_TOO_LONG : 0) | (v.sk ? TRF_SK : 0) | ((st & ST_ONEGAP) ? TRF_ONEGAP : 0) |
+                 (v.no_n ? TRF_NO_N : 0);
+  r4[0] = make_int4(v.as, v.ae, (int32_t)((uint32_t)v.len | ((uint32_t)(uint16_t)v.abr << 16)), fl);
+  r4[1] = make_int4(v.refstart, (int32_t)v.roff, actf, (int32_t)(st >> 8));
   r4[2] = make_int4(p[0], p[1], p[2], p[3]);
   r4[3] = make_int4(p[4], p[5], p[6], p[7]);
 }
@@ -198,16 +189,22 @@
   int32_t cap;
 };
 
+__device__ __forceinline__ void rec_store_val(int64_t i, const RecGeom& g, int nf, int nb, int af, int bases, int64_t slot_i, const RecInfo& ri,
+                                              const SlotInfo& si, int64_t read_base, uint32_t* flags, int64_t n_local, bool lean) {
+  const int flen = g.ncols_f + nf, blen = g.split ? g.ncols_b + nb : 0;
+  if (!lean) { ri.flen[i] = flen; ri.blen[i] = blen; ri.actf[i] = af + nf; }
+  const int64_t ls = slot_i - si.base;
+  if (ls >= 0 && ls + (g.split ? 1 : 0) < n_local) {
+    if (!lean) {
+      const unsigned long long me = ((unsigned long long)(read_base + i) << 20) | LINK_NONE;
+      si.reclen[ls] = flen; si.recact[ls] = af + nf; si.mult[ls] = 1; si.writer[ls] = me;
+      if (g.split) { si.reclen[ls + 1] = blen; si.recact[ls + 1] = bases - (af + nf); si.mult[ls + 1] = 1; si.writer[ls + 1] = me; }
+    }
+  } else atomicOr(flags, 4u);
+}
 __device__ __forceinline__ void rec_store_at(int64_t i, const RecGeom& g, int nf, int nb, int af, int bases, int64_t slot_i, RecInfo& ri,
                                              SlotInfo& si, int64_t read_base, uint32_t* flags) {
-  const int flen = g.ncols_f + nf, blen = g.split ? g.ncols_b + nb : 0;
-  ri.flen[i] = flen; ri.blen[i] = blen; ri.actf[i] = af + nf;
-  const int64_t ls = slot_i - si.base;
-  if (ls >= 0 && ls + (g.split ? 1 : 0) < (*si.n_local_p)) {
-    const unsigned long long me = ((unsigned long long)(read_base + i) << 20) | LINK_NONE;
-    si.reclen[ls] = flen; si.recact[ls] = af + nf; si.mult[ls] = 1; si.writer[ls] = me;
-    if (g.split) { si.reclen[ls + 1] = blen; si.recact[ls + 1] = bases - (af + nf); si.mult[ls + 1] = 1; si.writer[ls + 1] = me; }
-  } else atomicOr(flags, 4u);
+  rec_store_val(i, g, nf, nb, af, bases, slot_i, ri, si, read_base, flags, *si.n_local_p, false);
 }
 __device__ __forceinline__ void rec_store(int64_t i, const RecGeom& g, int nf, int nb, int af, int bases, const int64_t* slot, RecInfo& ri,
                                           SlotInfo& si, int64_t read_base, uint32_t* flags) {
@@ -288,28 +285,42 @@
   }
 }
 
-__global__ __launch_bounds__(256) void k_slot_count(ReadSet rs, int32_t L, int64_t* partial, int nb, int64_t base, int64_t* total, uint32_t* blocks_done, const int32_t* abort_if = nullptr) {
+__global__ void k_link_marks(int64_t n, const int64_t* back_slot, const int64_t* front_slot0, uint8_t* link_mark) {
+  const int64_t i = (int64_t)blockIdx.x * blockDim.x + threadIdx.x;
+  if (i < n) link_mark[i] = (uint8_t)cull_link_mark(back_slot[i], front_slot0[i]);
+}
+
+__global__ __launch_bounds__(256) void k_slot_count(ReadSet rs, int32_t L, int64_t* partial, int nb, int64_t base, int64_t* total, uint32_t* blocks_done, const int32_t* abort_if = nullptr,
+                                                      const uint8_t* __restrict__ link_mark = nullptr) {
   if (abort_if && *abort_if != 0) return;
   __shared__ bool last;
   __shared__ int64_t s_run[256];
-  __shared__ int32_t wsum[16][4];
+  __shared__ int32_t wsum[16][4], lsum[4];
   const int64_t base_read = (int64_t)blockIdx.x * 4096;
-  uint8_t sk16[16];
+  uint8_t sk16[16], mk16[16];
   int32_t as16[16], ae16[16];
 #pragma unroll
   for (int k = 0; k < 16; k++) {
     const int64_t i = base_read + k * 256 + threadIdx.x;
     const bool in = i < rs.n;
-    sk16[k] = in ? rs.sk[i] : (uint8_t)0;
+    sk16[k] = in ? rs.sk[i] : (uint8_t)1;
     as16[k] = in ? rs.as[i] : 0;
     ae16[k] = in ? rs.ae[i] : 0;
-  }
+    mk16[k] = (in && link_mark) ? link_mark[i] : (uint8_t)0;
+  }
+  int my_links = 0;
 #pragma unroll
   for (int k = 0; k < 16; k++) {
-    const int cnt = sk16[k] ? (rec_geom(as16[k], ae16[k], L).split ? 2 : 1) : 0;
+    const int64_t i = base_read + k * 256 + threadIdx.x;
+    const bool in = i < rs.n;
+    const int cnt = in ? cull_records(sk16[k] != 0, as16[k], ae16[k], L) : 0;
     const int w = __popcll(__ballot(cnt >= 1)) + __popcll(__ballot(cnt == 2));
     if ((threadIdx.x & 63) == 0) wsum[k][threadIdx.x >> 6] = w;
-  }
+    my_links += cull_links_marked(sk16[k] != 0, cnt == 2, mk16[k]);
+  }
+#pragma unroll
+  for (int o = 32; o; o >>= 1) my_links += __shfl_xor(my_links, o);
+  if ((threadIdx.x & 63) == 0) lsum[threadIdx.x >> 6] = my_links;
   __syncthreads();
   if (threadIdx.x < 16 && blockIdx.x * 16 + (int)threadIdx.x < nb)
     partial[blockIdx.x * 16 + threadIdx.x] = (int64_t)wsum[threadIdx.x][0] + wsum[threadIdx.x][1] + wsum[threadIdx.x][2] + wsum[threadIdx.x][3];
@@ -318,6 +329,7 @@
       int64_t g = 0;
       for (int k = 0; k < 16; k++) g += (int64_t)wsum[k][0] + wsum[k][1] + wsum[k][2] + wsum[k][3];
       partial[nb + blockIdx.x] = g;
+      partial[nb + cull_groups(nb) + blockIdx.x] = (int64_t)lsum[0] + lsum[1] + lsum[2] + lsum[3];
     }
     return;
   }
@@ -344,59 +356,72 @@
   if (t == 0) *blocks_done = 0;
 }
 
-__global__ __launch_bounds__(256) void k_cull_records(ReadSet rs, int32_t L, const int64_t* partial, int64_t* slot, RecInfo ri, SlotInfo si, int64_t read_base,
-                                                        uint32_t* flags, uint8_t* slot_dropped, int64_t n_slots, int32_t hard_cut, double slope, double intercept,
-                                                        int64_t* back_slot, const int64_t* front_slot0, Links lk, const double* dev_cut, const int32_t* abort_if = nullptr,
+__global__ __launch_bounds__(256) void k_cull_records(ReadSet rs, int32_t L, const int64_t* __restrict__ partial, int64_t* __restrict__ slot, RecInfo ri, SlotInfo si,
+                                                        int64_t read_base, uint32_t* flags, uint8_t* __restrict__ slot_dropped, int64_t n_slots, int32_t hard_cut,
+                                                        double slope, double intercept, int64_t* __restrict__ back_slot, const int64_t* __restrict__ front_slot0, Links lk,
+                                                        const double* __restrict__ dev_cut, const int32_t* abort_if = nullptr,
                                                         int32_t raw_nb = 0, int64_t slot_base = 0, int64_t* total_out = nullptr,
-                                                        int32_t with_records = 0, uint8_t* drop_front = nullptr, uint8_t* drop_back = nullptr, const int32_t* umax = nullptr) {
+                                                        int32_t with_records = 0, uint8_t* __restrict__ drop_front = nullptr, uint8_t* __restrict__ drop_back = nullptr,
+                                                        const int32_t* __restrict__ umax = nullptr, int32_t lean_ok = 0, int32_t* __restrict__ stats = nullptr,
+                                                        uint32_t* apply_ticket = nullptr, int32_t* link_len = nullptr, int32_t* link_act = nullptr,
+                                                        uint8_t* __restrict__ link_mark = nullptr) {
   if (abort_if && *abort_if != 0) return;
   __shared__ int32_t wsum[4];
-  __shared__ int64_t s_red[2][4], s_first, s_total;
+  __shared__ int64_t s_red[3][4];
   const int lane = threadIdx.x & 63, wv = threadIdx.x >> 6;
-  if (raw_nb) {
-    const int ng = (raw_nb + 15) >> 4, myg = (int)(blockIdx.x >> 4);
-    int64_t pre = 0, tot = 0;
-    for (int g = threadIdx.x; g < ng; g += 256) { const int64_t v = partial[raw_nb + g]; tot += v; if (g < myg) pre += v; }
-    if (threadIdx.x < 16) { const int b = myg * 16 + (int)threadIdx.x; if (b < (int)blockIdx.x) pre += partial[b]; }
-#pragma unroll
-    for (int o = 32; o; o >>= 1) { pre += __shfl_xor(pre, o); tot += __shfl_xor(tot, o); }
-    if (lane == 0) { s_red[0][wv] = pre; s_red[1][wv] = tot; }
-    __syncthreads();
-    if (threadIdx.x == 0) {
-      s_first = slot_base + s_red[0][0] + s_red[0][1] + s_red[0][2] + s_red[0][3];
-      s_total = s_red[1][0] + s_red[1][1] + s_red[1][2] + s_red[1][3];
-      if (blockIdx.x == 0 && total_out) *total_out = s_total;
-    }
-    si.n_local_p = &s_total;
-  }
   const int64_t i0 = (int64_t)blockIdx.x * 256 + (threadIdx.x & ~63);
   const int64_t me = i0 + lane;
   const bool in = me < rs.n;
-  const bool sk = in && rs.sk[me];
-  int as_me = 0, ae_me = 0;
-  if (sk) { as_me = rs.as[me]; ae_me = rs.ae[me]; }
-  const RecGeom g_me = rec_geom(as_me, ae_me, L);
+  const int64_t ix = in ? me : rs.n - 1;
+  RecVals v;
+  v.sk = rs.sk[ix] != 0; v.rc = rs.rc[ix] != 0;
+  v.as = rs.as[ix]; v.ae = rs.ae[ix]; v.len = rs.len[ix]; v.abr = rs.abr[ix]; v.refstart = rs.refstart[ix]; v.roff = rs.roff[ix];
+  const int32_t score_me = rs.score[ix];
+  uint32_t my_st = rs.status[ix];
+  const int mark_me = link_mark[ix];
+  const int32_t umax_me = (umax ? umax : (const int32_t*)rs.as)[ix];
+  if (dev_cut) { slope = dev_cut[0]; intercept = dev_cut[1]; }
+  int64_t first = 0, n_local = 0, n_links = -1;
+  if (raw_nb) {
+    CullShare sh = cull_share(partial, raw_nb, (int)blockIdx.x, (int)threadIdx.x, 256);
+#pragma unroll
+    for (int o = 32; o; o >>= 1) { sh.pre += __shfl_xor(sh.pre, o); sh.tot += __shfl_xor(sh.tot, o); sh.links += __shfl_xor(sh.links, o); }
+    if (lane == 0) { s_red[0][wv] = sh.pre; s_red[1][wv] = sh.tot; s_red[2][wv] = sh.links; }
+  } else {
+    first = partial[blockIdx.x];
+    n_local = *si.n_local_p;
+  }
+  const bool sk = in && v.sk;
+  const RecGeom g_me = rec_geom(sk ? v.as : 0, sk ? v.ae : 0, L);
   const int cnt = sk ? (g_me.split ? 2 : 1) : 0;
   const unsigned long long m1 = __ballot(cnt >= 1), m2 = __ballot(cnt == 2), below = (1ull << lane) - 1ull;
   if (lane == 0) wsum[wv] = __popcll(m1) + __popcll(m2);
   __syncthreads();
-  int64_t my_slot = (raw_nb ? s_first : partial[blockIdx.x]) + __popcll(m1 & below) + __popcll(m2 & below);
+  if (raw_nb) {
+    first = slot_base + s_red[0][0] + s_red[0][1] + s_red[0][2] + s_red[0][3];
+    n_local = s_red[1][0] + s_red[1][1] + s_red[1][2] + s_red[1][3];
+    n_links = s_red[2][0] + s_red[2][1] + s_red[2][2] + s_red[2][3];
+    if (blockIdx.x == 0 && threadIdx.x == 0 && total_out) *total_out = n_local;
+  }
+  v.no_n = umax && umax_me >= 0;
+  const bool lean = lean_ok && raw_nb && with_records && n_links == 0;
+  if (blockIdx.x == 0 && threadIdx.x == 0 && stats) { stats[0] = (int32_t)(n_links < INT32_MAX ? n_links : INT32_MAX); stats[1] = lean ? 1 : 0; }
+  int64_t my_slot = first + __popcll(m1 & below) + __popcll(m2 & below);
   for (int k = 0; k < wv; k++) my_slot += wsum[k];
-  if (in) slot[me] = my_slot;
+  if (in && !lean) slot[me] = my_slot;
   int my_flen = 0, my_actf = 0, my_blen = 0;
-  uint32_t my_st = in ? rs.status[me] : 0u;
   bool walk = false;
   if (in) {
-    if (!sk) { ri.flen[me] = 0; ri.blen[me] = 0; ri.actf[me] = 0; }
-    else if (rs.status[me] & ST_DIAG) {
-      const int len2 = rs.len[me], abr = rs.abr[me];
+    if (!sk) { if (!lean) { ri.flen[me] = 0; ri.blen[me] = 0; ri.actf[me] = 0; } }
+    else if (my_st & ST_DIAG) {
+      const int len2 = v.len, abr = v.abr;
       const int af = (len2 - abr) < g_me.ncols_f ? (len2 - abr) : g_me.ncols_f;
-      rec_store_at(me, g_me, 0, 0, af, len2 - abr, my_slot, ri, si, read_base, flags);
+      rec_store_val(me, g_me, 0, 0, af, len2 - abr, my_slot, ri, si, read_base, flags, n_local, lean);
       my_flen = g_me.ncols_f; my_actf = af; my_blen = g_me.split ? g_me.ncols_b : 0;
-    } else if ((rs.status[me] & ST_ONEGAP) && !g_me.split) {
-      const uint32_t desc = rs.status[me] >> 8;
-      const int len2 = rs.len[me], abr = rs.abr[me], gn = (int)((desc >> 10) & 63u), ins = (int)(desc & 1u);
-      rec_store_at(me, g_me, ins ? gn : 0, 0, len2 - abr - (ins ? gn : 0), len2 - abr, my_slot, ri, si, read_base, flags);
+    } else if ((my_st & ST_ONEGAP) && !g_me.split) {
+      const uint32_t desc = my_st >> 8;
+      const int len2 = v.len, abr = v.abr, gn = (int)((desc >> 10) & 63u), ins = (int)(desc & 1u);
+      rec_store_val(me, g_me, ins ? gn : 0, 0, len2 - abr - (ins ? gn : 0), len2 - abr, my_slot, ri, si, read_base, flags, n_local, lean);
       my_flen = g_me.ncols_f + (ins ? gn : 0); my_actf = len2 - abr;
     } else walk = true;
   }
@@ -450,15 +475,14 @@
       const uint32_t want = one ? (ST_ONEGAP | (((uint32_t)ev_kind | ((uint32_t)ev_row << 1) | ((uint32_t)gn << 10)) << 8)) : ST_OK;
       if (st_new != want) { if (lane == 0) rs.status[i] = want; st_new = want; }
     }
-    if (lane == 0) rec_store_at(i, g, nf, nb, af, len2 - abr, slot_i, ri, si, read_base, flags);
+    if (lane == 0) rec_store_val(i, g, nf, nb, af, len2 - abr, slot_i, ri, si, read_base, flags, n_local, lean);
     if (lane == li) { my_flen = g.ncols_f + nf; my_actf = af + nf; my_blen = g.split ? g.ncols_b + nb : 0; my_st = st_new; }
   }
   __shared__ int4 s_rec[4][256];
   int4 r4[4] = {make_int4(0, 0, 0, 0), make_int4(0, 0, 0, 0), make_int4(0, 0, 0, 0), make_int4(0, 0, 0, 0)};
   if (in) {
-  if (dev_cut) { slope = dev_cut[0]; intercept = dev_cut[1]; }
-  const double min_score = hard_cut > 0 ? (double)hard_cut : (double)(intercept + (slope * (double)rs.len[me]));
-  const bool low = (double)rs.score[me] < min_score;
+  const double min_score = hard_cut > 0 ? (double)hard_cut : (double)(intercept + (slope * (double)v.len));
+  const bool low = (double)score_me < min_score;
   auto add_link = [&](int64_t target, int kind, int fl, int ac) {
     const int e = atomicAdd(lk.n, 1);
     if (e < lk.cap) {
@@ -470,9 +494,11 @@
   };
   int32_t p[8] = {0, 0, 0, 0, 0, 0, 0, 0};
   if (!sk) {
-    if (front_slot0[me] >= 0) add_link(front_slot0[me], 1, 0, 0);
-    if (back_slot[me] >= 0) add_link(back_slot[me], 2, 0, 0);
-    if (with_records) rec_make(rs, me, drop_front, drop_back, 0, 0, p, my_st, 0, umax, r4);
+    if (!lean) {
+      if (mark_me & 2) add_link(front_slot0[me], 1, 0, 0);
+      if (mark_me & 1) add_link(back_slot[me], 2, 0, 0);
+    }
+    if (with_records) { drop_front[me] = 0; drop_back[me] = 0; rec_make(v, 0, 0, p, my_st, 0, r4); }
   } else {
   uint8_t df = 0, db = 0;
   if (with_records && my_slot < n_slots) df = low ? (uint8_t)1 : slot_dropped[my_slot];
@@ -481,21 +507,48 @@
   if (g_me.split) {
     if (low && my_slot + 1 < n_slots) slot_dropped[my_slot + 1] = 1;
     back_slot[me] = my_slot + 1;
-  } else if (back_slot[me] >= 0) add_link(back_slot[me], 0, my_flen, my_actf);
+    if (!(mark_me & 1)) link_mark[me] = (uint8_t)(mark_me | 1);
+  } else if (mark_me & 1) add_link(back_slot[me], 0, my_flen, my_actf);
   if (with_records) {
-    const int64_t ls = my_slot - si.base, n_local = *si.n_local_p;
+    const int64_t ls = my_slot - si.base;
     if (ls >= 0 && ls < n_local) { p[2] = my_flen + my_blen; p[3] = 1; }
     if (g_me.split && ls + 1 < n_local) { p[4] = my_flen; p[5] = my_actf; p[6] = my_flen + my_blen; p[7] = 1; }
-    rec_make(rs, me, drop_front, drop_back, df, db, p, my_st, my_actf, umax, r4);
+    drop_front[me] = df; drop_back[me] = db;
+    rec_make(v, df, db, p, my_st, my_actf, r4);
   }
   }
   }
   if (with_records) rec_store_wave(ri.trec, i0, rs.n, r4, lane, s_rec[wv]);
+  if (apply_ticket && !lean) {
+    __shared__ bool s_last;
+    __threadfence();
+    __syncthreads();
+    if (threadIdx.x == 0) s_last = atomicAdd(apply_ticket, 1u) == gridDim.x - 1u;
+    __syncthreads();
+    if (s_last) {
+      __threadfence();
+      const int n_apply = min(__hip_atomic_load(lk.n, __ATOMIC_RELAXED, __HIP_MEMORY_SCOPE_AGENT), lk.cap);
+      for (int e = threadIdx.x; e < n_apply; e += 256) {
+        const int64_t* r = lk.rec + (int64_t)e * 4;
+        const int64_t reader = __builtin_nontemporal_load(r), target = __builtin_nontemporal_load(r + 1), low_kind = __builtin_nontemporal_load(r + 3);
+        const int64_t ls = target - si.base;
+        link_len[e] = -1;
+        link_act[e] = -1;
+        if (ls < 0 || ls >= n_local) continue;
+        atomicMax(&si.writer[ls], ((unsigned long long)reader << 20) | (unsigned long long)e);
+        atomicAdd(&si.mult[ls], 1);
+        if ((low_kind & 1) && target < n_slots) slot_dropped[target] = 1;
+        link_len[e] = __builtin_nontemporal_load(si.reclen + ls);
+        link_act[e] = __builtin_nontemporal_load(si.recact + ls);
+      }
+      if (threadIdx.x == 0) *apply_ticket = 0;
+    }
+  }
 }
 
 __global__ void k_cull_mark(ReadSet rs, int32_t L, const int64_t* slot, uint8_t* slot_dropped, int64_t n_slots, int32_t hard_cut, double slope,
                             double intercept, int64_t* back_slot, const int64_t* front_slot0, RecInfo ri, Links lk, int64_t read_base,
-                            uint32_t* flags, const double* dev_cut) {
+                            uint32_t* flags, const double* dev_cut, uint8_t* link_mark = nullptr) {
   int64_t i = (int64_t)blockIdx.x * blockDim.x + threadIdx.x;
   if (i >= rs.n) return;
   if (dev_cut) { slope = dev_cut[0]; intercept = dev_cut[1]; }
@@ -521,6 +574,7 @@
   if (split) {
     if (low && s + 1 < n_slots) slot_dropped[s + 1] = 1;
     back_slot[i] = s + 1;
+    if (link_mark) link_mark[i] |= 1;
   } else if (back_slot[i] >= 0) add_link(back_slot[i], 0, ri.flen[i], ri.actf[i]);
 }
 
diff --git a/mapping-iterative-assembler_amd/csrc/mia_hip.hip b/mapping-iterative-assembler_amd/csrc/mia_hip.hip
--- a/mapping-iterative-assembler_amd/csrc/mia_hip.hip
+++ b/mapping-iterative-assembler_amd/csrc/mia_hip.hip
@@ -176,6 +176,7 @@
   DevBuf<uint8_t> d_slot_dropped, d_drop_f, d_drop_b; int64_t n_slots = 0;
   DevBuf<int64_t> d_back_slot;
   DevBuf<int64_t> d_front_slot0;
+  DevBuf<uint8_t> d_link_mark;
   DevBuf<int32_t> d_link_act;
   RecInfo ri{};
   DevBuf<int32_t> d_ri_flen, d_ri_blen, d_ri_actf, d_ri_trec;
@@ -195,6 +196,11 @@
   std::vector<DevBuf<int64_t>> owned_links;
   bool cull_scan = false, tail_scans = false;
   bool cull_with_records = true;
+  bool no_cull_lean = false;
+  bool no_cull_apply = false;
+  bool cull_applied = false;
+  bool cull_lean_ok = false;
+  DevBuf<int32_t> d_cull_stats;
   int64_t pre_cull_records = 0, pre_cull_links = 0; bool pre_cull_valid = false;
 
   TallyBuf tb{}; DevBuf<int32_t> d_tb_tally, d_ins_off, d_ins_total; DevBuf<uint64_t> d_tb_events;
@@ -311,6 +317,8 @@
   if (on("MIA_HIP_CULL_SCAN")) ctx->cull_scan = true;
   if (on("MIA_HIP_TAIL_SCANS")) ctx->tail_scans = true;
   if (on("MIA_HIP_NO_CULL_RECORDS")) ctx->cull_with_records = false;
+  if (on("MIA_HIP_NO_CULL_LEAN")) ctx->no_cull_lean = true;
+  if (on("MIA_HIP_NO_CULL_APPLY")) ctx->no_cull_apply = true;
   if (on("MIA_HIP_NO_BINNED_TALLY")) ctx->use_binned_tally = 0;
   if (on("MIA_HIP_NO_LINEAR_TALLY")) ctx->no_linear_tally = true;
   if (on("MIA_HIP_SORT2_UNPACKED")) ctx->sort2_unpacked = true;
@@ -570,12 +578,12 @@
   nomem |= dev_alloc(ctx, ctx->d_wide_list, n);
   nomem |= dev_alloc(ctx, ctx->d_retry_list, n);
   nomem |= dev_alloc(ctx, ctx->d_slot, n);
-  nomem |= dev_alloc(ctx, ctx->d_partial, (size_t)(n / 256 + n / 4096 + 8));
+  nomem |= dev_alloc(ctx, ctx->d_partial, (size_t)cull_partial_words(n));
   nomem |= dev_alloc(ctx, ctx->d_drop_f, n);
   nomem |= dev_alloc(ctx, ctx->d_drop_b, n);
   nomem |= dev_alloc(ctx, ctx->d_slot_dropped, 2 * n + 16);
   ctx->n_slots = ctx->d_slot_dropped.cap;
-  nomem |= dev_alloc(ctx, ctx->d_back_slot, n) | dev_alloc(ctx, ctx->d_front_slot0, n);
+  nomem |= dev_alloc(ctx, ctx->d_back_slot, n) | dev_alloc(ctx, ctx->d_front_slot0, n) | dev_alloc(ctx, ctx->d_link_mark, n);
   nomem |= dev_alloc(ctx, ctx->d_ri_flen, n) | dev_alloc(ctx, ctx->d_ri_blen, n) | dev_alloc(ctx, ctx->d_ri_actf, n) |
          dev_alloc(ctx, ctx->d_ri_trec, n * 16);
   const int64_t slot_cap = 2 * n + 16;
@@ -601,6 +609,7 @@
   HIPCHK(hipMemsetAsync(ctx->d_slot_dropped, 0, (size_t)ctx->n_slots, ctx->stream));
   HIPCHK(hipMemsetAsync(ctx->d_back_slot, 0xFF, (size_t)n * 8, ctx->stream));
   HIPCHK(hipMemsetAsync(ctx->d_front_slot0, 0xFF, (size_t)n * 8, ctx->stream));
+  HIPCHK(hipMemsetAsync(ctx->d_link_mark, 0, (size_t)n, ctx->stream));
   HIPCHK(hipMemsetAsync(ctx->d_drop_f, 0, (size_t)n, ctx->stream));
   HIPCHK(hipMemsetAsync(ctx->d_drop_b, 0, (size_t)n, ctx->stream));
   HIPCHK(hipStreamSynchronize(ctx->stream));
@@ -1563,8 +1572,9 @@
 static int finish_cull(mia_hip_ctx* ctx) {
   const int64_t nl = ctx->links_cap_all;
   if (dev_ensure(ctx, ctx->d_link_len, nl, nl + 64) || dev_ensure(ctx, ctx->d_link_act, nl, nl + 64)) return MIA_HIP_ERR_NOMEM;
-  hipLaunchKernelGGL(k_links_apply, dim3(32), dim3(256), 0, ctx->stream, ctx->d_links_all, ctx->d_n_links_all, (int32_t)ctx->links_cap_all, ctx->si,
-                     ctx->d_slot_dropped, ctx->n_slots, ctx->d_link_len, ctx->d_link_act, ctx->d_cull_flags, ctx->abort_if);
+  if (!(ctx->cull_applied && ctx->d_links_all == ctx->lk.rec))
+    hipLaunchKernelGGL(k_links_apply, dim3(32), dim3(256), 0, ctx->stream, ctx->d_links_all, ctx->d_n_links_all, (int32_t)ctx->links_cap_all, ctx->si,
+                       ctx->d_slot_dropped, ctx->n_slots, ctx->d_link_len, ctx->d_link_act, ctx->d_cull_flags, ctx->abort_if);
   ctx->links_applied = true;
   return finish_params(ctx);
 }
@@ -1602,7 +1612,12 @@
     if (dev_alloc(ctx, ctx->d_cull_sync, 4)) return MIA_HIP_ERR_NOMEM;
     HIPCHK(hipMemsetAsync(ctx->d_cull_sync, 0, 16, ctx->stream));
   }
-  hipLaunchKernelGGL(k_slot_count, dim3((unsigned)((n + 4095) / 4096)), dim3(256), 0, ctx->stream, ctx->rs, ctx->L, ctx->d_partial, nb, slot_base, ctx->d_total, (uint32_t*)nullptr, ctx->abort_if);
+  if (!ctx->d_cull_stats) {
+    if (dev_alloc(ctx, ctx->d_cull_stats, 4)) return MIA_HIP_ERR_NOMEM;
+    HIPCHK(hipMemsetAsync(ctx->d_cull_stats, 0, 16, ctx->stream));
+  }
+  hipLaunchKernelGGL(k_slot_count, dim3((unsigned)((n + 4095) / 4096)), dim3(256), 0, ctx->stream, ctx->rs, ctx->L, ctx->d_partial, nb, slot_base, ctx->d_total, (uint32_t*)nullptr, ctx->abort_if,
+                     (const uint8_t*)ctx->d_link_mark);
   if (ctx->cull_scan) hipLaunchKernelGGL(k_scan_partials, dim3(1), dim3(256), 0, ctx->stream, ctx->d_partial, nb, slot_base, ctx->d_total, ctx->abort_if);
   if (slot_base + 2 * n + 16 > ctx->n_slots) {
     DevBuf<uint8_t> nd;
@@ -1618,12 +1633,21 @@
   ctx->si.base = slot_base;
   ctx->si.n_local_p = ctx->d_total;
   if (!ctx->in_iterate) HIPCHK(hipMemsetAsync(ctx->lk.n, 0, 8, ctx->stream));
+  const bool lean_ok = ctx->in_iterate && !ctx->comm && ctx->cull_with_records && !ctx->cull_scan && !ctx->no_cull_lean;
+  const bool apply = lean_ok && !ctx->no_cull_apply;
+  if (apply && (dev_ensure(ctx, ctx->d_link_len, (int64_t)ctx->lk.cap, (int64_t)ctx->lk.cap + 64) || dev_ensure(ctx, ctx->d_link_act, (int64_t)ctx->lk.cap, (int64_t)ctx->lk.cap + 64)))
+    return MIA_HIP_ERR_NOMEM;
   hipLaunchKernelGGL(k_cull_records, dim3((unsigned)nb), dim3(256), 0, ctx->stream, ctx->rs, ctx->L, (const int64_t*)ctx->d_partial, ctx->d_slot, ctx->ri, ctx->si,
                      ctx->read_base, ctx->d_cull_flags, ctx->d_slot_dropped, ctx->n_slots, hard_cut, slope, intercept, ctx->d_back_slot,
                      (const int64_t*)ctx->d_front_slot0, ctx->lk, ctx->dev_cut, ctx->abort_if, ctx->cull_scan ? 0 : nb, slot_base, ctx->d_total,
                      ctx->cull_with_records ? 1 : 0, ctx->d_drop_f, ctx->d_drop_b,
-                     (ctx->umax_valid && ctx->rs.roff == ctx->d_roff && ctx->d_rplanes && ctx->d_umax) ? ctx->d_umax : (const int32_t*)nullptr);
+                     (ctx->umax_valid && ctx->rs.roff == ctx->d_roff && ctx->d_rplanes && ctx->d_umax) ? ctx->d_umax : (const int32_t*)nullptr,
+                     lean_ok ? 1 : 0, (int32_t*)ctx->d_cull_stats,
+                     apply ? (uint32_t*)ctx->d_cull_sync : (uint32_t*)nullptr, (int32_t*)ctx->d_link_len, (int32_t*)ctx->d_link_act,
+                     (uint8_t*)ctx->d_link_mark);
   HIPCHK(hipGetLastError());
+  ctx->cull_lean_ok = lean_ok;
+  ctx->cull_applied = apply;
   ctx->d_links_all = ctx->lk.rec;
   ctx->d_n_links_all = ctx->lk.n;
   ctx->links_cap_all = ctx->lk.cap;
@@ -1632,12 +1656,47 @@
   return finish_cull(ctx);
 }
 
+static int link_marks_launch(mia_hip_ctx* ctx) {
+  const int64_t n = ctx->rs.n;
+  if (n == 0) return MIA_HIP_OK;
+  hipLaunchKernelGGL(k_link_marks, dim3((unsigned)((n + 255) / 256)), dim3(256), 0, ctx->stream, n, (const int64_t*)ctx->d_back_slot, (const int64_t*)ctx->d_front_slot0,
+                     (uint8_t*)ctx->d_link_mark);
+  HIPCHK(hipGetLastError());
+  return MIA_HIP_OK;
+}
+static int cull_stats_read(mia_hip_ctx* ctx, int32_t* st) {
+  st[0] = -1; st[1] = 0;
+  if (!ctx->d_cull_stats) return MIA_HIP_OK;
+  HIPCHK(hipSetDevice(ctx->device));
+  HIPCHK(hipMemcpyAsync(st, ctx->d_cull_stats, 8, hipMemcpyDeviceToHost, ctx->stream));
+  HIPCHK(hipStreamSynchronize(ctx->stream));
+  return MIA_HIP_OK;
+}
+extern "C" int mia_hip_cull_stats(mia_hip_ctx* ctx, int64_t* links_before, int32_t* lean) {
+  if (!ctx) return MIA_HIP_ERR_ARG;
+  if (!ctx->culled) { ctx->err = "cull first"; return MIA_HIP_ERR_STATE; }
+  int32_t st[2];
+  if (int rc = cull_stats_read(ctx, st)) return rc;
+  if (links_before) *links_before = st[0];
+  if (lean) *lean = st[1];
+  return MIA_HIP_OK;
+}
+static int refuse_after_lean_cull(mia_hip_ctx* ctx) {
+  if (!ctx->cull_lean_ok) return MIA_HIP_OK;
+  int32_t st[2];
+  if (int rc = cull_stats_read(ctx, st)) return rc;
+  if (!st[1]) return MIA_HIP_OK;
+  ctx->err = "the last cull ran inside mia_hip_iterate without a link and left the slot and link side arrays unwritten: call mia_hip_cull first";
+  return MIA_HIP_ERR_STATE;
+}
+
 extern "C" int mia_hip_set_back_slots(mia_hip_ctx* ctx, const int64_t* back_slot) {
   if (ctx) ctx->pre_cull_valid = false;
   if (!ctx || !back_slot) return MIA_HIP_ERR_ARG;
   if (!ctx->d_back_slot) { ctx->err = "upload_reads first"; return MIA_HIP_ERR_STATE; }
   HIPCHK(hipSetDevice(ctx->device));
   HIPCHK(hipMemcpyAsync(ctx->d_back_slot, back_slot, (size_t)ctx->rs.n * 8, hipMemcpyHostToDevice, ctx->stream));
+  if (int rcm = link_marks_launch(ctx)) return rcm;
   HIPCHK(hipStreamSynchronize(ctx->stream));
   return MIA_HIP_OK;
 }
@@ -1651,6 +1710,7 @@
   if (front_slot) HIPCHK(hipMemcpyAsync(ctx->d_front_slot0, front_slot, n * 8, hipMemcpyHostToDevice, ctx->stream));
   if (back_slot) HIPCHK(hipMemcpyAsync(ctx->d_back_slot, back_slot, n * 8, hipMemcpyHostToDevice, ctx->stream));
   if (score) HIPCHK(hipMemcpyAsync(ctx->d_score, score, n * 4, hipMemcpyHostToDevice, ctx->stream));
+  if (int rcm = link_marks_launch(ctx)) return rcm;
   HIPCHK(hipStreamSynchronize(ctx->stream));
   return MIA_HIP_OK;
 }
@@ -1676,6 +1736,7 @@
   if (!ctx || n_all < 0 || (n_all > 0 && !d_links_all)) return MIA_HIP_ERR_ARG;
   if (!ctx->culled) { ctx->err = "cull first"; return MIA_HIP_ERR_STATE; }
   if (n_all >= (int64_t)LINK_NONE) { ctx->err = "too many links"; return MIA_HIP_ERR_RANGE; }
+  if (int rcl = refuse_after_lean_cull(ctx)) return rcl;
   HIPCHK(hipSetDevice(ctx->device));
   if (n_all * 4 > (ctx->owned_links.empty() ? 0 : ctx->owned_links.back().cap)) {
     DevBuf<int64_t> nb;
@@ -1702,6 +1763,7 @@
 
 extern "C" int mia_hip_link_lengths(mia_hip_ctx* ctx, int32_t** d_len, int32_t** d_act, int64_t* n) {
   if (!ctx || !ctx->links_applied) return MIA_HIP_ERR_STATE;
+  if (int rcl = refuse_after_lean_cull(ctx)) return rcl;
   HIPCHK(hipSetDevice(ctx->device));
   HIPCHK(hipStreamSynchronize(ctx->stream));
   if (d_len) *d_len = ctx->d_link_len;
@@ -1712,6 +1774,7 @@
 
 extern "C" int mia_hip_finish_links(mia_hip_ctx* ctx) {
   if (!ctx || !ctx->links_applied) return MIA_HIP_ERR_STATE;
+  if (int rcl = refuse_after_lean_cull(ctx)) return rcl;
   HIPCHK(hipSetDevice(ctx->device));
   HIPCHK(hipMemsetAsync(ctx->d_cull_flags, 0, 4, ctx->stream));
   return finish_params(ctx);
```
